# nfrasser/lasgun

Hardware: AMD Instinct MI355X
Metric: Mrays/s (primary+shadow) at 4096x4096; bit-exact RGBA8 vs CPU (higher is better)
Workload: dtype f64; 1 GPU; configs[2]: 4096x4096, Cornell shell + 1024 random plastic spheres (SplitMix64 0x1A560001), 1 spp, 1 point light; workload_key=configs2, rays_per_frame=33554429, primary=16777216

## Files before the change

bindings/rust/lasgun-hip-sys/src/lib.rs:

```rust
#![allow(non_camel_case_types)]

use std::os::raw::{c_char, c_int, c_void};

#[repr(C)]
pub struct lg_scene {
    _private: [u8; 0],
}
#[repr(C)]
pub struct lg_aggregate {
    _private: [u8; 0],
}
#[repr(C)]
pub struct lg_accel {
    _private: [u8; 0],
}
#[repr(C)]
pub struct lg_film {
    _private: [u8; 0],
}
#[repr(C)]
pub struct lg_multi {
    _private: [u8; 0],
}

// ... 250 lines not shown
    pub fn lg_scene_set_perspective_camera(a0: *mut lg_scene, fov: f64);
    pub fn lg_scene_set_orthographic_camera(a0: *mut lg_scene, scale: f64);
    pub fn lg_camera_look_at(a0: *mut lg_scene, origin: *const [f64; 3], look: *const [f64; 3], up: *const [f64; 3]);
    pub fn lg_camera_set_supersampling(a0: *mut lg_scene, base: u8);
    pub fn lg_camera_set_aperture_radius(a0: *mut lg_scene, radius: f64);
    pub fn lg_scene_set_solid_background(a0: *mut lg_scene, color: *const [f64; 3]);
    pub fn lg_scene_set_radial_background(a0: *mut lg_scene, inner: *const [f64; 3], outer: *const [f64; 3], scale: f64);
    pub fn lg_scene_set_ambient_light(a0: *mut lg_scene, color: *const [f64; 3]);
    pub fn lg_scene_set_mesh_smoothing(a0: *mut lg_scene, enabled: c_int);
    pub fn lg_scene_set_max_recursion_depth(a0: *mut lg_scene, max_depth: u32);
    pub fn lg_scene_set_threads(a0: *mut lg_scene, threads: usize);
    pub fn lg_scene_add_point_light(a0: *mut lg_scene, position: *const [f64; 3], intensity: *const [f64; 3], falloff: *const [f64; 3]);
    pub fn lg_scene_parse_obj(a0: *mut lg_scene, text: *const c_char, len: usize, out_ref: *mut u32) -> c_int;
    pub fn lg_scene_load_obj(a0: *mut lg_scene, path: *const c_char, out_ref: *mut u32) -> c_int;
    pub fn lg_scene_root(a0: *mut lg_scene) -> *mut lg_aggregate;
    pub fn lg_scene_set_root(a0: *mut lg_scene, moved: *mut lg_aggregate);
    pub fn lg_aggregate_new() -> *mut lg_aggregate;
    pub fn lg_aggregate_free(a0: *mut lg_aggregate);
    pub fn lg_aggregate_add_group(a0: *mut lg_aggregate, moved: *mut lg_aggregate);
    pub fn lg_aggregate_add_sphere(a0: *mut lg_aggregate, center: *const [f64; 3], radius: f64, a3: *const lg_material);
    pub fn lg_aggregate_add_cube(a0: *mut lg_aggregate, origin: *const [f64; 3], dim: f64, a3: *const lg_material);
    pub fn lg_aggregate_add_box(a0: *mut lg_aggregate, minbound: *const [f64; 3], maxbound: *const [f64; 3], a3: *const lg_material);
    pub fn lg_aggregate_add_obj(a0: *mut lg_aggregate, mesh: u32);
    pub fn lg_aggregate_add_obj_of(a0: *mut lg_aggregate, mesh: u32, a2: *const lg_material);
    pub fn lg_aggregate_swap_backface(a0: *mut lg_aggregate);
    pub fn lg_aggregate_translate(a0: *mut lg_aggregate, delta: *const [f64; 3]);
    pub fn lg_aggregate_scale(a0: *mut lg_aggregate, x: f64, y: f64, z: f64);
    pub fn lg_aggregate_rotate_x(a0: *mut lg_aggregate, theta_deg: f64);
    pub fn lg_aggregate_rotate_y(a0: *mut lg_aggregate, theta_deg: f64);
    pub fn lg_aggregate_rotate_z(a0: *mut lg_aggregate, theta_deg: f64);
    pub fn lg_aggregate_rotate(a0: *mut lg_aggregate, theta_deg: f64, axis: *const [f64; 3]);
    pub fn lg_film_new(width: u32, height: u32) -> *mut lg_film;
    pub fn lg_film_wrap(width: u32, height: u32, rgba: *mut u8) -> *mut lg_film;
    pub fn lg_film_pixels(a0: *mut lg_film) -> *mut u8;
    pub fn lg_film_width(a0: *mut lg_film) -> u32;
    pub fn lg_film_height(a0: *mut lg_film) -> u32;
    pub fn lg_film_free(a0: *mut lg_film);
    pub fn lg_accel_from(a0: *const lg_scene) -> *mut lg_accel;
    pub fn lg_accel_free(a0: *mut lg_accel);
    pub fn lg_capture(a0: *const lg_scene, a1: *mut lg_film) -> c_int;
    pub fn lg_capture_subset(k: usize, n: usize, a2: *const lg_accel, a3: *mut lg_film) -> c_int;
    pub fn lg_render(a0: *const lg_scene, width: u32, height: u32) -> *mut lg_film;
    pub fn lg_set_device(device: c_int) -> c_int;
    pub fn lg_device_count() -> c_int;
    pub fn lg_trim_pool(device: c_int) -> u64;
    pub fn lg_set_devices(device_ids: *const c_int, count: c_int) -> c_int;
    pub fn lg_accel_from_on(a0: *const lg_scene, device: c_int) -> *mut lg_accel;
    pub fn lg_multi_create(a0: *const lg_scene, device_ids: *const c_int, count: c_int, block_rows: u32) -> *mut lg_multi;
    pub fn lg_multi_free(a0: *mut lg_multi);
    pub fn lg_multi_capture_device(a0: *mut lg_multi, width: u32, height: u32, dev_rgba_on_root: *mut c_void) -> c_int;
    pub fn lg_multi_capture(a0: *mut lg_multi, a1: *mut lg_film) -> c_int;
    pub fn lg_multi_capture_device_all(a0: *mut lg_multi, width: u32, height: u32, dev_rgba: *mut *const c_void) -> c_int;
    pub fn lg_multi_rank_count(a0: *const lg_multi) -> c_int;
    pub fn lg_multi_accel(a0: *const lg_multi, rank: c_int) -> *mut lg_accel;
    pub fn lg_multi_uses_rccl(a0: *const lg_multi) -> c_int;
    pub fn lg_capture_rows_device(a0: *const lg_accel, width: u32, height: u32, y0: u32, y1: u32, row0: u32, dev_rgba: *mut c_void, hip_stream: *mut c_void) -> c_int;
    pub fn lg_capture_interleaved_device(a0: *const lg_accel, width: u32, height: u32, block_rows: u32, n: u32, r: u32, dev_rgba: *mut c_void, hip_stream: *mut c_void) -> c_int;
    pub fn lg_capture_subset_device(k: usize, n: usize, a2: *const lg_accel, width: u32, height: u32, dev_rgba: *mut c_void, hip_stream: *mut c_void) -> c_int;
    pub fn lg_capture_subsets(ks: *const usize, count: usize, n: usize, a3: *const lg_accel, a4: *mut lg_film) -> c_int;
    pub fn lg_capture_subsets_device(ks: *const usize, count: usize, n: usize, a3: *const lg_accel, width: u32, height: u32, dev_rgba: *mut c_void, hip_stream: *mut c_void) -> c_int;
    pub fn lg_accel_stream(a0: *const lg_accel) -> *mut c_void;
    pub fn lg_accel_synchronize(a0: *const lg_accel) -> c_int;
    pub fn lg_capture_radiance(k: usize, n: usize, a2: *const lg_accel, width: u32, height: u32, rgb: *mut f64) -> c_int;
    pub fn lg_capture_pixels(a0: *const lg_accel, width: u32, height: u32, offsets: *const u64, count: usize, rgba_out: *mut u8, rgb_out: *mut f64) -> c_int;
    pub fn lg_capture_rect(a0: *const lg_accel, width: u32, height: u32, x0: u32, y0: u32, x1: u32, y1: u32, rgba_out: *mut u8, rgb_out: *mut f64) -> c_int;
    pub fn lg_capture_stats(a0: *const lg_accel, width: u32, height: u32, y0: u32, y1: u32, out: *mut lg_stats) -> c_int;
    pub fn lg_audit_prune(a0: *const lg_accel, width: u32, height: u32, y0: u32, y1: u32, out: *mut lg_prune_audit) -> c_int;
    pub fn lg_audit_fast(a0: *const lg_accel, width: u32, height: u32, y0: u32, y1: u32, out: *mut lg_fast_audit) -> c_int;
    pub fn lg_accel_set_mode(a0: *const lg_accel, mode: c_int) -> c_int;
    pub fn lg_accel_set_prune(a0: *const lg_accel, enabled: c_int) -> c_int;
    pub fn lg_accel_set_shadow_skip(a0: *const lg_accel, enabled: c_int) -> c_int;
    pub fn lg_accel_set_level_door(a0: *const lg_accel, mask: c_int) -> c_int;
    pub fn lg_accel_set_l0_relative(a0: *const lg_accel, enabled: c_int) -> c_int;
    pub fn lg_accel_last_l0_relative(a0: *const lg_accel) -> c_int;
    pub fn lg_scene_l0_relative_origins(a0: *const lg_scene, origins: *mut f64, cap: c_int) -> c_int;
    pub fn lg_accel_set_node_pairs(a0: *const lg_accel, enabled: c_int) -> c_int;
    pub fn lg_accel_last_node_pairs(a0: *const lg_accel) -> c_int;
    pub fn lg_accel_set_packet_walk(a0: *const lg_accel, enabled: c_int) -> c_int;
    pub fn lg_accel_last_packet_walk(a0: *const lg_accel) -> c_int;
    pub fn lg_scene_packet_walk_gate(a0: *const lg_scene) -> c_int;
    pub fn lg_accel_set_fused_shade(a0: *const lg_accel, enabled: c_int) -> c_int;
    pub fn lg_accel_last_fused_shade(a0: *const lg_accel) -> c_int;
    pub fn lg_scene_fused_shade_gate(a0: *const lg_scene, camera_level0: c_int) -> c_int;
    pub fn lg_scene_lds_image(a0: *const lg_scene, pairs: c_int, words: *mut u32, cap: usize, info: *mut u32) -> i64;
    pub fn lg_accel_get_prune(a0: *const lg_accel) -> c_int;
    pub fn lg_accel_set_streaming(a0: *const lg_accel, enabled: c_int) -> c_int;
    pub fn lg_tune_export(out: *mut lg_tune_entry, capacity: usize) -> usize;
    pub fn lg_tune_import(entries: *const lg_tune_entry, count: usize) -> c_int;
    pub fn lg_tune_clear();
    pub fn lg_accel_last_organisation(a0: *const lg_accel) -> c_int;
    pub fn lg_accel_set_tile_order(a0: *const lg_accel, order: c_int) -> c_int;
    pub fn lg_accel_set_sample_order(a0: *const lg_accel, order: c_int) -> c_int;
    pub fn lg_accel_set_tile_parts(a0: *const lg_accel, parts: c_int) -> c_int;
    pub fn lg_accel_set_wf_split(a0: *const lg_accel, bands: c_int) -> c_int;
    pub fn lg_accel_set_lds_scene(a0: *const lg_accel, enabled: c_int) -> c_int;
    pub fn lg_profile_enable(a0: *const lg_accel, enabled: c_int);
    pub fn lg_profile_read(a0: *const lg_accel, total_ms: *mut f64, launches: *mut u64) -> c_int;
    pub fn lg_profile_read_kinds(a0: *const lg_accel, ms: *mut [f64; 5], launches: *mut [u64; 5]) -> c_int;
    pub fn lg_capture_stats_kind(a0: *const lg_accel, width: u32, height: u32, y0: u32, y1: u32, kind: c_int, out: *mut lg_stats) -> c_int;
    pub fn lg_accel_dump(a0: *const lg_accel, f: *mut *const f64, nf: *mut usize, i: *mut *const i64, ni: *mut usize) -> c_int;
    pub fn lg_accel_info(a0: *const lg_accel, out: *mut [u64; 8]) -> c_int;
    pub fn lg_aggregate_get_transform(a0: *mut lg_aggregate, m: *mut [f64; 16], minv: *mut [f64; 16]);
    pub fn lg_host_build_dump(a0: *const lg_scene, f: *mut *const f64, nf: *mut usize, i: *mut *const i64, ni: *mut usize, info: *mut [u64; 8]) -> c_int;
    pub fn lg_host_check_wide_records(a0: *const lg_scene, out: *mut [u64; 8]) -> c_int;
    pub fn lg_host_check_strips(a0: *const lg_scene, out: *mut [u64; 8]) -> c_int;
    pub fn lg_trace_pixel(a0: *const lg_accel, width: u32, height: u32, x: u32, y: u32, fast: c_int, out: *mut f64, out_len: usize) -> c_int;
    pub fn lg_intersect(a0: *const lg_accel, rays: *const f64, n: usize, hits: *mut lg_hit) -> c_int;
    pub fn lg_occluded(a0: *const lg_accel, rays: *const f64, n: usize, occluded: *mut u8) -> c_int;
    pub fn lg_intersect_device(a0: *const lg_accel, dev_rays: *const f64, n: usize, dev_hits: *mut lg_hit, hip_stream: *mut c_void) -> c_int;
    pub fn lg_occluded_device(a0: *const lg_accel, dev_rays: *const f64, n: usize, dev_occluded: *mut u8, hip_stream: *mut c_void) -> c_int;
    pub fn lg_visibility(a0: *const lg_accel, from: *const f64, n_from: usize, to: *const f64, n_to: usize, bits: *mut u8, row_bytes: usize, blocked: *mut u32) -> c_int;
    pub fn lg_visibility_device(a0: *const lg_accel, dev_from: *const f64, n_from: usize, dev_to: *const f64, n_to: usize, dev_bits: *mut u8, row_bytes: usize, dev_blocked: *mut u32, hip_stream: *mut c_void) -> c_int;
    pub fn lg_open_directions(a0: *const lg_accel, points: *const f64, normals: *const f64, n_points: usize, dirs: *const f64, n_dirs: usize, bits: *mut u8, row_bytes: usize, open: *mut u32, above: *mut u32) -> c_int;
    pub fn lg_open_directions_device(a0: *const lg_accel, dev_points: *const f64, dev_normals: *const f64, n_points: usize, dev_dirs: *const f64, n_dirs: usize, dev_bits: *mut u8, row_bytes: usize, dev_open: *mut u32, dev_above: *mut u32, hip_stream: *mut c_void) -> c_int;
    pub fn lg_range_scan(a0: *const lg_accel, origins: *const f64, frames: *const f64, n_poses: usize, beams: *const f64, n_beams: usize, lanes: c_int, out: *const lg_scan_out) -> c_int;
    pub fn lg_range_scan_device(a0: *const lg_accel, dev_origins: *const f64, dev_frames: *const f64, n_poses: usize, dev_beams: *const f64, n_beams: usize, lanes: c_int, dev_out: *const lg_scan_out, hip_stream: *mut c_void) -> c_int;
    pub fn lg_range_scan_lanes(n_poses: usize, n_beams: usize, lanes: c_int) -> c_int;
    pub fn lg_radiance(a0: *const lg_accel, rays: *const f64, n: usize, radiance: *mut f64) -> c_int;
    pub fn lg_radiance_device(a0: *const lg_accel, dev_rays: *const f64, n: usize, dev_radiance: *mut f64, hip_stream: *mut c_void) -> c_int;
    pub fn lg_radiance_gather(a0: *const lg_accel, origins: *const f64, frames: *const f64, n_poses: usize, dirs: *const f64, n_dirs: usize, weights: *const f64, n_weights: usize, lanes: c_int, out: *const lg_gather_out) -> c_int;
    pub fn lg_radiance_gather_device(a0: *const lg_accel, dev_origins: *const f64, dev_frames: *const f64, n_poses: usize, dev_dirs: *const f64, n_dirs: usize, dev_weights: *const f64, n_weights: usize, lanes: c_int, dev_out: *const lg_gather_out, hip_stream: *mut c_void) -> c_int;
    pub fn lg_radiance_gather_lanes(n_poses: usize, n_dirs: usize, lanes: c_int) -> c_int;
    pub fn lg_camera_rays(a0: *const lg_accel, width: u32, height: u32, x0: u32, y0: u32, x1: u32, y1: u32, rays: *mut f64) -> c_int;
    pub fn lg_camera_rays_device(a0: *const lg_accel, width: u32, height: u32, x0: u32, y0: u32, x1: u32, y1: u32, dev_rays: *mut f64, hip_stream: *mut c_void) -> c_int;
    pub fn lg_camera_samples(a0: *const lg_accel) -> u32;
    pub fn lg_capture_rays(a0: *const lg_accel, rays: *const f64, pixels: usize, samples: u32, pixel_offsets: *const u64, film: *mut lg_film, rgb: *mut f64, width: u32, height: u32) -> c_int;
    pub fn lg_capture_rays_device(a0: *const lg_accel, dev_rays: *const f64, pixels: usize, samples: u32, dev_pixel_offsets: *const u64, width: u32, height: u32, dev_rgba: *mut c_void, dev_rgb: *mut f64, hip_stream: *mut c_void) -> c_int;
    pub fn lg_capture_features(a0: *const lg_accel, width: u32, height: u32, x0: u32, y0: u32, x1: u32, y1: u32, out: *const lg_features, material_rgb: *const f64) -> c_int;
    pub fn lg_capture_features_device(a0: *const lg_accel, width: u32, height: u32, x0: u32, y0: u32, x1: u32, y1: u32, dev_out: *const lg_features, dev_material_rgb: *const f64, hip_stream: *mut c_void) -> c_int;
    pub fn lg_accel_material_count(a0: *const lg_accel) -> usize;
    pub fn lg_lens_rays(a0: *const lg_lens, width: u32, height: u32, samples_root: u32, pixel_offsets: *const u64, pixels: usize, rays: *mut f64) -> c_int;
    pub fn lg_lens_rays_device(device: c_int, a1: *const lg_lens, width: u32, height: u32, samples_root: u32, dev_pixel_offsets: *const u64, pixels: usize, dev_rays: *mut f64, hip_stream: *mut c_void) -> c_int;
    pub fn lg_view_look_at(out: *mut lg_view, perspective: c_int, param: f64, origin: *const [f64; 3], look: *const [f64; 3], up: *const [f64; 3], supersampling: u8) -> c_int;
    pub fn lg_scene_view(a0: *const lg_scene, out: *mut lg_view) -> c_int;
    pub fn lg_accel_view(a0: *const lg_accel, out: *mut lg_view) -> c_int;
    pub fn lg_view_rays(a0: *const lg_accel, a1: *const lg_view, width: u32, height: u32, x0: u32, y0: u32, x1: u32, y1: u32, rays: *mut f64) -> c_int;
    pub fn lg_view_rays_device(a0: *const lg_accel, a1: *const lg_view, width: u32, height: u32, x0: u32, y0: u32, x1: u32, y1: u32, dev_rays: *mut f64, hip_stream: *mut c_void) -> c_int;
    pub fn lg_capture_views(a0: *const lg_accel, views: *const lg_view, n_views: usize, width: u32, height: u32, rgba: *mut u8, rgb: *mut f64) -> c_int;
    pub fn lg_capture_views_device(a0: *const lg_accel, views: *const lg_view, n_views: usize, width: u32, height: u32, dev_rgba: *mut c_void, dev_rgb: *mut f64, hip_stream: *mut c_void) -> c_int;
    pub fn lg_capture_view_features(a0: *const lg_accel, views: *const lg_view, n_views: usize, width: u32, height: u32, out: *const lg_view_features, material_rgb: *const f64) -> c_int;
    pub fn lg_capture_view_features_device(a0: *const lg_accel, views: *const lg_view, n_views: usize, width: u32, height: u32, dev_out: *const lg_view_features, dev_material_rgb: *const f64, hip_stream: *mut c_void) -> c_int;
    pub fn lg_hit_layers(a0: *const lg_accel, rays: *const f64, n: usize, max_layers: u32, out: *const lg_layers_out) -> c_int;
    pub fn lg_hit_layers_device(a0: *const lg_accel, dev_rays: *const f64, n: usize, max_layers: u32, dev_out: *const lg_layers_out, hip_stream: *mut c_void) -> c_int;
    pub fn lg_trace_paths(a0: *const lg_accel, rays: *const f64, n: usize, max_bounces: u32, rules: *const lg_path_rule, n_rules: usize, normal: c_int, start_medium: *const u32, out: *const lg_paths_out) -> c_int;
    pub fn lg_trace_paths_device(a0: *const lg_accel, dev_rays: *const f64, n: usize, max_bounces: u32, rules: *const lg_path_rule, n_rules: usize, normal: c_int, dev_start_medium: *const u32, dev_out: *const lg_paths_out, hip_stream: *mut c_void) -> c_int;
    pub fn lg_radiance_groups(a0: *const lg_accel, rays: *const f64, n: usize, groups: *const lg_light_group, n_groups: usize, radiance: *mut f64) -> c_int;
    pub fn lg_radiance_groups_device(a0: *const lg_accel, dev_rays: *const f64, n: usize, groups: *const lg_light_group, n_groups: usize, dev_radiance: *mut f64, hip_stream: *mut c_void) -> c_int;
    pub fn lg_scatter(a0: *const lg_accel, rays: *const f64, n: usize, out: *const lg_scatter_out) -> c_int;
    pub fn lg_scatter_device(a0: *const lg_accel, dev_rays: *const f64, n: usize, dev_out: *const lg_scatter_out, hip_stream: *mut c_void) -> c_int;
    pub fn lg_scatter_lit(a0: *const lg_accel, rays: *const f64, n: usize, lights: *const lg_light_set, out: *const lg_lit_out) -> c_int;
    pub fn lg_scatter_lit_device(a0: *const lg_accel, dev_rays: *const f64, n: usize, lights: *const lg_light_set, dev_out: *const lg_lit_out, hip_stream: *mut c_void) -> c_int;
    pub fn lg_hit_attributes(a0: *const lg_accel, rays: *const f64, n: usize, out: *const lg_attr_out) -> c_int;
    pub fn lg_hit_attributes_device(a0: *const lg_accel, dev_rays: *const f64, n: usize, dev_out: *const lg_attr_out, hip_stream: *mut c_void) -> c_int;
    pub fn lg_hit_attributes_of(a0: *const lg_accel, rays: *const f64, hits: *const lg_hit, n: usize, out: *const lg_attr_out) -> c_int;
    pub fn lg_hit_attributes_of_device(a0: *const lg_accel, dev_rays: *const f64, dev_hits: *const lg_hit, n: usize, dev_out: *const lg_attr_out, hip_stream: *mut c_void) -> c_int;
    pub fn lg_closest_points(a0: *const lg_accel, points: *const f64, n: usize, radius: f64, out: *const lg_closest_out) -> c_int;
    pub fn lg_closest_points_device(a0: *const lg_accel, dev_points: *const f64, n: usize, radius: f64, dev_out: *const lg_closest_out, hip_stream: *mut c_void) -> c_int;
    pub fn lg_scene_closest_gate(a0: *const lg_scene, shrink: *mut f64, cap: c_int) -> c_int;
    pub fn lg_scene_closest_depth(a0: *const lg_scene) -> c_int;
    pub fn lg_accel_light_count(a0: *const lg_accel) -> c_int;
    pub fn lg_accel_set_query_order(a0: *const lg_accel, order: c_int) -> c_int;
    pub fn lg_accel_get_query_order(a0: *const lg_accel) -> c_int;
    pub fn lg_query_order(a0: *const lg_accel, rays: *const f64, n: usize, perm: *mut u32, keys: *mut u32) -> c_int;
    pub fn lg_query_order_device(a0: *const lg_accel, dev_rays: *const f64, n: usize, dev_perm: *mut u32, dev_keys: *mut u32, hip_stream: *mut c_void) -> c_int;
    pub fn lg_accel_material(a0: *const lg_accel, index: i32, out: *mut lg_material) -> c_int;
    pub fn lg_accel_instance(a0: *const lg_accel, instance: u32, parent: *mut i32, obj_ref: *mut i64) -> c_int;
// ... 6 lines not shown
```

include/lasgun_hip.h:

```cpp
#ifndef LASGUN_HIP_H
#define LASGUN_HIP_H

#include <stddef.h>
#include <stdint.h>

#ifdef __cplusplus
extern "C" {
#endif

typedef struct lg_scene lg_scene;
typedef struct lg_aggregate lg_aggregate;
typedef struct lg_accel lg_accel;
typedef struct lg_film lg_film;

typedef struct lg_material {
    int32_t kind;
    double p[10];
} lg_material;

const char *lg_last_error(void);

lg_material lg_material_default(void);
lg_material lg_material_matte(const double kd[3], double sigma);
lg_material lg_material_plastic(const double kd[3], const double ks[3], double roughness);
// ... 35 lines not shown
void lg_aggregate_rotate_y(lg_aggregate *, double theta_deg);
void lg_aggregate_rotate_z(lg_aggregate *, double theta_deg);
void lg_aggregate_rotate(lg_aggregate *, double theta_deg, const double axis[3]);

lg_film *lg_film_new(uint32_t width, uint32_t height);
lg_film *lg_film_wrap(uint32_t width, uint32_t height, uint8_t *rgba);
uint8_t *lg_film_pixels(lg_film *);
uint32_t lg_film_width(lg_film *);
uint32_t lg_film_height(lg_film *);
void lg_film_free(lg_film *);

lg_accel *lg_accel_from(const lg_scene *);
void lg_accel_free(lg_accel *);

int lg_capture(const lg_scene *, lg_film *);
int lg_capture_subset(size_t k, size_t n, const lg_accel *, lg_film *);
lg_film *lg_render(const lg_scene *, uint32_t width, uint32_t height);

typedef struct lg_stats {
    uint64_t primary_rays, shadow_rays, secondary_rays, nodes_tested, spheres_tested, cuboids_tested, triangles_tested,
        accel_entries, hits;
} lg_stats;

int lg_set_device(int device);
int lg_device_count(void);
uint64_t lg_trim_pool(int device);
int lg_set_devices(const int *device_ids, int count);

lg_accel *lg_accel_from_on(const lg_scene *, int device);

typedef struct lg_multi lg_multi;
lg_multi *lg_multi_create(const lg_scene *, const int *device_ids, int count, uint32_t block_rows);
void lg_multi_free(lg_multi *);
int lg_multi_capture_device(lg_multi *, uint32_t width, uint32_t height, void *dev_rgba_on_root);
int lg_multi_capture(lg_multi *, lg_film *);
int lg_multi_capture_device_all(lg_multi *, uint32_t width, uint32_t height, void *const *dev_rgba);
int lg_multi_rank_count(const lg_multi *);
lg_accel *lg_multi_accel(const lg_multi *, int rank);
int lg_multi_uses_rccl(const lg_multi *);

int lg_capture_rows_device(const lg_accel *, uint32_t width, uint32_t height, uint32_t y0, uint32_t y1, uint32_t row0,
                           void *dev_rgba, void *hip_stream);
int lg_capture_interleaved_device(const lg_accel *, uint32_t width, uint32_t height, uint32_t block_rows, uint32_t n,
                                  uint32_t r, void *dev_rgba, void *hip_stream);
int lg_capture_subset_device(size_t k, size_t n, const lg_accel *, uint32_t width, uint32_t height, void *dev_rgba,
                             void *hip_stream);
int lg_capture_subsets(const size_t *ks, size_t count, size_t n, const lg_accel *, lg_film *);
int lg_capture_subsets_device(const size_t *ks, size_t count, size_t n, const lg_accel *, uint32_t width, uint32_t height,
                              void *dev_rgba, void *hip_stream);
void *lg_accel_stream(const lg_accel *);
int lg_accel_synchronize(const lg_accel *);

int lg_capture_radiance(size_t k, size_t n, const lg_accel *, uint32_t width, uint32_t height, double *rgb);
int lg_capture_pixels(const lg_accel *, uint32_t width, uint32_t height, const uint64_t *offsets, size_t count,
                      uint8_t *rgba_out, double *rgb_out);
int lg_capture_rect(const lg_accel *, uint32_t width, uint32_t height, uint32_t x0, uint32_t y0, uint32_t x1, uint32_t y1,
                    uint8_t *rgba_out, double *rgb_out);
int lg_capture_stats(const lg_accel *, uint32_t width, uint32_t height, uint32_t y0, uint32_t y1, lg_stats *out);

typedef struct lg_prune_audit {
    uint64_t skipped_nodes, skipped_runs, primitives, violations;
    double min_slack_nodes, min_slack_runs;
    double max_margin_used_nodes;
} lg_prune_audit;
int lg_audit_prune(const lg_accel *, uint32_t width, uint32_t height, uint32_t y0, uint32_t y1, lg_prune_audit *out);
typedef struct lg_fast_audit { uint64_t rays, fallbacks, violations; } lg_fast_audit;
int lg_audit_fast(const lg_accel *, uint32_t width, uint32_t height, uint32_t y0, uint32_t y1, lg_fast_audit *out);

int lg_accel_set_mode(const lg_accel *, int mode);
int lg_accel_set_prune(const lg_accel *, int enabled);
int lg_accel_set_shadow_skip(const lg_accel *, int enabled);
int lg_accel_set_level_door(const lg_accel *, int mask);
int lg_accel_set_l0_relative(const lg_accel *, int enabled);
int lg_accel_last_l0_relative(const lg_accel *);
int lg_scene_l0_relative_origins(const lg_scene *, double *origins, int cap);
int lg_accel_set_node_pairs(const lg_accel *, int enabled);
int lg_accel_last_node_pairs(const lg_accel *);
int lg_accel_set_packet_walk(const lg_accel *, int enabled);
int lg_accel_last_packet_walk(const lg_accel *);
int lg_scene_packet_walk_gate(const lg_scene *);
int lg_accel_set_fused_shade(const lg_accel *, int enabled);
int lg_accel_last_fused_shade(const lg_accel *);
int lg_scene_fused_shade_gate(const lg_scene *, int camera_level0);
int64_t lg_scene_lds_image(const lg_scene *, int pairs, uint32_t *words, size_t cap, uint32_t *info);
int lg_accel_get_prune(const lg_accel *);

int lg_accel_set_streaming(const lg_accel *, int enabled);
typedef struct lg_tune_entry { uint64_t key[12]; int32_t choice; int32_t reserved; } lg_tune_entry;
size_t lg_tune_export(lg_tune_entry *out, size_t capacity);
int lg_tune_import(const lg_tune_entry *entries, size_t count);
void lg_tune_clear(void);
int lg_accel_last_organisation(const lg_accel *);
int lg_accel_set_tile_order(const lg_accel *, int order);
int lg_accel_set_sample_order(const lg_accel *, int order);
int lg_accel_set_tile_parts(const lg_accel *, int parts);


int lg_accel_set_wf_split(const lg_accel *, int bands);

int lg_accel_set_lds_scene(const lg_accel *, int enabled);


void lg_profile_enable(const lg_accel *, int enabled);
int lg_profile_read(const lg_accel *, double *total_ms, uint64_t *launches);
int lg_profile_read_kinds(const lg_accel *, double ms[5], uint64_t launches[5]);
int lg_capture_stats_kind(const lg_accel *, uint32_t width, uint32_t height, uint32_t y0, uint32_t y1, int kind, lg_stats *out);

int lg_accel_dump(const lg_accel *, const double **f, size_t *nf, const int64_t **i, size_t *ni);
int lg_accel_info(const lg_accel *, uint64_t out[8]);
void lg_aggregate_get_transform(lg_aggregate *, double m[16], double minv[16]);
int lg_host_build_dump(const lg_scene *, const double **f, size_t *nf, const int64_t **i, size_t *ni, uint64_t info[8]);
int lg_host_check_wide_records(const lg_scene *, uint64_t out[8]);
int lg_host_check_strips(const lg_scene *, uint64_t out[8]);

int lg_trace_pixel(const lg_accel *, uint32_t width, uint32_t height, uint32_t x, uint32_t y, int fast, double *out, size_t out_len);

typedef struct lg_hit {
    double t;
    double p[3];
    double ng[3];
    double ns[3];
    uint32_t kind;
    uint32_t prim;
    uint32_t instance;
    int32_t material;
} lg_hit;

int lg_intersect(const lg_accel *, const double *rays, size_t n, lg_hit *hits);
int lg_occluded(const lg_accel *, const double *rays, size_t n, uint8_t *occluded);
int lg_intersect_device(const lg_accel *, const double *dev_rays, size_t n, lg_hit *dev_hits, void *hip_stream);
int lg_occluded_device(const lg_accel *, const double *dev_rays, size_t n, uint8_t *dev_occluded, void *hip_stream);
int lg_visibility(const lg_accel *, const double *from, size_t n_from, const double *to, size_t n_to, uint8_t *bits, size_t row_bytes,
                  uint32_t *blocked);
int lg_visibility_device(const lg_accel *, const double *dev_from, size_t n_from, const double *dev_to, size_t n_to, uint8_t *dev_bits,
                         size_t row_bytes, uint32_t *dev_blocked, void *hip_stream);
int lg_open_directions(const lg_accel *, const double *points, const double *normals, size_t n_points, const double *dirs, size_t n_dirs,
                       uint8_t *bits, size_t row_bytes, uint32_t *open, uint32_t *above);
int lg_open_directions_device(const lg_accel *, const double *dev_points, const double *dev_normals, size_t n_points,
                              const double *dev_dirs, size_t n_dirs, uint8_t *dev_bits, size_t row_bytes, uint32_t *dev_open,
                              uint32_t *dev_above, void *hip_stream);
typedef struct lg_scan_out {
    float    *range;
    float    *point;
    float    *normal;
    uint32_t *id;
    uint32_t *hits;
    float    *nearest;
} lg_scan_out;
int lg_range_scan(const lg_accel *, const double *origins, const double *frames, size_t n_poses, const double *beams, size_t n_beams,
                  int lanes, const lg_scan_out *out);
int lg_range_scan_device(const lg_accel *, const double *dev_origins, const double *dev_frames, size_t n_poses, const double *dev_beams,
                         size_t n_beams, int lanes, const lg_scan_out *dev_out, void *hip_stream);
int lg_range_scan_lanes(size_t n_poses, size_t n_beams, int lanes);
int lg_radiance(const lg_accel *, const double *rays, size_t n, double *radiance);
int lg_radiance_device(const lg_accel *, const double *dev_rays, size_t n, double *dev_radiance, void *hip_stream);
typedef struct lg_gather_out {
    double *radiance;
    double *sums;
} lg_gather_out;
int lg_radiance_gather(const lg_accel *, const double *origins, const double *frames, size_t n_poses, const double *dirs, size_t n_dirs,
                       const double *weights, size_t n_weights, int lanes, const lg_gather_out *out);
int lg_radiance_gather_device(const lg_accel *, const double *dev_origins, const double *dev_frames, size_t n_poses, const double *dev_dirs,
                              size_t n_dirs, const double *dev_weights, size_t n_weights, int lanes, const lg_gather_out *dev_out,
                              void *hip_stream);
int lg_radiance_gather_lanes(size_t n_poses, size_t n_dirs, int lanes);
int lg_camera_rays(const lg_accel *, uint32_t width, uint32_t height, uint32_t x0, uint32_t y0, uint32_t x1, uint32_t y1, double *rays);
// ... 185 lines not shown
```

lasgun_amd/__init__.py:

```python
import ctypes as _C
import os as _os

import numpy as _np

from ._capi import Api, CStats, LasgunError, ObjError, QUERY_ORDER_SIGNATURES, RADIANCE_SIGNATURES, RAY_FILM_SIGNATURES, VISIBILITY_SIGNATURES, DIRECTIONS_SIGNATURES, RANGE_SCAN_SIGNATURES, HIT_LAYERS_SIGNATURES, PATHS_SIGNATURES, LIGHT_GROUPS_SIGNATURES, GATHER_SIGNATURES, FEATURES_SIGNATURES, VIEWS_SIGNATURES, VIEW_FEATURES_SIGNATURES, CView, CLens, CFeatures, CViewFeatures, CScanOut, CLayersOut, CPathRule, CPathsOut, CGatherOut, CLightGroup, GROUP_AMBIENT, MAX_LIGHT_GROUPS, SCATTER_SIGNATURES, CScatterOut, SCATTER_HIT, SCATTER_REFLECT, SCATTER_REFRACT, LIT_SIGNATURES, CLight, CLightSet, CLitOut, MAX_CALL_LIGHTS, ATTRIBUTES_SIGNATURES, CAttrOut, ATTR_HIT, ATTR_NO_HIT, ATTR_BAD_RECORD, CLOSEST_SIGNATURES, CClosestOut
from . import scenes

_HERE = _os.path.dirname(_os.path.abspath(__file__))
LIB_PATH = _os.environ.get("LASGUN_HIP_LIB") or _os.path.join(_HERE, "liblasgun_hip.so")

if not _os.path.exists(LIB_PATH):
    raise ImportError(
        "lasgun_amd: %s is missing -- build it with `python -c 'import __graft_entry__ as g; g.build()'` "
        "or `make -C lasgun_amd/csrc` (there is no CPU fallback)" % LIB_PATH)

_EXTRA = {
    "set_device": (_C.c_int, [_C.c_int]),
    "device_count": (_C.c_int, []),
    "trim_pool": (_C.c_uint64, [_C.c_int]),
    "set_devices": (_C.c_int, [_C.POINTER(_C.c_int), _C.c_int]),
    "capture_rows_device": (_C.c_int, [_C.c_void_p, _C.c_uint32, _C.c_uint32, _C.c_uint32, _C.c_uint32, _C.c_uint32,
                                       _C.c_void_p, _C.c_void_p]),
    "capture_subset_device": (_C.c_int, [_C.c_size_t, _C.c_size_t, _C.c_void_p, _C.c_uint32, _C.c_uint32, _C.c_void_p,
                                         _C.c_void_p]),
    "capture_subsets": (_C.c_int, [_C.POINTER(_C.c_size_t), _C.c_size_t, _C.c_size_t, _C.c_void_p, _C.c_void_p]),
    "capture_subsets_device": (_C.c_int, [_C.POINTER(_C.c_size_t), _C.c_size_t, _C.c_size_t, _C.c_void_p, _C.c_uint32, _C.c_uint32, _C.c_void_p,
                                          _C.c_void_p]),
    "capture_interleaved_device": (_C.c_int, [_C.c_void_p, _C.c_uint32, _C.c_uint32, _C.c_uint32, _C.c_uint32, _C.c_uint32,
                                              _C.c_void_p, _C.c_void_p]),
    "accel_stream": (_C.c_void_p, [_C.c_void_p]),
    "accel_set_mode": (_C.c_int, [_C.c_void_p, _C.c_int]),
    "accel_set_prune": (_C.c_int, [_C.c_void_p, _C.c_int]),
    "accel_set_shadow_skip": (_C.c_int, [_C.c_void_p, _C.c_int]),
    "accel_set_level_door": (_C.c_int, [_C.c_void_p, _C.c_int]),
    "accel_set_l0_relative": (_C.c_int, [_C.c_void_p, _C.c_int]),
    "accel_last_l0_relative": (_C.c_int, [_C.c_void_p]),
    "scene_l0_relative_origins": (_C.c_int, [_C.c_void_p, _C.POINTER(_C.c_double), _C.c_int]),
    "accel_set_node_pairs": (_C.c_int, [_C.c_void_p, _C.c_int]),
    "accel_last_node_pairs": (_C.c_int, [_C.c_void_p]),
    "accel_set_packet_walk": (_C.c_int, [_C.c_void_p, _C.c_int]),
    "accel_last_packet_walk": (_C.c_int, [_C.c_void_p]),
    "scene_packet_walk_gate": (_C.c_int, [_C.c_void_p]),
    "accel_set_fused_shade": (_C.c_int, [_C.c_void_p, _C.c_int]),
    "accel_last_fused_shade": (_C.c_int, [_C.c_void_p]),
    "scene_fused_shade_gate": (_C.c_int, [_C.c_void_p, _C.c_int]),
    "scene_lds_image": (_C.c_longlong, [_C.c_void_p, _C.c_int, _C.POINTER(_C.c_uint32), _C.c_size_t, _C.POINTER(_C.c_uint32)]),
    "accel_set_streaming": (_C.c_int, [_C.c_void_p, _C.c_int]),
    "accel_get_prune": (_C.c_int, [_C.c_void_p]),
    "accel_last_organisation": (_C.c_int, [_C.c_void_p]),
    "accel_set_tile_order": (_C.c_int, [_C.c_void_p, _C.c_int]),
    "accel_set_sample_order": (_C.c_int, [_C.c_void_p, _C.c_int]),
    "accel_set_tile_parts": (_C.c_int, [_C.c_void_p, _C.c_int]),
    "accel_set_lds_scene": (_C.c_int, [_C.c_void_p, _C.c_int]),
    "accel_set_wf_split": (_C.c_int, [_C.c_void_p, _C.c_int]),
    "accel_synchronize": (_C.c_int, [_C.c_void_p]),
    "capture_radiance": (_C.c_int, [_C.c_size_t, _C.c_size_t, _C.c_void_p, _C.c_uint32, _C.c_uint32, _C.c_void_p]),
    "capture_pixels": (_C.c_int, [_C.c_void_p, _C.c_uint32, _C.c_uint32, _C.c_void_p, _C.c_size_t, _C.c_void_p, _C.c_void_p]),
    "capture_rect": (_C.c_int, [_C.c_void_p, _C.c_uint32, _C.c_uint32, _C.c_uint32, _C.c_uint32, _C.c_uint32, _C.c_uint32, _C.c_void_p, _C.c_void_p]),
    "audit_prune": (_C.c_int, [_C.c_void_p, _C.c_uint32, _C.c_uint32, _C.c_uint32, _C.c_uint32, _C.c_void_p]),
    "audit_fast": (_C.c_int, [_C.c_void_p, _C.c_uint32, _C.c_uint32, _C.c_uint32, _C.c_uint32, _C.c_void_p]),
    "capture_stats": (_C.c_int, [_C.c_void_p, _C.c_uint32, _C.c_uint32, _C.c_uint32, _C.c_uint32, _C.POINTER(CStats)]),
    "profile_enable": (None, [_C.c_void_p, _C.c_int]),
    "profile_read_kinds": (_C.c_int, [_C.c_void_p, _C.c_double * 5, _C.c_uint64 * 5]),
    "capture_stats_kind": (_C.c_int, [_C.c_void_p, _C.c_uint32, _C.c_uint32, _C.c_uint32, _C.c_uint32, _C.c_int, _C.POINTER(CStats)]),
    "profile_read": (_C.c_int, [_C.c_void_p, _C.POINTER(_C.c_double), _C.POINTER(_C.c_uint64)]),
    "probe_rate": (_C.c_int, [_C.c_int, _C.POINTER(_C.c_double)]),
    "accel_from_on": (_C.c_void_p, [_C.c_void_p, _C.c_int]),
    "tune_export": (_C.c_size_t, [_C.c_void_p, _C.c_size_t]),
    "tune_import": (_C.c_int, [_C.c_void_p, _C.c_size_t]),
    "tune_clear": (None, []),
    "multi_create": (_C.c_void_p, [_C.c_void_p, _C.POINTER(_C.c_int), _C.c_int, _C.c_uint32]),
    "multi_free": (None, [_C.c_void_p]),
    "multi_capture_device": (_C.c_int, [_C.c_void_p, _C.c_uint32, _C.c_uint32, _C.c_void_p]),
    "multi_capture": (_C.c_int, [_C.c_void_p, _C.c_void_p]),
    "multi_capture_device_all": (_C.c_int, [_C.c_void_p, _C.c_uint32, _C.c_uint32, _C.POINTER(_C.c_void_p)]),
    "multi_rank_count": (_C.c_int, [_C.c_void_p]),
    "multi_accel": (_C.c_void_p, [_C.c_void_p, _C.c_int]),
    "multi_uses_rccl": (_C.c_int, [_C.c_void_p]),
    "accel_info": (_C.c_int, [_C.c_void_p, _C.c_uint64 * 8]),
    "trace_pixel": (_C.c_int, [_C.c_void_p, _C.c_uint32, _C.c_uint32, _C.c_uint32, _C.c_uint32, _C.c_int, _C.POINTER(_C.c_double), _C.c_size_t]),
    "host_build_dump": (_C.c_int, [_C.c_void_p, _C.POINTER(_C.POINTER(_C.c_double)), _C.POINTER(_C.c_size_t),
                                   _C.POINTER(_C.POINTER(_C.c_int64)), _C.POINTER(_C.c_size_t), _C.c_uint64 * 8]),
    "host_check_wide_records": (_C.c_int, [_C.c_void_p, _C.c_uint64 * 8]),
    "host_check_strips": (_C.c_int, [_C.c_void_p, _C.c_uint64 * 8]),
    "intersect": (_C.c_int, [_C.c_void_p, _C.c_void_p, _C.c_size_t, _C.c_void_p]),
    "occluded": (_C.c_int, [_C.c_void_p, _C.c_void_p, _C.c_size_t, _C.c_void_p]),
    "intersect_device": (_C.c_int, [_C.c_void_p, _C.c_void_p, _C.c_size_t, _C.c_void_p, _C.c_void_p]),
    "occluded_device": (_C.c_int, [_C.c_void_p, _C.c_void_p, _C.c_size_t, _C.c_void_p, _C.c_void_p]),
    "camera_rays": (_C.c_int, [_C.c_void_p] + [_C.c_uint32] * 6 + [_C.c_void_p]),
    "camera_rays_device": (_C.c_int, [_C.c_void_p] + [_C.c_uint32] * 6 + [_C.c_void_p, _C.c_void_p]),
    "camera_samples": (_C.c_uint32, [_C.c_void_p]),
    "accel_material": (_C.c_int, [_C.c_void_p, _C.c_int32, _C.c_void_p]),
    "accel_instance": (_C.c_int, [_C.c_void_p, _C.c_uint32, _C.POINTER(_C.c_int32), _C.POINTER(_C.c_int64)]),
    **QUERY_ORDER_SIGNATURES,
    **RADIANCE_SIGNATURES,
    **RAY_FILM_SIGNATURES,
    **VISIBILITY_SIGNATURES,
    **DIRECTIONS_SIGNATURES,
    **RANGE_SCAN_SIGNATURES,
    **HIT_LAYERS_SIGNATURES,
    **PATHS_SIGNATURES,
    **SCATTER_SIGNATURES,
    **LIT_SIGNATURES,
    **ATTRIBUTES_SIGNATURES,
    **CLOSEST_SIGNATURES,
    **LIGHT_GROUPS_SIGNATURES,
    **GATHER_SIGNATURES,
    **FEATURES_SIGNATURES,
    **VIEWS_SIGNATURES,
    **VIEW_FEATURES_SIGNATURES,
}


class Hit(_C.Structure):
    _fields_ = [("t", _C.c_double), ("p", _C.c_double * 3), ("ng", _C.c_double * 3), ("ns", _C.c_double * 3),
                ("kind", _C.c_uint32), ("prim", _C.c_uint32), ("instance", _C.c_uint32), ("material", _C.c_int32)]


HIT_DTYPE = _np.dtype(Hit)
assert _C.sizeof(Hit) == 96 and HIT_DTYPE.itemsize == 96, "lg_hit is 96 bytes"
LENS_EQUIRECTANGULAR, LENS_FISHEYE = 0, 1
assert _C.sizeof(CLens) == 112, "lg_lens is 112 bytes"
assert _C.sizeof(CFeatures) == 40, "lg_features is 40 bytes"
FEATURE_PLANES = ("depth", "normal", "albedo", "coverage", "id")
assert _C.sizeof(CScanOut) == 48, "lg_scan_out is 48 bytes"
SCAN_PLANES = ("range", "point", "normal", "id", "hits", "nearest")
_SCAN_SHAPE = {"range": ((), _np.float32, True), "point": ((3,), _np.float32, True), "normal": ((3,), _np.float32, True), "id": ((4,), _np.uint32, True),
               "hits": ((), _np.uint32, False), "nearest": ((), _np.float32, False)}
SCAN_LANES = {"auto": 0, "beam": 1, "pose": 2}
assert _C.sizeof(CLayersOut) == 40, "lg_layers_out is 40 bytes"
LAYER_PLANES = ("hits", "along", "id", "count", "inside")
_LAYER_SHAPE = {"hits": ((), HIT_DTYPE, True), "along": ((), _np.float64, True), "id": ((4,), _np.uint32, True), "count": ((), _np.uint32, False),
                "inside": ((), _np.float64, False)}
assert _C.sizeof(CPathRule) == 24 and _C.sizeof(CPathsOut) == 72, "lg_path_rule is 24 bytes, lg_paths_out 72"
PATH_PLANES = ("hits", "point", "id", "along", "count", "end", "gain", "last", "medium")
_PATH_SHAPE = {"hits": ((), HIT_DTYPE, True), "point": ((3,), _np.float64, True), "id": ((4,), _np.uint32, True), "along": ((), _np.float64, True),
               "count": ((), _np.uint32, False), "end": ((), _np.uint32, False), "gain": ((), _np.float64, False), "last": ((6,), _np.float64, False),
               "medium": ((), _np.uint32, False)}
PATH_ABSORB, PATH_REFLECT, PATH_PASS, PATH_REFRACT = 0, 1, 2, 3
PATH_END_CUT, PATH_END_ESCAPED, PATH_END_ABSORBED, PATH_END_DEGENERATE = 0, 1, 2, 3
PATH_RULE_DTYPE = _np.dtype([("action", _np.uint32), ("reserved", _np.uint32), ("ior", _np.float64), ("gain", _np.float64)])
assert PATH_RULE_DTYPE.itemsize == 24
assert _C.sizeof(CScatterOut) == 56, "lg_scatter_out is 56 bytes"
SCATTER_PLANES = ("hits", "direct", "flags", "reflect", "reflect_weight", "refract", "refract_weight")
_SCATTER_SHAPE = {"hits": ((), HIT_DTYPE), "direct": ((3,), _np.float64), "flags": ((), _np.uint32), "reflect": ((6,), _np.float64),
                  "reflect_weight": ((3,), _np.float64), "refract": ((6,), _np.float64), "refract_weight": ((5,), _np.float64)}
assert _C.sizeof(CLight) == 72 and _C.sizeof(CLightSet) == 40 and _C.sizeof(CLitOut) == 72, "lg_light is 72 bytes, lg_light_set 40, lg_lit_out 72"
LIT_PLANES = SCATTER_PLANES + ("terms", "visible")
assert _C.sizeof(CAttrOut) == 56, "lg_attr_out is 56 bytes"
ATTR_PLANES = ("hits", "flags", "bary", "uv", "local", "frame", "dp")
_ATTR_SHAPE = {"hits": ((), HIT_DTYPE), "flags": ((), _np.uint32), "bary": ((3,), _np.float64), "uv": ((2,), _np.float64), "local": ((3,), _np.float64),
               "frame": ((6,), _np.float64), "dp": ((6,), _np.float64)}
assert _C.sizeof(CClosestOut) == 24, "lg_closest_out is 24 bytes"
CLOSEST_PLANES = ("distance", "point", "id")
_CLOSEST_SHAPE = {"distance": ((), _np.float64), "point": ((3,), _np.float64), "id": ((4,), _np.uint32)}
LIGHT_DTYPE = _np.dtype([("position", _np.float64, (3,)), ("intensity", _np.float64, (3,)), ("falloff", _np.float64, (3,))])
assert LIGHT_DTYPE.itemsize == 72


def Light(position, intensity, falloff=(1.0, 0.0, 0.0)):
    return (tuple(float(x) for x in position), tuple(float(x) for x in intensity), tuple(float(x) for x in falloff))


def lights_array(lights):
    if isinstance(lights, _np.ndarray) and lights.dtype == LIGHT_DTYPE:
        return _np.ascontiguousarray(lights)
    if isinstance(lights, _np.ndarray):
        a = _np.ascontiguousarray(lights, dtype=_np.float64)
        if a.ndim < 1 or a.shape[-1] != 9:
            raise ValueError("lights: the last axis holds position, intensity and falloff, nine doubles")
        return a.view(LIGHT_DTYPE).reshape(a.shape[:-1])
    out = _np.zeros(len(lights), dtype=LIGHT_DTYPE)
    for k, (p, i, f) in enumerate(lights):
        out[k] = (p, i, f)
    return out


assert _C.sizeof(CGatherOut) == 16, "lg_gather_out is 16 bytes"
GATHER_PLANES = ("radiance", "sums")
GATHER_LANES = {"auto": 0, "direction": 1, "pose": 2}
_FEATURE_SHAPE = {"depth": ((), _np.float32), "normal": ((3,), _np.float32), "albedo": ((3,), _np.float32), "coverage": ((), _np.float32),
                  "id": ((4,), _np.uint32)}
assert _C.sizeof(CViewFeatures) == 48, "lg_view_features is 48 bytes"
VIEW_FEATURE_PLANES = FEATURE_PLANES + ("point",)
_VIEW_FEATURE_SHAPE = dict(_FEATURE_SHAPE, point=((3,), _np.float32))


def Lens(kind, origin, right, up, forward, fov_deg=180.0):
    three = lambda v: (_C.c_double * 3)(*[float(c) for c in v])
    return CLens(int(kind), 0, three(origin), three(right), three(up), three(forward), float(fov_deg))


View = CView


def _views(views):
    vs = [views] if isinstance(views, CView) else list(views)
    for v in vs:
        if not isinstance(v, CView):
            raise TypeError("views: View records (lasgun_amd.View)")
    return (CView * len(vs))(*vs)


# ... 18 lines not shown
            return _C.c_void_p(self.call("accel_stream", accel.h))
        return _C.c_void_p(int(stream))

    def set_mode(self, accel, fast):
        if self.call("accel_set_mode", accel.h, 1 if fast else 0):
            raise LasgunError(self.last_error())

    def set_prune(self, accel, enabled):
        if self.call("accel_set_prune", accel.h, -1 if enabled is None or enabled == -1 else (1 if enabled else 0)):
            raise LasgunError(self.last_error())

    def set_shadow_skip(self, accel, enabled):
        if self.call("accel_set_shadow_skip", accel.h, 1 if enabled else 0):
            raise LasgunError(self.last_error())

    def set_level_door(self, accel, mask):
        if self.call("accel_set_level_door", accel.h, int(mask)):
            raise LasgunError(self.last_error())

    def set_l0_relative(self, accel, enabled):
        if self.call("accel_set_l0_relative", accel.h, 1 if enabled else 0):
            raise LasgunError(self.last_error())

    def last_l0_relative(self, accel):
        v = self.call("accel_last_l0_relative", accel.h)
        return None if v < 0 else bool(v)

    def set_node_pairs(self, accel, enabled):
        if self.call("accel_set_node_pairs", accel.h, 1 if enabled else 0):
            raise LasgunError(self.last_error())

    def last_node_pairs(self, accel):
        v = self.call("accel_last_node_pairs", accel.h)
        return None if v < 0 else bool(v)

    def set_packet_walk(self, accel, enabled):
        if self.call("accel_set_packet_walk", accel.h, 1 if enabled else 0):
            raise LasgunError(self.last_error())

    def last_packet_walk(self, accel):
        v = self.call("accel_last_packet_walk", accel.h)
        return None if v < 0 else bool(v)

    def scene_lds_image(self, scene, pairs):
        info = (_C.c_uint32 * 8)()
        n = self.call("scene_lds_image", scene.h, 1 if pairs else 0, None, 0, info)
        if n < 0:
            raise LasgunError(self.last_error())
        if n == 0:
            return None
        words = _np.zeros(n, dtype=_np.uint32)
        self.call("scene_lds_image", scene.h, 1 if pairs else 0, words.ctypes.data_as(_C.POINTER(_C.c_uint32)), n, info)
        keys = ("units", "node_off", "prim_off", "soup_off", "accel_off", "pairs", "accels", "nodes")
        return words, {k: int(info[i]) for i, k in enumerate(keys)}

    def l0_relative_origins(self, scene):
        import numpy as np
        out = np.zeros((64, 3), dtype=np.float64)
        n = self.call("scene_l0_relative_origins", scene.h, out.ctypes.data_as(_C.POINTER(_C.c_double)), 64)
        if n < 0:
            raise LasgunError(self.last_error())
        return out[:n].copy() if n else None

    def scene_packet_walk_gate(self, scene):
        v = self.call("scene_packet_walk_gate", scene.h)
        if v < 0:
            raise LasgunError(self.last_error())
        return int(v)

    def set_fused_shade(self, accel, enabled):
        if self.call("accel_set_fused_shade", accel.h, 1 if enabled else 0):
            raise LasgunError(self.last_error())

    def last_fused_shade(self, accel):
        v = self.call("accel_last_fused_shade", accel.h)
        return None if v < 0 else bool(v)

    def scene_fused_shade_gate(self, scene, camera_level0=True):
        v = self.call("scene_fused_shade_gate", scene.h, 1 if camera_level0 else 0)
        if v < 0:
            raise LasgunError(self.last_error())
        return int(v)

    def last_organisation(self, accel):
        v = self.call("accel_last_organisation", accel.h)
        name = {0: "megakernel", 1: "wavefront", 2: "queue"}.get(v & 15) if v >= 0 else None
        if name and (v & 16):
            name += ", bottom-up"
        if name and (v & 64):
            name += ", middle-out"
        if name and (v & 32):
            name += ", samples in a row"
        if name and (v & 128):
            name += ", tiles in parts"
        return name

    def set_tile_order(self, accel, order):
        if self.call("accel_set_tile_order", accel.h, -1 if order is None else int(order)):
            raise LasgunError(self.last_error())

    def set_tile_parts(self, accel, parts):
        if self.call("accel_set_tile_parts", accel.h, -1 if parts is None else int(parts)):
            raise LasgunError(self.last_error())

    def set_sample_order(self, accel, order):
        if self.call("accel_set_sample_order", accel.h, -1 if order is None else int(order)):
            raise LasgunError(self.last_error())

    def get_prune(self, accel):
        return bool(self.call("accel_get_prune", accel.h))

    def set_streaming(self, accel, enabled):
        if self.call("accel_set_streaming", accel.h, int(enabled) if enabled in (0, 1, 2, 3) else (1 if enabled else 0)):
            raise LasgunError(self.last_error())

    def set_wf_split(self, accel, bands):
        self.call("accel_set_wf_split", accel.h, int(bands))

    def set_lds_scene(self, accel, enabled):
        return bool(self.call("accel_set_lds_scene", accel.h, 1 if enabled else 0))

    def set_device(self, device):
        if self.call("set_device", int(device)):
            raise LasgunError(self.last_error())

    def trace_pixel_log(self, accel, w, h, x, y, fast=False, nlights=1):
        need = 7 + 2 * nlights
        n = need + 1 + 4 * 4000
        out = (_C.c_double * n)()
        if self.call("trace_pixel", accel.h, int(w), int(h), int(x), int(y), 1 if fast else 0, out, n):
            raise LasgunError(self.last_error())
        cnt = int(out[need])
        return [tuple(out[need + 1 + 4 * i + k] for k in range(4)) for i in range(cnt)]

    def trace_pixel(self, accel, w, h, x, y, fast=False, max_lights=64):
        n = 7 + 2 * max_lights
        out = (_C.c_double * n)()
        if self.call("trace_pixel", accel.h, int(w), int(h), int(x), int(y), 1 if fast else 0, out, n):
            raise LasgunError(self.last_error())
        nl = int(out[3])
        return {"t": out[0], "ref": int(out[1]), "accel": int(out[2]), "shadow": [(out[4 + 2 * l], int(out[5 + 2 * l])) for l in range(nl)],
                "shadow_origin": [out[4 + 2 * nl], out[5 + 2 * nl], out[6 + 2 * nl]]}

    def set_devices(self, ids=None):
        ids = list(ids or [])
        arr = (_C.c_int * max(len(ids), 1))(*ids)
        if self.call("set_devices", arr, len(ids)):
            raise LasgunError(self.last_error())

    def trim_pool(self, device=-1):
        return int(self.call("trim_pool", int(device)))

    def device_count(self):
        return int(self.call("device_count"))

    def capture_rows_device(self, accel, width, height, y0, y1, dev_ptr, row0=None, stream=None):
        if self.call("capture_rows_device", accel.h, width, height, y0, y1, y0 if row0 is None else row0,
                     _C.c_void_p(int(dev_ptr)), self._stream(accel, stream)):
            raise LasgunError(self.last_error())

    def capture_interleaved_device(self, accel, width, height, block_rows, n, r, dev_ptr, stream=None):
        if self.call("capture_interleaved_device", accel.h, width, height, block_rows, n, r, _C.c_void_p(int(dev_ptr)),
                     self._stream(accel, stream)):
            raise LasgunError(self.last_error())

    def capture_subset_device(self, k, n, accel, width, height, dev_ptr, stream=None):
# ... 1101 lines not shown
```

lasgun_amd/csrc/accel.cpp:

```cpp
#include "internal.h"
#include "attributes_host.h"
#include "pairs_host.h"

static std::vector<uint32_t> attr_counts_of(const FlatScene &f, const Scene &scene) {
    std::vector<uint32_t> faces(f.accels.size(), 0u), tri_base(f.accels.size(), 0u), sphere_accel(f.spheres.size(), NO_HIT), cuboid_accel(f.cuboids.size(), NO_HIT);
    std::vector<uint32_t> todo;
    for (size_t id = 0; id < f.accels.size(); ++id) {
        const DAccel &A = f.accels[id];
        if (A.flags & AF_MESH) {
            const int64_t obj = id < f.accel_obj.size() ? f.accel_obj[id] : -1;
            if (obj >= 0 && (size_t)obj < scene.meshes.size() && scene.meshes[(size_t)obj]) faces[id] = (uint32_t)(scene.meshes[(size_t)obj]->tri.size() / 3);
            tri_base[id] = id < f.accel_tri_base.size() ? f.accel_tri_base[id] : 0u;
            if ((size_t)tri_base[id] + faces[id] > f.tri_v.size() / 3) faces[id] = 0u;
            continue;
        }
        if (A.node_base >= f.nodes.size()) continue;
        todo.assign(1, 0u);
        while (!todo.empty()) {
            const uint32_t nidx = todo.back();
            todo.pop_back();
            const DNode &nd = f.nodes[A.node_base + nidx];
            if (!(nd.meta & NODE_LEAF)) { todo.push_back(nidx + 1u); todo.push_back(nd.link); continue; }
            for (uint32_t k = 0; k < (nd.meta & 0xFFFFu); ++k) {
                const uint32_t ref = f.primref[(size_t)A.prim_base + nd.link + k], kind = ref >> 30, idx = ref & PRIM_INDEX_MASK;
                if (kind == PK_SPHERE && idx < sphere_accel.size()) sphere_accel[idx] = (uint32_t)id;
                else if (kind == PK_CUBOID && idx < cuboid_accel.size()) cuboid_accel[idx] = (uint32_t)id;
            }
        }
    }
    return attr_counts_build(faces, tri_base, sphere_accel, cuboid_accel);
}

static void set_lds_limits(size_t bytes, bool ldss) {
    for (auto set : {mega_set_lds_limit, wf_set_lds_limit, queue_set_lds_limit, query_set_lds_limit, rq_set_lds_limit, visibility_set_lds_limit, features_set_lds_limit,
                     open_directions_set_lds_limit, range_scan_set_lds_limit, hit_layers_set_lds_limit, trace_paths_set_lds_limit, gather_set_lds_limit, view_set_lds_limit, view_features_set_lds_limit, light_groups_set_lds_limit, scatter_set_lds_limit, lit_set_lds_limit, attributes_set_lds_limit})
        HIP_TRY(set(bytes, ldss));
}

constexpr size_t LDS_MAX = 160 * 1024;
static bool make_lds_image(lg_accel *a, size_t big_mesh_tris, std::vector<uint32_t> &img) {
    static const bool times = std::getenv("LASGUN_DEBUG_TIMES") != nullptr;
    a->lds_image_n16 = 0; a->lds_pairs = false; a->pair_refusal.clear(); a->pair_rel.clear();
    {
        {
            FlatScene &fm = a->flat;
            std::vector<uint32_t> nb, pb;
            for (const DAccel &A : fm.accels) { nb.push_back(A.node_base); nb.push_back(A.fnode_base); pb.push_back(A.prim_base); pb.push_back(A.fprim_base); }
            std::sort(nb.begin(), nb.end()); nb.erase(std::unique(nb.begin(), nb.end()), nb.end());
            std::sort(pb.begin(), pb.end()); pb.erase(std::unique(pb.begin(), pb.end()), pb.end());
            auto extent = [](const std::vector<uint32_t> &starts, uint32_t b, size_t total) {
                auto it = std::upper_bound(starts.begin(), starts.end(), b);
                return (uint32_t)((it == starts.end() ? total : (size_t)*it) - b);
            };
            std::vector<std::pair<uint32_t, uint32_t>> nruns, pruns;
            uint32_t nn = 0, np = 0;
            uint32_t np_soup = 0;
            const size_t stack_bytes = (size_t)a->stack_depth * 1024 * 4;
            const size_t accel16 = fm.accels.size() * LDS_ACCEL_UNITS;
            auto number = [&](bool own_trees) {
                nruns.clear(); pruns.clear(); nn = np = np_soup = 0;
                for (int pass = 0; pass < 2; ++pass) {
                  if (pass == 1) np_soup = np;
                  for (DAccel &A : fm.accels) {
                    if (((A.flags & AF_MESH) != 0u) != (pass == 1)) continue;
                    auto fn = own_trees ? nruns.end() : std::find_if(nruns.begin(), nruns.end(), [&](auto &r) { return r.first == A.node_base; });
                    if (fn == nruns.end()) { nruns.emplace_back(A.node_base, nn); A.lnode_base = nn; nn += extent(nb, A.node_base, fm.nodes.size()); }
                    else A.lnode_base = fn->second;
                    auto fp = std::find_if(pruns.begin(), pruns.end(), [&](auto &r) { return r.first == A.prim_base; });
                    if (fp == pruns.end()) { pruns.emplace_back(A.prim_base, np); A.lprim_base = np; np += extent(pb, A.prim_base, fm.primref.size()); }
                    else A.lprim_base = fp->second;
                  }
                }
                return (size_t)nn * LDS_NODE_STRIDE + ((size_t)np + 3) / 4 + (size_t)np_soup * 3 + accel16;
            };
            size_t n16 = number(false);
            if (fm.accels.size() <= L0_REL_MAX_ACCELS && nruns.size() < fm.accels.size()) {
                const size_t shared16 = n16, own16 = number(true);
                if (stack_bytes + own16 * 16 > LDS_MAX || (own16 - shared16) * 16 > shared16) n16 = number(false);
                else n16 = own16;
            }
            const size_t prim16 = ((size_t)np + 3) / 4;
            a->l0_rel.clear();
            if (stack_bytes + n16 * 16 <= LDS_MAX) {
                img.assign(n16 * 4, 0u);
                a->lds_node_off = 0;
                for (auto &r : nruns)
                    for (uint32_t i = 0, e = extent(nb, r.first, fm.nodes.size()); i < e; ++i) {
                        uint32_t *rec = &img[((size_t)(r.second + i) * LDS_NODE_STRIDE) * 4];
                        std::memcpy(rec, &fm.nodes[r.first + i], 56);
                    }
                a->lds_prim_off = nn * LDS_NODE_STRIDE;
                a->lds_soup_off = a->lds_prim_off + (uint32_t)prim16;
                for (auto &r : pruns)
                    for (uint32_t i = 0, e = extent(pb, r.first, fm.primref.size()); i < e; ++i) {
                        img[(size_t)a->lds_prim_off * 4 + r.second + i] = fm.primref[r.first + i];
                        if (r.second + i < np_soup)
                            std::memcpy(&img[((size_t)a->lds_soup_off + (size_t)(r.second + i) * 3) * 4], &fm.leaf_soup[r.first + i], 48);
                    }
                for (const DAccel &A : fm.accels) {
                    const uint32_t tree0 = a->lds_node_off * 16u + A.lnode_base * LDS_NODE_STRIDE * 16u;
                    for (uint32_t i = 0, e = extent(nb, A.node_base, fm.nodes.size()); i < e; ++i) {
                        uint32_t *rec = &img[((size_t)(A.lnode_base + i) * LDS_NODE_STRIDE) * 4];
                        const DNode &nd = fm.nodes[A.node_base + i];
                        if (nd.meta & NODE_LEAF) { rec[16] = A.lprim_base + nd.link; rec[17] = NODE_LEAF; rec[18] = rec[16] + (nd.meta & 0xFFFFu); rec[19] = nd.pad; }
                        else { rec[16] = tree0 + nd.link * LDS_NODE_STRIDE * 16u; rec[17] = 1u << (nd.meta & 3u); rec[18] = 0u; }
                        rec[17] |= nd.meta & NODE_NOPRUNE;
                    }
                }
                a->lds_accel_off = a->lds_soup_off + np_soup * 3u;
                for (size_t i = 0; i < fm.accels.size(); ++i) {
                    const DAccel &A = fm.accels[i];
                    uint32_t *rec = &img[((size_t)a->lds_accel_off + i * LDS_ACCEL_UNITS) * 4];
                    std::memcpy(rec, &A.minv, 96);
// ... 124 lines not shown
                    double v = (c == 3 ? A.m.c[3][r] : 0.0);
                    for (int k = 0; k < 3; ++k) v += A.m.c[k][r] * (c == 3 ? A.minv.c[3][k] : A.minv.c[c][k]);
                    const double want = (c < 3 && r == c) ? 1.0 : 0.0;
                    if (!(std::fabs(v - want) <= worst)) worst = std::fabs(v - want);
                }
            if (!(worst <= 1e-11)) {
                a->fast_available = false;
                a->fast_refusal = "fast mode unavailable: an aggregate's transform and inverse do not match (rotate() about a non-unit axis?)";
            }
        }
        for (const auto &m : a->scene->meshes) {
            if (!m || !with_fast) continue;
            double max_abs = 0.0, min_edge = INFINITY;
            for (float v : m->position) if (std::isfinite(v)) max_abs = std::fmax(max_abs, std::fabs((double)v));
            for (size_t t = 0; t + 2 < m->tri.size(); t += 3) {
                double longest = 0.0;
                for (int e = 0; e < 3; ++e) {
                    const size_t i = (size_t)m->tri[t + e].v, j = (size_t)m->tri[t + (e + 1) % 3].v;
                    double d2 = 0.0;
                    for (int c = 0; c < 3; ++c) { const double d = (double)m->position[3 * i + c] - (double)m->position[3 * j + c]; d2 += d * d; }
                    longest = std::fmax(longest, std::sqrt(d2));
                }
                if (longest > 0.0 && std::isfinite(longest)) min_edge = std::fmin(min_edge, longest);
            }
            if (std::isfinite(min_edge) && max_abs > min_edge * 0x1p20) {
                a->fast_available = false;
                a->fast_refusal = "fast mode unavailable: a mesh whose coordinates exceed 2^20 times its smallest triangle (a ray in a far triangle's plane is accepted by the reference wherever it passes)";
            }
        }
        if (!a->fast_available) a->stack_depth_fast1 = a->stack_depth;
        a->accel_image_n16 = 0;
        {
            const size_t img = f.accels.size() * LDS_ACCEL_UNITS * 16;
            if (f.accels.size() <= 64 && ((size_t)a->stack_depth * 256 * 4 + img) * 4 <= LDS_MAX) a->accel_image_n16 = (uint32_t)(f.accels.size() * LDS_ACCEL_UNITS);
        }
        const size_t extra_lds = (size_t)a->accel_image_n16 * 16;
        size_t lds = (size_t)std::max(a->stack_depth, a->stack_depth_fast1) * 256 * 4 + extra_lds;
        if (lds > 64 * 1024) set_lds_limits(lds, false);
        int per_cu = 0, cus = 0;
        HIP_TRY(trace_occupancy(a->stack_depth, false, extra_lds, &per_cu));
        int per_cu_fast = 0;
        HIP_TRY(trace_occupancy(a->stack_depth_fast1, true, 0, &per_cu_fast));
        if (per_cu_fast < 1) per_cu_fast = 1;
        a->max_blocks_fast = (uint32_t)per_cu_fast;
        HIP_TRY(hipDeviceGetAttribute(&cus, hipDeviceAttributeMultiprocessorCount, a->device));
        if (per_cu < 1) per_cu = 1;
        a->max_blocks = (uint32_t)(per_cu * cus);
        a->max_blocks_fast *= (uint32_t)cus;
        int wb = 0, wbf = 0;
        HIP_TRY(wf_trace_occupancy(a->stack_depth, false, extra_lds, &wb));
        HIP_TRY(wf_trace_occupancy(a->stack_depth_fast1, true, 0, &wbf));
        a->wf_blocks = (uint32_t)((wb < 1 ? 1 : wb) * cus);
        a->wf_blocks_fast = (uint32_t)((wbf < 1 ? 1 : wbf) * cus);
        int qb = 0;
        HIP_TRY(queue_occupancy(a->stack_depth, extra_lds, &qb));
        a->queue_blocks = (uint32_t)((qb < 1 ? 1 : qb) * cus);
        a->cus = (uint32_t)cus;
        {
            std::vector<uint32_t> img;
            if (make_lds_image(a, big_mesh_tris, img)) {
                stage.add(a->lds_image, img);
                set_lds_limits(LDS_MAX, true);
                a->ldss_blocks = (uint32_t)cus;
            }
            FlatScene &fm = a->flat;
            stage.add(a->accels, fm.accels);
            if (a->accel_image_n16) {
                std::vector<uint32_t> img((size_t)a->accel_image_n16 * 4, 0u);
                for (size_t i = 0; i < fm.accels.size(); ++i) {
                    const DAccel &A = fm.accels[i];
                    uint32_t *rec = &img[i * LDS_ACCEL_UNITS * 4];
                    std::memcpy(rec, &A.minv, 96);
                    rec[24] = A.node_base; rec[25] = A.prim_base; rec[26] = 0u; rec[27] = A.flags;
                    rec[28] = (uint32_t)A.parent; rec[29] = A.nchain; rec[30] = A.lone;
                    for (int k = 0; k < MAX_CHAIN; ++k) rec[32 + k] = A.chain[k];
                    std::memcpy(rec + 40, A.prune, sizeof A.prune);
                    std::memcpy(rec + LDS_ACCEL_DOOR * 4, A.door, sizeof A.door);
                }
                stage.add(a->accel_image, img);
            }
        }
        stage.add(a->accel_tri_base, f.accel_tri_base);
        stage.add(a->attr_counts, attr_counts_of(a->flat, *a->scene));
        stage.commit(a->arena);
        {
            size_t big_mesh = 0;
            for (const auto &m : a->scene->meshes) if (m && m->tri.size() / 3 > big_mesh) big_mesh = m->tri.size() / 3;
            a->prune_default = big_mesh >= PRUNE_MIN_TRIS;
            a->streaming_pays = f.spheres.size() + f.cuboids.size() >= 512 && !(f.has_specular && big_mesh >= 4096);
            a->mega_narrow = f.spheres.size() + f.cuboids.size() < 512;
            bool specular_mesh = false;
            for (const DAccel &A : f.accels)
                if ((A.flags & AF_MESH) && A.material >= 0) {
                    const int kind = f.materials[(size_t)A.material].kind;
                    size_t tris = 0;
                    for (const auto &m : a->scene->meshes) if (m && m->tri.size() / 3 > tris) tris = m->tri.size() / 3;
                    specular_mesh = specular_mesh || ((kind == MAT_GLASS || kind == MAT_MIRROR) && tris >= 4096);
                }
            a->queue_default = f.has_specular && big_mesh >= 4096 && specular_mesh;
            a->streaming_min_items = big_mesh >= 4096 ? (1ull << 23) : (1ull << 21);
        }
        if (times) {
            const auto t_end = std::chrono::steady_clock::now();
            auto ms = [](auto a0, auto a1) { return std::chrono::duration<double, std::milli>(a1 - a0).count(); };
            std::fprintf(stderr, "[lasgun] accel build: flatten %.3f ms, table uploads %.3f ms, streams / occupancy / LDS images %.3f ms\n", ms(t_begin, t_flat), ms(t_flat, t_up), ms(t_up, t_end));
        }
}

static void swap_tables(lg_accel &x, lg_accel &y) {
    using std::swap;
    swap(x.flat, y.flat);
    swap(x.arena, y.arena); swap(x.stats, y.stats);
    swap(x.nodes, y.nodes); swap(x.nodes4, y.nodes4); swap(x.primref, y.primref); swap(x.spheres, y.spheres); swap(x.sphere_mat, y.sphere_mat);
    swap(x.cuboids, y.cuboids); swap(x.cuboid_mat, y.cuboid_mat); swap(x.tri_v, y.tri_v); swap(x.tri_n, y.tri_n); swap(x.tri_t, y.tri_t);
    swap(x.vpos, y.vpos); swap(x.vnorm, y.vnorm); swap(x.vtex, y.vtex); swap(x.leaf_soup, y.leaf_soup); swap(x.chunks, y.chunks); swap(x.strips, y.strips);
    swap(x.sphere_ref_leaf, y.sphere_ref_leaf); swap(x.cuboid_ref_leaf, y.cuboid_ref_leaf); swap(x.tri_ref_leaf, y.tri_ref_leaf); swap(x.accel_ref_leaf, y.accel_ref_leaf);
    swap(x.accels, y.accels); swap(x.materials, y.materials); swap(x.lights, y.lights); swap(x.accel_tri_base, y.accel_tri_base); swap(x.attr_counts, y.attr_counts);
    swap(x.lds_image, y.lds_image); swap(x.accel_image, y.accel_image); swap(x.accel_image_n16, y.accel_image_n16);
    swap(x.lds_image_n16, y.lds_image_n16); swap(x.lds_node_off, y.lds_node_off); swap(x.lds_prim_off, y.lds_prim_off);
    swap(x.lds_soup_off, y.lds_soup_off); swap(x.lds_accel_off, y.lds_accel_off);
    swap(x.ldss_blocks, y.ldss_blocks); swap(x.cus, y.cus); swap(x.l0_rel, y.l0_rel);
    swap(x.lds_pairs, y.lds_pairs); swap(x.pair_refusal, y.pair_refusal); swap(x.pair_rel, y.pair_rel);
    swap(x.stack_depth, y.stack_depth); swap(x.stack_depth_fast1, y.stack_depth_fast1); swap(x.max_blocks, y.max_blocks); swap(x.max_blocks_fast, y.max_blocks_fast);
    swap(x.wf_blocks, y.wf_blocks); swap(x.wf_blocks_fast, y.wf_blocks_fast); swap(x.queue_blocks, y.queue_blocks);
    swap(x.queue_default, y.queue_default); swap(x.prune_default, y.prune_default); swap(x.queue_min_items, y.queue_min_items); swap(x.specular_small_items, y.specular_small_items);
    swap(x.device_bytes, y.device_bytes); swap(x.fast_available, y.fast_available); swap(x.fast_refusal, y.fast_refusal);
    swap(x.streaming_pays, y.streaming_pays); swap(x.streaming_min_items, y.streaming_min_items); swap(x.mega_narrow, y.mega_narrow);
    x.packet_scene = y.packet_scene = -1;
}
void rebuild_tables(const lg_accel *ca, bool fast) {
    if (fast && ca->flat.has_fast) return;
    lg_accel *a = const_cast<lg_accel *>(ca);
    use_device(a->device);
    std::unique_ptr<lg_accel> next(new lg_accel());
    next->scene = a->scene;
    next->device = a->device;
    next->prune = a->prune == 1 || a->flat.has_records ? 1 : a->prune;
    next->node_pairs = a->node_pairs;
    next->image_prune = a->prune;
    build_and_upload(next.get(), fast || a->flat.has_fast);
    next->prune = a->prune;
    if (next->flat.dump_f.size() != a->flat.dump_f.size() ||
        (!a->flat.dump_f.empty() && std::memcmp(next->flat.dump_f.data(), a->flat.dump_f.data(), a->flat.dump_f.size() * sizeof(a->flat.dump_f[0])) != 0) ||
        next->flat.dump_i != a->flat.dump_i)
        throw Error("the scene was modified after lg_accel_from: the accel's reference trees no longer match it (build a new accel)");
    HIP_TRY(hipDeviceSynchronize());
    swap_tables(*a, *next);
    std::swap(a->flat.dump_f, next->flat.dump_f);
    std::swap(a->flat.dump_i, next->flat.dump_i);
}

lg_accel *accel_from_on(const lg_scene *s, int device) {
    lg_accel *a = nullptr;
    int rc = guarded([&] {
        a = new lg_accel();
        a->scene = &s->s;
        a->device = device;
        build_and_upload(a, false);
    });
    if (rc) { delete a; return nullptr; }
    return a;
}
```

lasgun_amd/csrc/capi.cpp:

```cpp
#include "internal.h"
#include "choice.h"
#include "packet_host.h"
#include "fused_host.h"
#include "closest_host.h"

extern "C" {

const char *lg_last_error(void) { return tl_error.c_str(); }

size_t lg_tune_export(lg_tune_entry *out, size_t capacity) {
    const size_t n = lg::tune::snapshot(nullptr, nullptr, 0);
    if (!out || capacity == 0) return n;
    std::vector<lg::tune::Key> keys(capacity);
    std::vector<int> choices(capacity);
    const size_t m = lg::tune::snapshot(keys.data(), choices.data(), capacity);
    for (size_t i = 0; i < std::min(m, capacity); ++i) {
        std::memcpy(out[i].key, keys[i].v, sizeof out[i].key);
        out[i].choice = choices[i];
        out[i].reserved = 0;
    }
    return m;
}
int lg_tune_import(const lg_tune_entry *entries, size_t count) {
    if (count != 0 && !entries) return fail("lg_tune_import: entries is NULL");
// ... 689 lines not shown
int lg_accel_set_packet_walk(const lg_accel *a, int enabled) {
    if (enabled != 0 && enabled != 1) return fail("packet walk must be 0 or 1");
    std::lock_guard<std::mutex> g(a->mtx);
    a->packet_walk = enabled == 1;
    return 0;
}
int lg_accel_last_packet_walk(const lg_accel *a) {
    std::lock_guard<std::mutex> g(a->mtx);
    return a->last_packet_walk;
}
int lg_scene_l0_relative_origins(const lg_scene *s, double *origins, int cap) {
    int n = 0;
    int rc = guarded([&] {
        FlatScene f;
        flatten_scene(s->s, f, false, false);
        const Camera &c = s->s.camera;
        std::vector<V3> local;
        if (!l0_relative_camera(c.origin, c.up, c.aux, c.pixel_separation) || !l0_relative_origins(f, c.origin, local)) return;
        n = (int)local.size();
        for (int i = 0; i < n && i < cap && origins; ++i) { origins[3 * i] = local[(size_t)i].x; origins[3 * i + 1] = local[(size_t)i].y; origins[3 * i + 2] = local[(size_t)i].z; }
    });
    return rc ? -1 : n;
}
int lg_scene_packet_walk_gate(const lg_scene *s) {
    int v = 0;
    int rc = guarded([&] {
        FlatScene f;
        flatten_scene(s->s, f, false, false);
        v = (int)packet_scene_gate(f.accels.data(), f.accels.size(), f.nodes.data(), f.nodes.size(), f.primref.data(), f.primref.size(), f.max_stack + 2u);
    });
    return rc ? -1 : v;
}
int lg_scene_closest_gate(const lg_scene *s, double *shrink, int cap) {
    int v = -1;
    int rc = guarded([&] {
        if (!s) throw Error("scene is NULL");
        FlatScene f;
        flatten_scene(s->s, f, false, false);
        v = closest_gate(ClosestScene{f.accels.data(), f.accels.size(), f.nodes.data(), f.nodes.size(), f.primref.data(), f.primref.size(), f.leaf_soup.data(),
                                      f.leaf_soup.size()}, shrink, cap);
    });
    return rc ? -2 : v;
}
int lg_scene_closest_depth(const lg_scene *s) {
    int v = 0;
    int rc = guarded([&] {
        if (!s) throw Error("scene is NULL");
        FlatScene f;
        flatten_scene(s->s, f, false, false);
        v = (int)closest_tables(ClosestScene{f.accels.data(), f.accels.size(), f.nodes.data(), f.nodes.size(), f.primref.data(), f.primref.size(), f.leaf_soup.data(),
                                             f.leaf_soup.size()}).depth;
    });
    return rc ? -1 : v;
}
int lg_accel_set_fused_shade(const lg_accel *a, int enabled) {
    if (enabled != 0 && enabled != 1) return fail("fused shade must be 0 or 1");
    std::lock_guard<std::mutex> g(a->mtx);
    a->fused_shade = enabled == 1;
    return 0;
}
int lg_accel_last_fused_shade(const lg_accel *a) {
    std::lock_guard<std::mutex> g(a->mtx);
    return a->last_fused_shade;
}
int lg_scene_fused_shade_gate(const lg_scene *s, int camera_level0) {
    int v = 0;
    int rc = guarded([&] {
        FlatScene f;
        flatten_scene(s->s, f, false, false);
        std::vector<uint32_t> img;
        uint32_t inf[8] = {0, 0, 0, 0, 0, 0, 0, 0};
        const bool pairs = scene_lds_image(s->s, true, img, inf) && inf[5] == 1u;
        FusedAsk q;
        q.switched_on = true;
        q.camera_level0 = camera_level0 != 0;
        q.levels = (f.has_specular && s->s.recursion > 0) ? (unsigned)s->s.recursion + 1u : 1u;
        q.nlights = (unsigned long)f.lights.size();
        q.packet_closest = pairs && packet_scene_gate(f.accels.data(), f.accels.size(), f.nodes.data(), f.nodes.size(), f.primref.data(), f.primref.size(), f.max_stack + 2u) == PACKET_OK;
        q.pair_shadow = pairs;
        v = (int)fused_shade_gate(q);
    });
    return rc ? -1 : v;
}
int lg_accel_set_mode(const lg_accel *a, int mode) {
    if (mode != 0 && mode != 1) return fail("mode must be 0 (reference traversal) or 1 (fast)");
    std::lock_guard<std::mutex> g(a->mtx);
    if (mode == 1) {
        int rc = guarded([&] { rebuild_tables(a, true); });
        if (rc) return rc;
    }
    if (mode == 1 && !a->fast_available) return fail(a->fast_refusal);
    a->fast = mode == 1;
    return 0;
}
void lg_profile_enable(const lg_accel *a, int enabled) {
    std::lock_guard<std::mutex> g(a->mtx);
    a->profiling = enabled != 0;
}
int lg_profile_read(const lg_accel *a, double *total_ms, uint64_t *launches) {
    return guarded([&] {
        std::lock_guard<std::mutex> g(a->mtx);
        double total = 0.0;
        for (auto &e : a->events) {
            HIP_TRY(hipEventSynchronize(e.second));
            float ms = 0.f;
            HIP_TRY(hipEventElapsedTime(&ms, e.first, e.second));
            total += ms;
            (void)hipEventDestroy(e.first); (void)hipEventDestroy(e.second);
        }
        *total_ms = total;
        *launches = a->events.size();
        a->events.clear();
    });
}

int lg_profile_read_kinds(const lg_accel *a, double ms[5], uint64_t launches[5]) {
    return guarded([&] {
        std::lock_guard<std::mutex> g(a->mtx);
        for (int k = 0; k < 5; ++k) {
            double total = 0.0;
            for (auto &e : a->kind_events[k]) {
                HIP_TRY(hipEventSynchronize(e.second));
                float t = 0.f;
                HIP_TRY(hipEventElapsedTime(&t, e.first, e.second));
                if (std::getenv("LASGUN_DEBUG")) std::fprintf(stderr, "[lasgun] kind %d launch: %.3f ms\n", k, t);
                total += t;
                (void)hipEventDestroy(e.first); (void)hipEventDestroy(e.second);
            }
            ms[k] = total; launches[k] = a->kind_events[k].size();
            a->kind_events[k].clear();
        }
    });
}
int lg_accel_dump(const lg_accel *a, const double **f, size_t *nf, const int64_t **i, size_t *ni) {
    *f = a->flat.dump_f.data(); *nf = a->flat.dump_f.size();
    *i = a->flat.dump_i.data(); *ni = a->flat.dump_i.size();
    return 0;
}
int lg_host_build_dump(const lg_scene *s, const double **f, size_t *nf, const int64_t **i, size_t *ni, uint64_t info[8]) {
    static thread_local FlatScene flat;
    return guarded([&] {
        flatten_scene(s->s, flat);
        *f = flat.dump_f.data(); *nf = flat.dump_f.size();
        *i = flat.dump_i.data(); *ni = flat.dump_i.size();
        info[0] = flat.nodes.size(); info[1] = flat.primref.size(); info[2] = flat.spheres.size(); info[3] = flat.cuboids.size();
        info[4] = flat.tri_v.size() / 3; info[5] = flat.accels.size(); info[6] = flat.max_stack; info[7] = flat.has_specular ? 1 : 0;
    });
}
int lg_host_check_strips(const lg_scene *s, uint64_t out[8]) {
    return guarded([&] {
        FlatScene flat;
        flatten_scene(s->s, flat, false);
        for (int k = 0; k < 8; ++k) out[k] = 0;
        std::vector<char> seen_node(flat.nodes.size(), 0);
        for (const DAccel &A : flat.accels) {
            if (!(A.flags & AF_MESH)) continue;
            std::vector<uint32_t> todo{0};
            while (!todo.empty()) {
                const uint32_t nidx = todo.back(); todo.pop_back();
                if (seen_node[A.node_base + nidx]) continue;
                seen_node[A.node_base + nidx] = 1;
                const DNode &nd = flat.nodes[A.node_base + nidx];
                if (!(nd.meta & NODE_LEAF)) { todo.push_back(nidx + 1); todo.push_back(nd.link); continue; }
                const uint32_t nrec = nd.pad >> 24, rec0 = nd.pad & 0x00FFFFFFu;
                if (nrec == 0) continue;
                out[0]++;
// ... 244 lines not shown
```

lasgun_amd/csrc/dscene.h:

```cpp
#pragma once
#include "vecmath.h"

namespace lg {

enum PrimKind : uint32_t { PK_SPHERE = 0, PK_CUBOID = 1, PK_TRIANGLE = 2, PK_ACCEL = 3 };
constexpr uint32_t PRIM_INDEX_MASK = 0x3FFFFFFFu;
constexpr uint32_t NO_HIT = 0xFFFFFFFFu;
constexpr uint32_t WF_NONE = 0xFFFFFFFFu, WF_MISS = 0xFFFFFFFEu;
constexpr uint32_t WF_SKIP = 0x80000000u;
constexpr int MAX_CHAIN = 8;
constexpr uint32_t TILE_HEADS = 8u, TILE_HEAD_STRIDE = 32u;
constexpr uint32_t TILE_HEAD0 = 32u, TILE_GONE = 16u;
constexpr uint32_t TILE_COUNTER_WORDS = TILE_HEAD0 + TILE_HEADS * TILE_HEAD_STRIDE;
constexpr uint32_t NO_TILE = 0xFFFFFFFFu;
constexpr uint32_t NODE_LEAF = 0x80000000u;
constexpr uint32_t NODE_NOPRUNE = 0x40000000u;
constexpr double PRUNE_E1 = 0x1p-46;
constexpr double PRUNE_E0_PER_COORD = 0x1p-46;
constexpr double PRUNE_E2_TIMES_RMIN = 0x1p-42;
constexpr double PRUNE_LIMIT_REL = 0x1p-40;
constexpr double PRUNE_RANGE = 0x1p100;
constexpr uint32_t LDS_NODE_STRIDE = 5u;
constexpr uint32_t LDS_ACCEL_UNITS = 16u;
constexpr uint32_t PAIR_REC_BYTES = 112u, PAIR_ROOT_BYTES = 64u, PAIR_WORDS_OFF = 96u, PAIR_ROOT_WORD_OFF = 48u;
// ... 33 lines not shown
struct alignas(64) DChunk {
    float bmin[3], bmax[3];
    float axis[3];
    float cos_t;
    float g2;
    float hmin;
    uint32_t start, count;
    float sin_t;
    uint32_t pad;
};
static_assert(sizeof(DChunk) == 64, "DChunk is one 64-byte line");
struct alignas(16) DStrip {
    float x, y, z;
    uint32_t code;
};
constexpr uint32_t STRIP_TRI = 0x80000000u, STRIP_SLOT_MASK = 0x0FFFFFFFu;
constexpr uint32_t CHUNK_SHIFT = 5u;
constexpr uint32_t CHUNK_GROUP = 2u;
constexpr uint32_t CHUNK_IS_GROUP = 0xFFFFFFFFu;
constexpr float CHUNK_K0 = 0x1p-38f;
constexpr float CHUNK_SIGMA_MIN = 1e-3f;
constexpr float CHUNK_HGATE = 0x1p-40f;

struct DMaterial {
    int32_t kind;
    int32_t pad;
    double p[10];
};
enum MatKind : int32_t { MAT_MATTE = 0, MAT_PLASTIC = 1, MAT_METAL = 2, MAT_GLASS = 3, MAT_MIRROR = 4 };

struct DLight {
    double pos[3], intensity[3], falloff[3];
};

enum AccelFlags : uint32_t { AF_SWAP_BACKFACE = 1, AF_MESH = 2, AF_HAS_N = 4, AF_HAS_UV = 8, AF_IDENTITY = 16  };

struct alignas(16) DAccel {
    Affine m;
    Affine minv;
    uint32_t node_base;
    uint32_t prim_base;
    int32_t parent;
    int32_t material;
    uint32_t flags;
    uint32_t nchain;
    uint32_t chain[MAX_CHAIN];
    uint32_t fnode_base;
    uint32_t fprim_base;
    uint32_t lnode_base;
    uint32_t lprim_base;
    uint32_t lone;
    uint32_t pad;
    double prune[6];
    double door[6];
};

constexpr uint32_t QC_FINISHED = 0u, QC_ERROR = 32u, QC_HEADS = 64u , QC_LEVEL0 = 384u,
                   QC_LEVEL_WORDS = 128u, QC_COUNT = 0u, QC_CLAIMED = 32u, QC_STATE = 64u;
constexpr uint32_t QC_MAX_LEVELS = 8u;
constexpr uint32_t QC_WORDS = QC_LEVEL0 + QC_LEVEL_WORDS * QC_MAX_LEVELS;
constexpr uint32_t QR_LAST = 0x80000000u;
constexpr uint32_t QR_SLACK = 16u;

struct DStats {
    unsigned long long primary_rays, shadow_rays, secondary_rays, nodes_tested, spheres_tested, cuboids_tested,
        triangles_tested, accel_entries, hits;
    unsigned long long audit_nodes, audit_runs, audit_prims, audit_violations, audit_slack_nodes, audit_slack_runs;
    unsigned long long audit_used_nodes;
};

constexpr int FRAME_DOUBLES = 18;
constexpr int STASH_DOUBLES = 13;

struct DRowTab { uint32_t base, rem; };

constexpr uint32_t L0_REL_MAX_ACCELS = 16u;
struct DRelAccel {
    double o[3];
    uint32_t node_off;
    uint32_t node_n;
    uint32_t slot0;
    uint32_t slot_n;
};

struct DParams {
    const DNode *nodes;
    const DNode4 *nodes4;
    const uint32_t *primref;
    const DSphere *spheres;
    const int32_t *sphere_mat;
    const DCuboid *cuboids;
    const int32_t *cuboid_mat;
    const uint32_t *tri_v;
    const uint32_t *tri_n;
    const uint32_t *tri_t;
    const float *vpos;
    const float *vnorm;
    const float *vtex;
    const DLeafRec *leaf_soup;
    const DChunk *chunks;
    const DStrip *strips;
    const uint32_t *sphere_ref_leaf, *cuboid_ref_leaf, *tri_ref_leaf, *accel_ref_leaf;
    const DAccel *accels;
    const DMaterial *materials;
    const DLight *lights;
    uint32_t nlights;
    uint32_t recursion;
    int32_t default_material;
    uint32_t stack_depth;
    V3 cam_origin, cam_view, cam_up, cam_aux;
    double image_plane_height, pixel_separation, ss_distance;
    uint32_t ss_root;
    uint32_t boxes_finite;
    double ah_omax, ah_dmin, ah_dmax;
    V3 bg_inner, bg_outer;
    double bg_scale;
    V3 ambient;
    uint32_t w, h;
    double winv, hinv, aspect;
    uint32_t mode;
    uint32_t x0, y0, x1, y1;
    uint32_t tiles_x;
    uint32_t ilv_n, ilv_r, ilv_b;
    unsigned long long sub_k, sub_n, sub_count;
    uint32_t sub_m;
    uint32_t sub_cols;
    uint32_t sub_rows;
    uint32_t sub_kk, sub_kdiv;
    const DRowTab *sub_rowtab;
    uint32_t ntiles;
    uint32_t tile_rev;
    uint32_t out_row0;
    uint32_t out_x0;
    uint32_t out_pitch;
    uint32_t out_compact;
    const unsigned long long *pixel_list;
    uint8_t *out_rgba;
    double *out_radiance;
    uint32_t *tile_counter;
    double *frames;
    unsigned long long frame_threads;
    double *stash;
    DStats *stats;
    double *dbg_log;
    unsigned long long n_items;
    double *frame;
    uint32_t *vis;
    double *accum;
    uint32_t sample_index;
    uint32_t ss_par;
    uint32_t split_shift;
    uint32_t wf_level;
    uint32_t wf_levels;
    uint32_t tile0;
    uint32_t prune;
    uint32_t *wf_counts;
    unsigned long long wf_cap;
    unsigned long long wf_cap_next;
    unsigned long long wf_hit_cap;
    unsigned long long wf_hit_stride;
    double *wf_q;
    double *wf_out;
    double *wf_spec;
    uint32_t *wf_child;
    double *wf_q_next;
    double *wf_out_next;
    uint32_t *wf_hq;
    uint32_t *q_ctl;
    uint32_t *q_ready;
    uint32_t *q_err;
    uint32_t q_units, q_unit_tiles;
    uint32_t q_order, q_blocks_x, q_tiles_y, q_seq_len;
    double *q_rays[8];
    double *q_out[8];
    double *q_spec[8];
    uint32_t *q_child[8];
    const void *lds_image;
    uint32_t lds_image_n16;
    uint32_t mega_lanes;
    uint32_t lds_node_off;
    uint32_t lds_prim_off;
    uint32_t lds_soup_off;
    uint32_t lds_accel_off;
    const void *accel_image;
    uint32_t accel_image_n16;
    unsigned long long *stamp_counts;
    uint32_t stats_filter;
    uint32_t audit;
    uint32_t shadow_skip;
    uint32_t level_door;
    uint32_t l0_rel_n;
    DRelAccel l0_rel[L0_REL_MAX_ACCELS];
    uint32_t lds_pairs;
    struct { uint32_t root_off, pair_off, pair_n, pad; } pair_rel[L0_REL_MAX_ACCELS];
    uint32_t packet;
    uint32_t fused;
};
static_assert(sizeof(DParams) <= 4096, "DParams is passed by value: a kernel's arguments are at most 4 KB");
inline bool wf_takes_pairs(const DParams &P, bool fast) { return P.lds_image && P.lds_pairs && !fast && !P.prune; }

struct RadianceArgs {
    const double *rays;
    double *radiance;
    const uint32_t *perm;
    unsigned long long n;
    unsigned long long base;
};
struct FilmArgs : RadianceArgs {
    const unsigned long long *offsets;
    unsigned long long npix;
    uint32_t *rgba;
    double *rgb;
};

constexpr uint32_t MAX_LIGHT_GROUPS = 64u;
constexpr uint32_t GROUP_AMBIENT = 1u;
struct DLightGroup { uint32_t lights, flags; };
struct GroupArgs : RadianceArgs {
    double *xout, *xout_next;
    uint32_t n_groups, pad;
    DLightGroup groups[MAX_LIGHT_GROUPS];
};

struct ScatterArgs : RadianceArgs {
    void *hits;
    double *direct;
    uint32_t *flags;
    double *reflect;
    double *reflect_weight;
    double *refract;
    double *refract_weight;
    const uint32_t *tri_base;
};
constexpr uint32_t SCATTER_HIT = 1u, SCATTER_REFLECT = 2u, SCATTER_REFRACT = 4u;

constexpr uint32_t MAX_CALL_LIGHTS = 1024u;
struct LitArgs : ScatterArgs {
    const DLight *lights;
    double *terms;
    uint32_t *visible;
    uint32_t n_lights, per_ray, vis_words, skip;
    double ambient[3];
};

struct GatherArgs {
    const double *origins;
    const double *frames;
    const double *dirs;
    double *li;
    unsigned long long n_poses, n_dirs;
    unsigned long long base_tile;
    uint32_t tiles_per;
    uint32_t pose_lanes;
};

struct DView {
    V3 origin, view, up, aux;
    double image_plane_height, pixel_separation, ss_distance;
    uint32_t ss_root, pad;
};
struct ViewArgs {
    const DView *views;
    unsigned long long n_views;
    uint32_t w, h;
    uint32_t tiles_x;
    uint32_t tiles_per_view;
    unsigned long long base_tile;
    uint32_t *rgba;
    double *rgb;
};

struct DLens {
    int32_t kind, reserved;
    V3 origin, right, up, forward;
    double fov_deg;
};

}
```

lasgun_amd/csrc/internal.h:

```cpp
#pragma once
#include <hip/hip_runtime_api.h>

#include <algorithm>
#include <array>
#include <atomic>
#include <chrono>
#include <cstdio>
#include <cstdlib>
#include <cmath>
#include <cstring>
#include <functional>
#include <map>
#include <memory>
#include <mutex>
#include <set>
#include <string>
#include <thread>
#include <vector>

#include "../../include/lasgun_hip.h"
#include "host.h"
#include "raykey.h"
#include "tune.h"

namespace lg {
hipError_t launch_trace(const DParams &P, bool stats, bool fast, uint32_t blocks, uint32_t stack_depth, hipStream_t stream);
hipError_t trace_occupancy(uint32_t stack_depth, bool fast, size_t extra_lds, int *blocks_per_cu);
hipError_t launch_wf_trace(const DParams &P, bool fast, bool shadow, uint32_t blocks, uint32_t stack_depth, hipStream_t stream);
hipError_t launch_wf_shade(const DParams &P, uint32_t blocks, hipStream_t stream);
hipError_t launch_wf_combine(const DParams &P, uint32_t blocks, hipStream_t stream);
hipError_t launch_query(const DParams &P, const double *rays, unsigned long long n, void *hits, uint8_t *occluded, const uint32_t *tri_base,
                        const uint32_t *perm, bool fast, uint32_t blocks, uint32_t stack_depth, hipStream_t stream);
size_t sort_scratch_bytes(unsigned long long n);
hipError_t launch_query_order(const double *rays, unsigned long long n, const KeyBounds &B, void *scratch, uint32_t *keys_out, uint32_t *perm_out,
                              const uint32_t **perm, uint32_t grid_cap, hipStream_t stream);
hipError_t launch_camera_rays(const DParams &P, double *rays, unsigned long long n, uint32_t blocks, hipStream_t stream);
hipError_t query_occupancy(const DParams &P, bool fast, uint32_t stack_depth, int *blocks_per_cu);
hipError_t query_set_lds_limit(size_t bytes, bool ldss);
hipError_t launch_wf_resolve(const DParams &P, uint32_t blocks, hipStream_t stream);
hipError_t launch_rq_closest(const DParams &P, const RadianceArgs &Q, bool fast, uint32_t blocks, uint32_t stack_depth, hipStream_t stream);
hipError_t launch_rq_shade(const DParams &P, const RadianceArgs &Q, uint32_t blocks, hipStream_t stream);
hipError_t launch_rq_combine(const DParams &P, const RadianceArgs &Q, uint32_t blocks, hipStream_t stream);
hipError_t launch_rf_closest(const DParams &P, const FilmArgs &Q, bool fast, uint32_t blocks, uint32_t stack_depth, hipStream_t stream);
hipError_t launch_rf_shade(const DParams &P, const FilmArgs &Q, uint32_t blocks, hipStream_t stream);
hipError_t launch_rf_combine(const DParams &P, const FilmArgs &Q, uint32_t blocks, hipStream_t stream);
hipError_t launch_rf_resolve(const FilmArgs &Q, const double *li, unsigned long long slots, uint32_t samples, uint32_t blocks, hipStream_t stream);
hipError_t rq_set_lds_limit(size_t bytes, bool ldss);
hipError_t launch_scatter_closest(const DParams &P, const ScatterArgs &Q, bool fast, uint32_t blocks, uint32_t stack_depth, hipStream_t stream);
hipError_t launch_scatter_emit(const DParams &P, const ScatterArgs &Q, uint32_t blocks, hipStream_t stream);
hipError_t scatter_set_lds_limit(size_t bytes, bool ldss);
hipError_t launch_lit_closest(const DParams &P, const LitArgs &Q, bool fast, uint32_t blocks, uint32_t stack_depth, hipStream_t stream);
hipError_t launch_lit_shadow(const DParams &P, const LitArgs &Q, bool fast, uint32_t blocks, uint32_t stack_depth, hipStream_t stream);
hipError_t launch_lit_emit(const DParams &P, const LitArgs &Q, uint32_t blocks, hipStream_t stream);
hipError_t lit_set_lds_limit(size_t bytes, bool ldss);
hipError_t launch_lg_closest(const DParams &P, const GroupArgs &Q, bool fast, uint32_t blocks, uint32_t stack_depth, hipStream_t stream);
hipError_t launch_lg_shade(const DParams &P, const GroupArgs &Q, uint32_t blocks, hipStream_t stream);
hipError_t launch_lg_combine(const DParams &P, const GroupArgs &Q, uint32_t blocks, hipStream_t stream);
hipError_t launch_lg_spread(const DParams &P, const GroupArgs &Q, uint32_t blocks, hipStream_t stream);
hipError_t light_groups_set_lds_limit(size_t bytes, bool ldss);
hipError_t launch_gather_closest(const DParams &P, const GatherArgs &Q, bool fast, uint32_t blocks, uint32_t stack_depth, hipStream_t stream);
hipError_t launch_gather_shade(const DParams &P, const GatherArgs &Q, uint32_t blocks, hipStream_t stream);
hipError_t launch_gather_combine(const DParams &P, const GatherArgs &Q, uint32_t blocks, hipStream_t stream);
hipError_t launch_gather_resolve(const double *li, const double *weights, double *sums, unsigned long long n_poses, unsigned long long n_dirs, unsigned long long n_weights,
                                 uint32_t blocks, hipStream_t stream);
hipError_t gather_set_lds_limit(size_t bytes, bool ldss);
hipError_t launch_view_closest(const DParams &P, const ViewArgs &Q, bool fast, uint32_t blocks, uint32_t stack_depth, hipStream_t stream);
hipError_t launch_view_shade(const DParams &P, const ViewArgs &Q, uint32_t blocks, hipStream_t stream);
hipError_t launch_view_combine(const DParams &P, const ViewArgs &Q, uint32_t blocks, hipStream_t stream);
hipError_t launch_view_resolve(const DParams &P, const ViewArgs &Q, uint32_t blocks, hipStream_t stream);
hipError_t view_set_lds_limit(size_t bytes, bool ldss);
hipError_t launch_lens_rays(const DLens &L, uint32_t w, uint32_t h, uint32_t root, const unsigned long long *offsets, unsigned long long n, double *rays,
                            uint32_t blocks, hipStream_t stream);
hipError_t launch_visibility(const DParams &P, const double *from, unsigned long long n_from, const double *to, unsigned long long n_to, uint8_t *bits,
                             unsigned long long row_bytes, uint32_t *blocked, bool fast, uint32_t blocks, uint32_t stack_depth, hipStream_t stream);
hipError_t visibility_occupancy(const DParams &P, bool fast, uint32_t stack_depth, int *blocks_per_cu);
hipError_t visibility_set_lds_limit(size_t bytes, bool ldss);
hipError_t launch_open_directions(const DParams &P, const double *points, const double *normals, unsigned long long n_points, const double *dirs,
                                  unsigned long long n_dirs, uint8_t *bits, unsigned long long row_bytes, uint32_t *open, uint32_t *above, bool fast,
                                  uint32_t blocks, uint32_t stack_depth, hipStream_t stream);
hipError_t open_directions_occupancy(const DParams &P, bool fast, uint32_t stack_depth, int *blocks_per_cu);
hipError_t open_directions_set_lds_limit(size_t bytes, bool ldss);
hipError_t launch_range_scan(const DParams &P, const double *origins, const double *frames, unsigned long long n_poses, const double *beams,
                             unsigned long long n_beams, bool pose_lanes, float *range, float *point, float *normal, void *id, uint32_t *hits, uint32_t *nearest,
                             const uint32_t *tri_base, bool fast, uint32_t blocks, uint32_t stack_depth, hipStream_t stream);
hipError_t range_scan_occupancy(const DParams &P, bool fast, uint32_t stack_depth, int *blocks_per_cu);
hipError_t range_scan_set_lds_limit(size_t bytes, bool ldss);
hipError_t launch_hit_layers(const DParams &P, const double *rays, unsigned long long n, uint32_t max_layers, void *hits, double *along, void *id, uint32_t *count,
                             double *inside, const uint32_t *tri_base, const uint32_t *perm, bool fast, uint32_t blocks, uint32_t stack_depth, hipStream_t stream);
hipError_t hit_layers_occupancy(const DParams &P, bool fast, uint32_t stack_depth, int *blocks_per_cu);
hipError_t hit_layers_set_lds_limit(size_t bytes, bool ldss);
hipError_t launch_attributes(const DParams &P, const double *rays, unsigned long long n, void *hits, uint32_t *flags, double *bary, double *uv, double *local,
                             double *frame, double *dp, const uint32_t *tri_base, const uint32_t *perm, bool fast, uint32_t blocks, uint32_t stack_depth,
                             hipStream_t stream);
hipError_t launch_attr_of(const DParams &P, const double *rays, const void *records, unsigned long long n, const uint32_t *counts, uint32_t *flags, double *bary,
                          double *uv, double *local, double *frame, double *dp, uint32_t blocks, hipStream_t stream);
hipError_t attributes_occupancy(const DParams &P, bool fast, uint32_t stack_depth, int *blocks_per_cu);
hipError_t attributes_set_lds_limit(size_t bytes, bool ldss);
hipError_t launch_closest(const DParams &P, const double *points, unsigned long long n, double r2, double qmax, double *distance, double *point, void *id,
                          const uint32_t *tri_base, const void *cl, uint32_t *tile_counter, uint32_t blocks, uint32_t stack_depth, hipStream_t stream);
hipError_t closest_occupancy(uint32_t stack_depth, int *blocks_per_cu);
hipError_t closest_set_lds_limit(size_t bytes);
size_t closest_stack_bytes(uint32_t stack_depth);
struct ClosestTables;
hipError_t launch_trace_paths(const DParams &P, const double *rays, unsigned long long n, uint32_t max_bounces, const void *rules, uint32_t n_rules, bool use_ns,
                              const uint32_t *start_medium, void *hits, double *point, void *id, double *along, uint32_t *count, uint32_t *end, double *gain, double *last,
                              uint32_t *medium, const uint32_t *tri_base, const uint32_t *perm, bool fast, uint32_t blocks, uint32_t stack_depth, hipStream_t stream);
hipError_t trace_paths_occupancy(const DParams &P, bool fast, uint32_t stack_depth, int *blocks_per_cu);
hipError_t trace_paths_set_lds_limit(size_t bytes, bool ldss);
hipError_t launch_features(const DParams &P, float *depth, float *normal, float *albedo, float *coverage, void *id, const double *material_rgb, uint32_t nmat,
                           const uint32_t *tri_base, bool fast, uint32_t blocks, uint32_t stack_depth, hipStream_t stream);
hipError_t features_occupancy(const DParams &P, bool fast, uint32_t stack_depth, int *blocks_per_cu);
hipError_t features_set_lds_limit(size_t bytes, bool ldss);
hipError_t launch_view_features(const DParams &P, const ViewArgs &V, float *depth, float *normal, float *albedo, float *coverage, void *id, float *point,
// ... 200 lines not shown
    void give(size_t cap, void *q) {
        if (!q) return;
        {
            std::lock_guard<std::mutex> g(mtx);
            if (spare.size() < 64) { spare.emplace_back(cap, q); return; }
        }
        (void)hipHostFree(q);
    }
};
extern PinnedPool &g_pinned;
struct PinnedBuf {
    void *p = nullptr;
    size_t cap = 0;
    PinnedBuf() = default;
    PinnedBuf(const PinnedBuf &) = delete;
    PinnedBuf &operator=(const PinnedBuf &) = delete;
    void need(size_t bytes) { if (cap < bytes) { g_pinned.give(cap, p); p = nullptr; cap = 0; p = g_pinned.take(bytes, &cap); } }
    ~PinnedBuf() { g_pinned.give(cap, p); }
};


struct ErrWords {
    std::mutex mtx;
    std::vector<uint32_t *> pages;
    std::vector<uint32_t *> spare;
    uint32_t *take() {
        std::lock_guard<std::mutex> g(mtx);
        if (spare.empty()) {
            void *q = nullptr;
            hipError_t e = hipHostMalloc(&q, 4096, hipHostMallocPortable | hipHostMallocMapped);
            if (e != hipSuccess) throw Error(std::string("hipHostMalloc(error words): ") + hipGetErrorString(e));
            std::memset(q, 0, 4096);
            pages.push_back((uint32_t *)q);
            for (int i = 1023; i >= 0; --i) spare.push_back((uint32_t *)q + i);
        }
        uint32_t *w = spare.back();
        spare.pop_back();
        *(volatile uint32_t *)w = 0u;
        return w;
    }
    void give(uint32_t *w) {
        if (!w) return;
        std::lock_guard<std::mutex> g(mtx);
        spare.push_back(w);
    }
};
extern ErrWords &g_err_words;

struct lg_scene {
    Scene s;
};
struct lg_aggregate {
    Aggregate a;
};
struct lg_film {
    uint32_t w = 0, h = 0;
    std::vector<uint8_t> owned;
    uint8_t *px = nullptr;
};

struct lg_accel {
    const Scene *scene = nullptr;
    int device = 0;
    FlatScene flat;
    DevBuf<uint8_t> arena;
    DevBuf<DNode> nodes;
    DevBuf<DNode4> nodes4;
    DevBuf<uint32_t> primref;
    DevBuf<DSphere> spheres;
    DevBuf<int32_t> sphere_mat;
    DevBuf<DCuboid> cuboids;
    DevBuf<int32_t> cuboid_mat;
    DevBuf<uint32_t> tri_v, tri_n, tri_t;
    DevBuf<float> vpos, vnorm, vtex;
    DevBuf<DLeafRec> leaf_soup;
    DevBuf<DChunk> chunks;
    DevBuf<DStrip> strips;
    DevBuf<uint32_t> sphere_ref_leaf, cuboid_ref_leaf, tri_ref_leaf, accel_ref_leaf;
    DevBuf<DAccel> accels;
    DevBuf<DMaterial> materials;
    DevBuf<DLight> lights;
    DevBuf<uint32_t> accel_tri_base;
    DevBuf<uint32_t> attr_counts;
    mutable std::shared_ptr<ClosestTables> closest;
    mutable DevBuf<uint8_t> closest_cl;
    struct LaunchCtx {
        hipStream_t key = nullptr;
        unsigned long long last_use = 0;
        DevBuf<uint32_t> tile_counter;
        DevBuf<double> frames, stash;
        DevBuf<uint8_t> wf_mem;
        DevBuf<uint32_t> wf_counters;
        DevBuf<double> film_li;
        DevBuf<double> gather_li;
        DevBuf<uint8_t> sort_mem;
        struct RowTable { uint32_t w = 0, h = 0; unsigned long long n = 0, last_use = 0; DevBuf<DRowTab> buf; PinnedBuf stage; hipEvent_t up = nullptr; };
        std::vector<std::unique_ptr<RowTable>> rowtabs;
        unsigned long long rowtab_clock = 0;
        struct KsTable { DevBuf<unsigned long long> buf; PinnedBuf stage; hipEvent_t done = nullptr; };
        std::vector<std::unique_ptr<KsTable>> ks_live;
        ~LaunchCtx() {
            for (auto &k : ks_live) if (k->done) (void)hipEventDestroy(k->done);
            for (auto &r : rowtabs) if (r->up) (void)hipEventDestroy(r->up);
        }
    };
    mutable std::vector<std::unique_ptr<LaunchCtx>> ctxs;
    mutable std::vector<hipStream_t> aux_streams;
    mutable std::vector<hipEvent_t> aux_done;
    mutable hipEvent_t aux_fork = nullptr;
    mutable unsigned wf_split = 0;
    mutable unsigned long long ctx_clock = 0;
    mutable bool streaming = true;
    mutable bool streaming_forced = false;
    bool streaming_pays = false;
    unsigned long long streaming_min_items = 1ull << 20;
    unsigned long long specular_small_items = 1ull << 20;
    bool mega_narrow = false;
    uint32_t wf_blocks = 1, wf_blocks_fast = 1;
    uint32_t queue_blocks = 1;
    mutable uint32_t *q_err = nullptr;
    mutable int queue = -1;
    mutable int last_org = -1;
    mutable int tile_parts = -1;
    mutable int sample_order = -1;
    mutable int query_order = 0;
    mutable int tile_order = -1;
    bool queue_default = false;
    mutable size_t queue_budget = 0;
    unsigned long long queue_min_items = 1ull << 16;
    mutable size_t wf_budget = 0;
    DevBuf<uint32_t> lds_image;
    DevBuf<uint32_t> accel_image;
    uint32_t accel_image_n16 = 0;
    uint32_t lds_image_n16 = 0, lds_node_off = 0, lds_prim_off = 0, lds_soup_off = 0, lds_accel_off = 0;
    std::vector<DRelAccel> l0_rel;
    mutable bool l0_relative = true;
    mutable int last_l0_relative = -1;
    bool lds_pairs = false;
    int image_prune = -2;
    std::string pair_refusal;
    std::vector<std::array<uint32_t, 3>> pair_rel;
    mutable bool node_pairs = true;
    mutable int last_node_pairs = -1;
    mutable bool packet_walk = true;
    mutable int last_packet_walk = -1;
    mutable bool fused_shade = true;
    mutable int last_fused_shade = -1;
    mutable int packet_scene = -1;
    uint32_t ldss_blocks = 0;
    uint32_t cus = 1;
    mutable bool lds_scene = true;
    mutable DevBuf<DStats> stats;
    mutable DevBuf<uint8_t> staging;
    mutable DevBuf<double> staging_rad;
    mutable std::mutex mtx;
    hipStream_t stream = nullptr;
    uint32_t stack_depth = 1;
    uint32_t stack_depth_fast1 = 1;
    uint32_t max_blocks = 1;
    uint32_t max_blocks_fast = 1;
    uint64_t device_bytes = 0;
    mutable bool profiling = false;
    mutable bool fast = false;
    mutable int prune = -1;
    bool prune_default = false;
    mutable bool shadow_skip = true;
    mutable uint32_t level_door = 3u;
    bool fast_available = true;
    std::string fast_refusal = "fast mode unavailable: its tree is too deep for the LDS stack";
    mutable std::vector<std::pair<hipEvent_t, hipEvent_t>> events;
    mutable std::vector<std::pair<hipEvent_t, hipEvent_t>> kind_events[5];
    ~lg_accel() {
        for (auto &e : events) { (void)hipEventDestroy(e.first); (void)hipEventDestroy(e.second); }
        for (auto &v : kind_events) for (auto &e : v) { (void)hipEventDestroy(e.first); (void)hipEventDestroy(e.second); }
        for (auto e : aux_done) (void)hipEventDestroy(e);
        if (aux_fork) (void)hipEventDestroy(aux_fork);
        for (auto st : aux_streams) g_streams.give(device, st);
        g_streams.give(device, stream);
        g_err_words.give(q_err);
    }
};

inline bool prune_effective(const lg_accel &a) {
    const bool dflt = prune_env() < 0 ? a.prune_default : prune_env() != 0;
    return !a.fast && (a.prune < 0 ? dflt : a.prune != 0);
}
inline bool lds_resident(const lg_accel &a) { return !a.fast && a.lds_scene && a.ldss_blocks && !(a.lds_pairs && prune_effective(a)); }

constexpr size_t MAX_LAUNCH_CTXS = 8;
constexpr unsigned MAX_WF_BANDS = 4;
constexpr size_t PRUNE_MIN_TRIS = 4096;

lg_accel::LaunchCtx &ctx_for(const lg_accel &a, hipStream_t stream);
void check_queue_error(const lg_accel &a);
void sync_checked(const lg_accel &a);
DParams base_params(const lg_accel &a, uint32_t w, uint32_t h);
void set_lds_scene(const lg_accel &a, DParams &P);
bool scene_lds_image(const Scene &scene, bool pairs, std::vector<uint32_t> &img, uint32_t info[8]);
void ensure_aux_streams(const lg_accel &a, unsigned n);
void enqueue(const lg_accel &a, DParams &P, bool stats, hipStream_t stream);
void enqueue_radiance(const lg_accel &a, const double *rays, size_t n, double *radiance, const uint32_t *perm, lg_accel::LaunchCtx &c, hipStream_t stream);
void enqueue_radiance_groups(const lg_accel &a, const double *rays, size_t n, const DLightGroup *groups, uint32_t n_groups, double *radiance, const uint32_t *perm,
                             lg_accel::LaunchCtx &c, hipStream_t stream);
void enqueue_scatter(const lg_accel &a, const double *rays, size_t n, ScatterArgs Q, const uint32_t *perm, lg_accel::LaunchCtx &c, hipStream_t stream);
void enqueue_scatter_lit(const lg_accel &a, const double *rays, size_t n, LitArgs Q, const DLight *shared, const uint32_t *perm, lg_accel::LaunchCtx &c, hipStream_t stream);
void enqueue_ray_film(const lg_accel &a, const double *rays, size_t slots, uint32_t samples, const FilmArgs &film, const uint32_t *perm, lg_accel::LaunchCtx &c,
                      hipStream_t stream);
struct GatherCall {
    const double *origins, *frames, *dirs, *weights;
    size_t n_poses, n_dirs, n_weights;
    bool pose_lanes;
    double *radiance, *sums;
    size_t batch_poses;
};
void enqueue_radiance_gather(const lg_accel &a, const GatherCall &g, lg_accel::LaunchCtx &c, hipStream_t stream);
void enqueue_view_batch(const lg_accel &a, const DView *views, ViewArgs V, uint32_t samples_root, lg_accel::LaunchCtx &c, hipStream_t stream);
const DView *stage_view_table(const DView *views, size_t n_views, lg_accel::LaunchCtx &c, hipStream_t stream);
const void *stage_rule_table(const void *rules, size_t bytes, lg_accel::LaunchCtx &c, hipStream_t stream);
void set_rect(DParams &P, uint32_t x0, uint32_t y0, uint32_t x1, uint32_t y1);
unsigned long long subset_count(unsigned long long area, unsigned long long k, unsigned long long n);
void set_subset(const lg_accel &a, hipStream_t stream, DParams &P, size_t k, size_t n, uint32_t w, uint32_t h);
struct SubsetBatch {
    std::vector<unsigned long long> ks;
    unsigned long long n = 1, periods = 0, items = 0;
    bool whole = false;
};
SubsetBatch make_batch(const size_t *ks, size_t count, size_t n, uint32_t w, uint32_t h);
void set_subsets(const lg_accel &a, DParams &P, const SubsetBatch &b, hipStream_t stream);
void subsets_enqueued(const lg_accel &a, hipStream_t stream);
void subsets_abandoned(const lg_accel &a, hipStream_t stream);
struct CallScope {
    CallScope();
    ~CallScope();
};
template <class F> int guarded(F f) {
    try {
        CallScope call;
        f();
        return 0;
    } catch (const std::exception &e) {
        return fail(e.what());
    }
}

void rebuild_tables(const lg_accel *ca, bool fast);
lg_accel *accel_from_on(const lg_scene *s, int device);
```

lasgun_amd/csrc/k_wavefront.hip:

```cpp
#include <cstdlib>

#include "wflevel.h"
#include "packet.h"

namespace lg {


#ifndef LG_REFILL_MIN
#define LG_REFILL_MIN 16
#endif
struct ShadowRefill {
    static constexpr bool enabled = true;
    static constexpr unsigned long long NONE = ~0ull;
    const DParams &P;
    const HitSlots &hs;
    uint32_t band, left;
    uint32_t tile = NO_TILE, slot = 64u;
    bool exhausted = false;
    unsigned long long h = NONE;
    uint32_t light = 0u, vis = 0u;
    V3 hit_p{0.0, 0.0, 0.0};
    __device__ __forceinline__ ShadowRefill(const DParams &p, const HitSlots &s, uint32_t b) : P(p), hs(s), band(b), left(TILE_HEADS) {}
    __device__ __forceinline__ uint32_t threshold() const { return exhausted ? (P.nlights > 1u ? 1u : 65u) : (uint32_t)LG_REFILL_MIN; }
    __device__ __forceinline__ Ray shadow_ray() const {
// ... 135 lines not shown
    const uint32_t level = L0 ? 0u : P.wf_level;
    unsigned long long n_work = 0;
    HitSlots hs;
    uint32_t ntiles;
    const uint32_t lpt = L0 ? 64u : wf_lanes_per_tile(wf_level_rays(P, level));
    if (SHADOW) { hs = hit_slots(P, level, lpt); ntiles = hs.tiles; }
    else {
        n_work = L0 ? (unsigned long long)P.ntiles * 64ull : P.wf_counts[level];
        ntiles = L0 ? P.ntiles : (uint32_t)((n_work + lpt - 1u) / lpt);
    }
    if (ntiles == 0u) return;
    uint32_t *stack = lds_stack + (PACKET ? tid & ~63u : tid);
    constexpr uint32_t stride = LDSS ? LG_LDSS_BLOCK : LG_BLOCK;
    const uint4 *scn = nullptr;
    if (LDSS) {
        uint4 *dst = reinterpret_cast<uint4 *>(lds_stack + P.stack_depth * stride);
        const uint4 *src = reinterpret_cast<const uint4 *>(P.lds_image);
        copy_to_lds(dst, src, P.lds_image_n16, tid, stride);
        __syncthreads();
        if (REL) {
            l0_rewrite<PAIR>(P, dst, tid);
            __syncthreads();
        }
        scn = dst;
    }
    const uint4 *const arec = (LDSS || FAST) ? nullptr : load_accel_image(P, P.stack_depth * LG_BLOCK);
    Counters cnt = {0, 0, 0, 0, 0, 0, 0, 0, 0}; (void)cnt;
    if (!wave_has_work(ntiles)) return;
    if (REFILL) {
        ShadowRefill rf(P, hs, xcc_id());
        Best b;
        b.ref = NO_HIT; b.t = INFINITY; b.accel = 0u;
        Ray first = ray_new(V3{0.0, 0.0, 0.0}, V3{0.0, 0.0, 1.0});
        const bool live = rf.next(true, b, first);
        bool tie = false;
        traverse_ref<LDSS, false, PRUNE, false, ShadowRefill>(P, first, true, stack, stride, b, scn, tie, cnt, arec, &rf, live);
        rf.finish(b);
        return;
    }
    uint32_t band = LDSS ? xcc_id() : 0u, bands_left = TILE_HEADS;
    for (bool final = false; !final;) {
        uint32_t tile;
        if (LDSS) tile = claim_tile(P.tile_counter, ntiles, band, bands_left, final);
        else tile = claim_tile_single(P.tile_counter, ntiles, final);
        if (tile == NO_TILE) break;
        if (!SHADOW) {
            const unsigned long long i = (unsigned long long)tile * lpt + lane;
            Pixel px;
            px.active = false;
            Ray ray = ray_new(V3{0.0, 0.0, 0.0}, V3{0.0, 0.0, 1.0});
            if (L0) {
                uint32_t sample;
                const uint32_t ptile = l0_tile(P, tile, sample);
                px = pixel_of(P, P.tile0 + ptile, lane);
                if (px.active) ray = camera_ray(P, px.x, px.y, sample);
            } else if (lane < lpt && i < n_work) {
                px.active = true;
                ray = wf_load_ray(P, i);
            }
            const bool active = px.active;
            Best b;
            b.ref = NO_HIT; b.t = INFINITY; b.accel = 0u;
            if constexpr (PACKET) packet_walk<REL>(P, ray, active, stack, stride, b, scn);
            else if (active) {
                bool tie = false;
                walk<LDSS, FAST, PRUNE, false, REL, PAIR ? 1 : 0>(P, ray, false, stack, stride, b, scn, cnt, arec);
                (void)tie;
            }
            const bool hit = active && b.ref != NO_HIT;
            const unsigned long long mask = __builtin_amdgcn_ballot_w64(hit);
            const uint32_t nhit = (uint32_t)__builtin_popcountll(mask);
            unsigned long long h = i;
            const bool mine = L0 || lane < lpt;
            if (nhit * 64u < WF_FULL_MIN * lpt) {
                if (mine) P.wf_hq[i] = WF_NONE;
                if (nhit != 0u) {
                    uint32_t base_v = 0u;
                    if (lane == 0u) base_v = atomicAdd(P.wf_counts + P.wf_levels + level, nhit);
                    h = P.wf_hit_cap + (uint32_t)__builtin_amdgcn_readfirstlane((int)base_v) + lanes_below(mask);
                }
            } else if (!hit && mine) P.wf_hq[i] = WF_NONE;
            if (hit) {
                Shade sh;
                shade_frame(P, ray, b, sh);
                if constexpr (FUSED) fused_closest_hit(P, px, i, h, sh);
                else {
                    const bool skip = P.shadow_skip && shadow_skippable(P, sh);
                    P.wf_hq[h] = skip ? (uint32_t)i | WF_SKIP : (uint32_t)i;
                    if (skip) P.vis[h] = 0u;
                    const unsigned long long n = P.wf_hit_stride;
                    double *f = P.frame + h;
                    f[0 * n] = sh.praw.x; f[1 * n] = sh.praw.y; f[2 * n] = sh.praw.z;
                    f[3 * n] = sh.ng.x; f[4 * n] = sh.ng.y; f[5 * n] = sh.ng.z;
                    f[6 * n] = sh.ns.x; f[7 * n] = sh.ns.y; f[8 * n] = sh.ns.z;
                    f[9 * n] = sh.ss.x; f[10 * n] = sh.ss.y; f[11 * n] = sh.ss.z;
                    f[12 * n] = (double)sh.mat;
                }
            } else if (active) {
                const V3 value = background(P, normalize(ray.d));
                if (P.wf_levels == 1u) finish_pixel(P, px, i, value);
                else {
                    const unsigned long long n = P.wf_cap;
                    P.wf_out[i] = value.x; P.wf_out[n + i] = value.y; P.wf_out[2 * n + i] = value.z;
                    if (level + 1u < P.wf_levels) P.wf_child[i] = WF_MISS;
                }
            }
        } else {
            unsigned long long h;
            bool skip;
            if (!hit_of(P, hs, tile, lane, h, skip) || skip) continue;
            const unsigned long long n = P.wf_hit_stride;
            if constexpr (FUSED) {
                const V3 hit_p{P.frame[0 * n + h], P.frame[1 * n + h], P.frame[2 * n + h]};
                const DLight L = P.lights[0];
                Ray sray = ray_new(hit_p, V3{L.pos[0], L.pos[1], L.pos[2]} - hit_p);
                Best b;
                walk<LDSS, FAST, PRUNE, false, false, PAIR ? 1 : 0>(P, sray, true, stack, stride, b, scn, cnt, arec);
                fused_shadow_tail(P, h, !(b.t < 1.0));
            } else {
                V3 praw{P.frame[0 * n + h], P.frame[1 * n + h], P.frame[2 * n + h]};
                V3 ng{P.frame[3 * n + h], P.frame[4 * n + h], P.frame[5 * n + h]};
                const double err = 2.220446049250313e-16 * 65536.0;
                V3 hit_p = praw + ng * err;
                uint32_t vis = 0u;
                for (uint32_t l = 0; l < P.nlights; ++l) {
                    const DLight L = P.lights[l];
                    Ray sray = ray_new(hit_p, V3{L.pos[0], L.pos[1], L.pos[2]} - hit_p);
                    Best b;
                    bool tie = false;
                    walk<LDSS, FAST, PRUNE, false, false, PAIR ? 1 : 0>(P, sray, true, stack, stride, b, scn, cnt, arec);
                    (void)tie;
                    if (!(b.t < 1.0)) vis |= 1u << l;
                }
                P.vis[h] = vis;
            }
        }
    }
}

template <int KIND, bool L0>
__global__ void __launch_bounds__(LG_BLOCK, 3) wf_shade_kernel(const DParams P) {
    const uint32_t level = L0 ? 0u : P.wf_level;
    const HitSlots hs = hit_slots(P, level, 64u);
    const uint32_t wave = threadIdx.x >> 6, lane = threadIdx.x & 63u;
    const unsigned long long t_step = L0 ? ~0ull >> 1 : (unsigned long long)gridDim.x * (LG_BLOCK / 64u);
    for (unsigned long long t = (unsigned long long)blockIdx.x * (LG_BLOCK / 64u) + wave; t < hs.tiles; t += t_step) {
        unsigned long long h = 0;
        const bool valid = hit_of(P, hs, (uint32_t)t, lane, h);
        unsigned long long j = 0;
        Pixel px;
        px.active = false;
        bool has_r = false, has_t = false;
        Sample sr, st;
        Shade sh;
        V3 output = vzero();
        if (valid) {
            j = hq_ray(P.wf_hq[h]);
            Ray ray;
            if (L0) {
                uint32_t sample;
                const uint32_t ptile = l0_tile(P, (uint32_t)(j >> 6), sample);
                px = pixel_of(P, P.tile0 + ptile, (uint32_t)(j & 63u));
                ray = camera_ray(P, px.x, px.y, sample);
            } else ray = wf_load_ray(P, j);
            const unsigned long long n = P.wf_hit_stride;
            const double *f = P.frame + h;
            V3 p{f[0 * n], f[1 * n], f[2 * n]};
            sh.ng = V3{f[3 * n], f[4 * n], f[5 * n]};
            sh.ns = V3{f[6 * n], f[7 * n], f[8 * n]};
// ... 217 lines not shown
```

lasgun_amd/csrc/launch.cpp:

```cpp
#include "internal.h"
#include "choice.h"
#include "packet_host.h"
#include "fused_host.h"

lg_accel::LaunchCtx &ctx_for(const lg_accel &a, hipStream_t stream) {
    for (auto &c : a.ctxs)
        if (c->key == stream) { c->last_use = ++a.ctx_clock; return *c; }
    lg_accel::LaunchCtx *c = nullptr;
    if (a.ctxs.size() < MAX_LAUNCH_CTXS) {
        a.ctxs.emplace_back(new lg_accel::LaunchCtx());
        c = a.ctxs.back().get();
        c->tile_counter.alloc(TILE_COUNTER_WORDS);
        HIP_TRY(hipMemset(c->tile_counter.p, 0, TILE_COUNTER_WORDS * sizeof(uint32_t)));
    } else {
        c = a.ctxs[0].get();
        for (auto &x : a.ctxs) if (x->last_use < c->last_use) c = x.get();
        HIP_TRY(hipDeviceSynchronize());
    }
    c->key = stream;
    c->last_use = ++a.ctx_clock;
    return *c;
}

void check_queue_error(const lg_accel &a) {
    if (!a.q_err) return;
    volatile uint32_t *w = a.q_err;
    if (*w == 0u) return;
    *w = 0u;
    throw Error("queue organisation: a wave gave up waiting for work (scheduler stalled); the film is incomplete");
}
void sync_checked(const lg_accel &a) {
    HIP_TRY(hipStreamSynchronize(a.stream));
    check_queue_error(a);
}

DParams base_params(const lg_accel &a, uint32_t w, uint32_t h) {
    const Scene &s = *a.scene;
    DParams P{};
    P.nodes = a.nodes.p; P.nodes4 = a.nodes4.p; P.primref = a.primref.p; P.spheres = a.spheres.p; P.sphere_mat = a.sphere_mat.p;
    P.cuboids = a.cuboids.p; P.cuboid_mat = a.cuboid_mat.p; P.tri_v = a.tri_v.p; P.tri_n = a.tri_n.p; P.tri_t = a.tri_t.p;
    P.vpos = a.vpos.p; P.vnorm = a.vnorm.p; P.vtex = a.vtex.p; P.leaf_soup = a.leaf_soup.p; P.chunks = a.chunks.p; P.strips = a.strips.p; P.sphere_ref_leaf = a.sphere_ref_leaf.p; P.cuboid_ref_leaf = a.cuboid_ref_leaf.p;
    P.tri_ref_leaf = a.tri_ref_leaf.p; P.accel_ref_leaf = a.accel_ref_leaf.p; P.accels = a.accels.p; P.materials = a.materials.p;
    P.lights = a.lights.p;
    P.nlights = (uint32_t)a.flat.lights.size();
    P.recursion = s.recursion;
    P.default_material = a.flat.default_material;
    P.stack_depth = a.stack_depth;
    {
        static const bool accel_lds = env_on("LASGUN_ACCEL_LDS");
        P.accel_image = a.accel_image_n16 && accel_lds ? a.accel_image.p : nullptr; P.accel_image_n16 = a.accel_image_n16;
    }
    {
        P.prune = prune_effective(a) ? 1u : 0u;
    }
    {
        static const bool skip_env = env_on("LASGUN_SHADOW_SKIP");
        bool ok = skip_env && a.shadow_skip && !a.flat.lights.empty() && a.flat.lights.size() <= 32;
        for (const DLight &L : a.flat.lights)
            for (int k = 0; k < 3; ++k) ok = ok && std::isfinite(PI * L.intensity[k]);
        P.shadow_skip = ok ? 1u : 0u;
    }
    {
        static const uint32_t door_env = [] { const char *e = std::getenv("LASGUN_LEVEL_DOOR"); return e && e[0] >= '0' && e[0] <= '3' && !e[1] ? (uint32_t)(e[0] - '0') : 3u; }();
        P.level_door = door_env & a.level_door;
    }
    P.cam_origin = s.camera.origin; P.cam_view = s.camera.view; P.cam_up = s.camera.up; P.cam_aux = s.camera.aux;
    P.image_plane_height = s.camera.image_plane_height;
    P.pixel_separation = s.camera.pixel_separation;
    P.ss_distance = s.camera.ss_distance;
    P.ss_root = s.camera.ss_root;
    {
        static const bool signs = env_on("LASGUN_SLAB_SIGNS");
        P.boxes_finite = a.flat.boxes_finite && signs ? 1u : 0u;
    }
    P.ah_omax = a.flat.ah_omax; P.ah_dmin = a.flat.ah_dmin; P.ah_dmax = a.flat.ah_dmax;
    P.bg_inner = s.bg_inner; P.bg_outer = s.bg_outer; P.bg_scale = s.bg_scale;
    P.ambient = s.ambient;
    P.w = w; P.h = h;
    P.winv = 1. / (double)w; P.hinv = 1. / (double)h; P.aspect = (double)w / (double)h;
    return P;
}

void ensure_aux_streams(const lg_accel &a, unsigned n) {
    while (a.aux_streams.size() < n) {
        hipStream_t st = g_streams.take(a.device); hipEvent_t ev = nullptr;
        HIP_TRY(hipEventCreateWithFlags(&ev, hipEventDisableTiming));
// ... 122 lines not shown
    GroupArgs *lg = nullptr;
    const std::vector<double *> *xout = nullptr;
    bool own() const { return q != nullptr; }
    bool every_level() const { return lg != nullptr; }
    void level(uint32_t d) const {
        if (!lg) return;
        lg->xout = (*xout)[d];
        lg->xout_next = d + 1 < xout->size() ? (*xout)[d + 1] : nullptr;
    }
    hipError_t spread(const DParams &P, uint32_t blocks, hipStream_t s) const { return launch_lg_spread(P, *lg, blocks, s); }
    hipError_t closest(const DParams &P, bool fast, uint32_t blocks, uint32_t depth, hipStream_t s) const { return closest_(P, q, fast, blocks, depth, s); }
    hipError_t shadow(const DParams &P, bool fast, uint32_t blocks, uint32_t depth, hipStream_t s) const { return shadow_(P, q, fast, blocks, depth, s); }
    hipError_t shade(const DParams &P, uint32_t blocks, hipStream_t s) const { return shade_(P, q, blocks, s); }
    hipError_t combine(const DParams &P, uint32_t blocks, hipStream_t s) const { return combine_(P, q, blocks, s); }
    hipError_t resolve(const DParams &P, uint32_t blocks, hipStream_t s) const { return resolve_(P, q, blocks, s); }
};
template <class ARGS> using L0Closest = hipError_t (*)(const DParams &, const ARGS &, bool, uint32_t, uint32_t, hipStream_t);
template <class ARGS> using L0Flat = hipError_t (*)(const DParams &, const ARGS &, uint32_t, hipStream_t);
template <class ARGS, L0Closest<ARGS> F> static hipError_t l0_closest(const DParams &P, const void *q, bool fast, uint32_t blocks, uint32_t depth, hipStream_t s) {
    return F(P, *static_cast<const ARGS *>(q), fast, blocks, depth, s);
}
template <class ARGS, L0Flat<ARGS> F> static hipError_t l0_flat(const DParams &P, const void *q, uint32_t blocks, hipStream_t s) { return F(P, *static_cast<const ARGS *>(q), blocks, s); }
template <class ARGS, L0Closest<ARGS> CLOSEST, L0Flat<ARGS> SHADE, L0Flat<ARGS> COMBINE> static Level0 bind_level0(const ARGS &Q) {
    Level0 l0;
    l0.q = &Q;
    l0.closest_ = l0_closest<ARGS, CLOSEST>;
    l0.shade_ = l0_flat<ARGS, SHADE>;
    l0.combine_ = l0_flat<ARGS, COMBINE>;
    return l0;
}
static void combine_levels(const lg_accel &a, DParams &P, const LevelArrays &K, const ChunkPlan &plan, hipStream_t s, const Level0 &l0 = Level0()) {
    const unsigned long long n0 = plan.n0();
    const uint32_t flat_blocks0 = (uint32_t)(((unsigned long long)P.ntiles * 64ull + 255ull) / 256ull), flat_cap = a.cus * 16u;
    for (uint32_t d = plan.levels - 1; d-- > 0;) {
        P.wf_level = d;
        P.wf_cap = n0 << d; P.wf_cap_next = n0 << (d + 1);
        P.wf_out = K.out[d]; P.wf_spec = K.spec[d]; P.wf_child = K.child[d]; P.wf_out_next = K.out[d + 1];
        l0.level(d);
        if (l0.own() && (d == 0 || l0.every_level())) timed(a, 1, s, [&] { return l0.combine(P, d == 0 ? flat_blocks0 : flat_cap, s); });
        else timed(a, 1, s, [&] { return launch_wf_combine(P, d == 0 ? flat_blocks0 : flat_cap, s); });
    }
}
static void resolve_samples(const lg_accel &a, const DParams &P, uint32_t pixel_tiles, hipStream_t s) {
    DParams R = P;
    R.ntiles = pixel_tiles;
    timed(a, 1, s, [&] { return launch_wf_resolve(R, (uint32_t)(((unsigned long long)pixel_tiles * 64ull + 255ull) / 256ull), s); });
}

static bool l0_relative(const lg_accel &a, DParams &P) {
    static const bool env = env_on("LASGUN_L0_RELATIVE");
    P.l0_rel_n = 0u;
    if (!env || !a.l0_relative || a.fast || P.prune || !P.lds_image || !P.boxes_finite || P.wf_level != 0u) return false;
    if (a.l0_rel.empty() || a.l0_rel.size() != a.flat.accels.size() || a.l0_rel.size() > L0_REL_MAX_ACCELS) return false;
    if (!l0_relative_camera(P.cam_origin, P.cam_up, P.cam_aux, P.pixel_separation)) return false;
    std::vector<V3> local;
    if (!l0_relative_origins(a.flat, P.cam_origin, local)) return false;
    for (size_t i = 0; i < a.l0_rel.size(); ++i) {
        P.l0_rel[i] = a.l0_rel[i];
        P.l0_rel[i].o[0] = local[i].x; P.l0_rel[i].o[1] = local[i].y; P.l0_rel[i].o[2] = local[i].z;
    }
    P.l0_rel_n = (uint32_t)a.l0_rel.size();
    return true;
}

static uint32_t packet_walk(const lg_accel &a, const DParams &P, bool camera_level0) {
    static const bool env = env_on("LASGUN_PACKET_WALK");
    if (packet_launch_gate(wf_takes_pairs(P, a.fast), camera_level0, a.packet_walk && env) != PACKET_OK) return 0u;
    if (a.packet_scene < 0)
        a.packet_scene = (int)packet_scene_gate(a.flat.accels.data(), a.flat.accels.size(), a.flat.nodes.data(), a.flat.nodes.size(), a.flat.primref.data(),
                                                a.flat.primref.size(), a.stack_depth);
    return a.packet_scene == (int)PACKET_OK ? 1u : 0u;
}

static uint32_t fused_shade(const lg_accel &a, const DParams &P, bool camera_level0, uint32_t levels) {
    static const bool env = env_on("LASGUN_FUSED_SHADE");
    FusedAsk q;
    q.switched_on = a.fused_shade && env;
    q.camera_level0 = camera_level0;
    q.levels = levels;
    q.nlights = (unsigned long)P.nlights;
    q.packet_closest = P.packet != 0u;
    q.pair_shadow = wf_takes_pairs(P, a.fast);
    return fused_shade_gate(q) == FUSED_OK ? 1u : 0u;
}

struct WfChunk {
    const ChunkPlan &plan;
    uint32_t levels, nlaunch;
    static constexpr uint32_t CL = TILE_COUNTER_WORDS;
    LevelArrays L;
    uint32_t *hq = nullptr, *vis = nullptr, *counters = nullptr;
    double *frame = nullptr;
    uint32_t groups;
    std::vector<double *> xout;
    uint32_t vis_words;
    WfChunk(const ChunkPlan &p, uint32_t groups_ = 1, uint32_t vis_words_ = 1) : plan(p), levels(p.levels), nlaunch(4 * p.levels), groups(groups_), vis_words(vis_words_) {}
    static size_t extra_per_item(uint32_t levels, uint32_t groups = 1, uint32_t vis_words = 1) {
        return ((size_t)(4 + STASH_DOUBLES * 8 + 4 * (size_t)vis_words) << (levels - 1)) * 7 / 4 + (levels > 1 ? (size_t)3 * 8 * (groups - 1) * (((size_t)1 << levels) - 1) : 0);
    }
    size_t hit_cap() const { return (size_t)plan.n0() << (levels - 1); }
    size_t hit_len() const { return hit_cap() + hit_cap() / 64 * (WF_FULL_MIN_HOST - 1); }
    void carve(lg_accel::LaunchCtx &cx) {
        grow(cx.wf_mem, plan.need());
        grow(cx.wf_counters, CL * (1 + nlaunch));
        L = plan.carve(cx.wf_mem.p, [&](auto &take) {
            hq = (uint32_t *)take(hit_len() * 4);
            frame = (double *)take(hit_len() * STASH_DOUBLES * 8);
            vis = (uint32_t *)take(hit_len() * 4 * vis_words);
            xout.assign(levels, nullptr);
            for (uint32_t d = 0; levels > 1 && groups > 1 && d < levels; ++d) xout[d] = (double *)take(((size_t)plan.n0() << d) * 3 * 8 * (groups - 1));
        });
        counters = cx.wf_counters.p;
    }
    void params(const lg_accel &a, DParams &P) const {
        P.n_items = plan.n0();
        P.accum = L.accum;
        P.wf_levels = levels;
        P.wf_counts = counters;
        P.wf_hit_cap = hit_cap(); P.wf_hit_stride = hit_len(); P.wf_hq = hq; P.frame = frame; P.vis = vis;
        if (lds_resident(a)) set_lds_scene(a, P);
    }
    void run(const lg_accel &a, DParams &P, hipStream_t ls, const Level0 &l0 = Level0()) const {
        const bool ldss = P.lds_image != nullptr;
        const uint32_t depth = a.fast ? a.stack_depth_fast1 : a.stack_depth;
        const uint32_t trace_cap = ldss ? a.ldss_blocks : (a.fast ? a.wf_blocks_fast : a.wf_blocks), flat_cap = a.cus * 16u;
        const uint32_t trace_blocks0 = ldss ? trace_cap : std::min(trace_cap, (P.ntiles + 3u) / 4u);
        const uint32_t shade_blocks0 = (uint32_t)(((unsigned long long)P.ntiles + ((unsigned long long)P.ntiles * (WF_FULL_MIN_HOST - 1) + 63ull) / 64ull + 3ull) / 4ull);
        const unsigned long long n0 = plan.n0();
        HIP_TRY(hipMemsetAsync(counters, 0, CL * (1 + nlaunch) * sizeof(uint32_t), ls));
        uint32_t launch_no = 0;
        auto level_params = [&](uint32_t d) {
            P.wf_level = d;
            P.wf_cap = n0 << d; P.wf_cap_next = n0 << (d + 1);
            P.wf_q = L.q[d]; P.wf_out = L.out[d]; P.wf_spec = L.spec[d]; P.wf_child = L.child[d];
            P.wf_q_next = d + 1 < levels ? L.q[d + 1] : nullptr;
            P.wf_out_next = d + 1 < levels ? L.out[d + 1] : nullptr;
            P.tile_counter = counters + CL * (1 + launch_no++);
            l0.level(d);
        };
        for (uint32_t d = 0; d < levels; ++d) {
            const uint32_t tb = d == 0 ? trace_blocks0 : trace_cap, fb = d == 0 ? shade_blocks0 : flat_cap;
            const bool own0 = d == 0 && l0.own();
            level_params(d);
            P.packet = packet_walk(a, P, d == 0 && !own0);
            if (d == 0) a.last_packet_walk = (int)P.packet;
            P.fused = d == 0 ? fused_shade(a, P, !own0 && !l0.every_level(), levels) : 0u;
            if (d == 0) a.last_fused_shade = (int)P.fused;
            if (own0) timed(a, 0, ls, [&] { return l0.closest(P, a.fast, tb, depth, ls); });
            else {
                if (d == 0) a.last_l0_relative = l0_relative(a, P) ? 1 : 0;
                timed(a, 0, ls, [&] { return launch_wf_trace(P, a.fast, false, tb, depth, ls); });
                P.l0_rel_n = 0u;
            }
            if (own0 && l0.own_shadow) {
                if (l0.shadow_) {
                    if (((unsigned long long)P.ntiles * 7ull / 4ull + 1ull) * l0.vis_words > 0xFFFFFFFFull) throw Error("level 0's shadow pass: hit tiles x visibility words do not fit 32 bits");
                    const uint32_t sb = ldss ? trace_cap : (uint32_t)std::min<unsigned long long>(trace_cap, ((unsigned long long)P.ntiles * l0.vis_words + 3ull) / 4ull);
                    level_params(d);
                    timed(a, 2, ls, [&] { return l0.shadow(P, a.fast, sb, depth, ls); });
                }
            } else
            if (P.nlights > 0) {
                level_params(d);
                timed(a, 2, ls, [&] { return launch_wf_trace(P, a.fast, true, tb, depth, ls); });
            }
            level_params(d);
            if (l0.every_level() && d >= 1 && d + 1 == levels) timed(a, 1, ls, [&] { return l0.spread(P, flat_cap, ls); });
            if (own0 || l0.every_level()) timed(a, 3, ls, [&] { return l0.shade(P, fb, ls); });
            else if (!P.fused) timed(a, 3, ls, [&] { return launch_wf_shade(P, fb, ls); });
        }
        P.packet = 0u; P.fused = 0u;
        combine_levels(a, P, L, plan, ls, l0);
    }
};

static void enqueue_wavefront(const lg_accel &a, DParams &P0, lg_accel::LaunchCtx &c, hipStream_t stream) {
    const uint32_t levels = levels_of(a, P0);
    const uint32_t nsamples = P0.ss_root * P0.ss_root;
    const uint32_t S = nsamples > 1 && a.sample_order != 1 ? nsamples : 1u;
    ChunkPlan plan(a, P0, false, S, WfChunk::extra_per_item(levels));
    static const unsigned split_env = [] { const char *e = std::getenv("LASGUN_WF_SPLIT"); return e && std::atoi(e) > 0 ? (unsigned)std::atoi(e) : 1u; }();
    const unsigned want = a.wf_split ? a.wf_split : split_env;
    const unsigned split = (unsigned long long)P0.ntiles * 64ull >= (1ull << 21) ? std::min(want, MAX_WF_BANDS) : 1u;
    if (split > 1) plan.chunk_tiles = std::min<unsigned long long>(plan.chunk_tiles, (P0.ntiles + split - 1) / split);
    const unsigned long long nchunks = (P0.ntiles + plan.chunk_tiles - 1) / plan.chunk_tiles;
    const unsigned nstreams = split > 1 && nchunks > 1 ? (unsigned)std::min<unsigned long long>(split, nchunks) : 0u;
    if (nstreams) ensure_aux_streams(a, nstreams);
    std::vector<WfChunk> carved;
    std::vector<hipStream_t> lanes;
    plan.fit([&] {
        carved.clear(); lanes.clear();
        if (nstreams) for (unsigned j = 0; j < nstreams; ++j) { lanes.push_back(a.aux_streams[j]); carved.emplace_back(plan); carved.back().carve(ctx_for(a, a.aux_streams[j])); }
        else { lanes.push_back(stream); carved.emplace_back(plan); carved.back().carve(c); }
    });
    const unsigned long long chunk_tiles = plan.chunk_tiles;
    if (nstreams) {
        HIP_TRY(hipEventRecord(a.aux_fork, stream));
        for (unsigned j = 0; j < nstreams; ++j) HIP_TRY(hipStreamWaitEvent(a.aux_streams[j], a.aux_fork, 0));
    }

    const bool ldss = lds_resident(a);
    Span span(a, stream);
    if (std::getenv("LASGUN_DEBUG"))
        std::fprintf(stderr, "[lasgun] wavefront: levels %u, %llu tiles in chunks of %llu on %u stream(s) (%.1f MiB per context), trace grid %u x %u, stack %u, max_blocks %u\n", levels,
                     (unsigned long long)P0.ntiles, chunk_tiles, nstreams ? nstreams : 1u, plan.need() / 1048576.0, ldss ? a.ldss_blocks : (a.fast ? a.wf_blocks_fast : a.wf_blocks),
                     ldss ? 1024u : 256u, a.fast ? a.stack_depth_fast1 : a.stack_depth, a.max_blocks);
    unsigned long long chunk_no = 0;
    for (unsigned long long t0 = 0; t0 < P0.ntiles; t0 += chunk_tiles, ++chunk_no) {
        const WfChunk &K = carved[chunk_no % carved.size()];
        const hipStream_t ls = lanes[chunk_no % lanes.size()];
        DParams P = P0;
        P.tile0 = (uint32_t)t0;
        const uint32_t pixel_tiles = (uint32_t)std::min<unsigned long long>(chunk_tiles, P0.ntiles - t0);
        P.ntiles = pixel_tiles * S;
        P.ss_par = S;
        K.params(a, P);
#ifdef LG_STAMPS
        P.stats = a.stats.p;
        P.stamp_counts = reinterpret_cast<unsigned long long *>(a.stats.p + 1);
#endif
        for (uint32_t sidx = 0; sidx < nsamples / S; ++sidx) {
            P.sample_index = sidx;
            K.run(a, P, ls);
        }
        if (S > 1) resolve_samples(a, P, pixel_tiles, ls);
    }
    for (unsigned j = 0; j < nstreams; ++j) {
        HIP_TRY(hipEventRecord(a.aux_done[j], a.aux_streams[j]));
        HIP_TRY(hipStreamWaitEvent(stream, a.aux_done[j], 0));
    }
    span.end(a.events);
}

struct Level0Call {
    uint32_t tiles = 0;
// ... 570 lines not shown
```

lasgun_amd/csrc/shade.h:

```cpp
#pragma once
#include "walk.h"

namespace lg {
__device__ __forceinline__ double cos2_theta(V3 w) { return w.z * w.z; }
__device__ __forceinline__ double abs_cos_theta(V3 w) { return fabs(w.z); }
__device__ __forceinline__ double sin2_theta(V3 w) { return fmax_(1.0 - cos2_theta(w), 0.0); }
__device__ __forceinline__ double sin_theta(V3 w) { return sqrt(sin2_theta(w)); }
__device__ __forceinline__ double tan_theta(V3 w) { return sin_theta(w) / w.z; }
__device__ __forceinline__ double tan2_theta(V3 w) { return sin2_theta(w) / cos2_theta(w); }
__device__ __forceinline__ double cos_phi(V3 w) { double s = sin_theta(w); return s == 0.0 ? 1.0 : fmin_(fmax_(w.x / s, -1.0), 1.0); }
__device__ __forceinline__ double sin_phi(V3 w) { double s = sin_theta(w); return s == 0.0 ? 0.0 : fmin_(fmax_(w.y / s, -1.0), 1.0); }

__device__ __forceinline__ double fr_dielectric(double cos_i, double eta_i, double eta_t) {
    cos_i = fmin_(fmax_(cos_i, -1.0), 1.0);
    bool entering = cos_i > 0.0;
    if (!entering) { double tmp = eta_i; eta_i = eta_t; eta_t = tmp; cos_i = fabs(cos_i); }
    double sin_i = sqrt(fmax_(1.0 - cos_i * cos_i, 0.0));
    double sin_t = eta_i / eta_t * sin_i;
    if (sin_t >= 1.0) return 1.0;
    double cos_t = sqrt(fmax_(1.0 - sin_t * sin_t, 0.0));
    double r_parl = ((eta_t * cos_i) - (eta_i * cos_t)) / ((eta_t * cos_i) + (eta_i * cos_t));
    double r_perp = ((eta_i * cos_i) - (eta_t * cos_t)) / ((eta_i * cos_i) + (eta_t * cos_t));
    return (r_parl * r_parl + r_perp * r_perp) * 0.5;
}
// ... 181 lines not shown
    return (uint32_t)as_u8(round(fmin_(fmax_(c, 0.0), 1.0) * 255.0));
}
__device__ __forceinline__ V3 background(const DParams &P, V3 d) {
    double a = fabs(dot(V3{0.0, 0.0, 1.0}, d));
    double t = fmin_(sqrt(1.0 - a * a) / P.bg_scale, 1.0);
    return V3{lerp(t, P.bg_inner.x, P.bg_outer.x), lerp(t, P.bg_inner.y, P.bg_outer.y), lerp(t, P.bg_inner.z, P.bg_outer.z)};
}

enum { FR_ACC = 0, FR_SPEC_R = 3, FR_STATE = 6, FR_TO = 7, FR_TD = 10, FR_SPEC_T = 13, FR_A = 16, FR_PDF = 17 };
__device__ __forceinline__ double &frame_at(const DParams &P, uint32_t depth, int field, unsigned long long gtid) {
    return P.frames[((unsigned long long)depth * FRAME_DOUBLES + field) * P.frame_threads + gtid];
}
__device__ __forceinline__ void frame_put3(const DParams &P, uint32_t depth, int field, unsigned long long g, V3 v) {
    frame_at(P, depth, field, g) = v.x; frame_at(P, depth, field + 1, g) = v.y; frame_at(P, depth, field + 2, g) = v.z;
}
__device__ __forceinline__ V3 frame_get3(const DParams &P, uint32_t depth, int field, unsigned long long g) {
    return V3{frame_at(P, depth, field, g), frame_at(P, depth, field + 1, g), frame_at(P, depth, field + 2, g)};
}

struct Pixel {
    uint32_t x, y;
    unsigned long long pix;
    bool active;
};
__device__ __forceinline__ Pixel pixel_of(const DParams &P, uint32_t tile, uint32_t lane) {
    Pixel px;
    if (P.mode == 0) {
        uint32_t tx = tile % P.tiles_x, ty = tile / P.tiles_x;
        px.x = P.x0 + tx * 8u + (lane & 7u);
        const uint32_t vy = P.y0 + ty * 8u + (lane >> 3);
        px.active = px.x < P.x1 && vy < P.y1;
        px.y = P.ilv_n > 1u ? ((vy / P.ilv_b) * P.ilv_n + P.ilv_r) * P.ilv_b + vy % P.ilv_b : vy;
        px.pix = (unsigned long long)(vy - P.out_row0) * P.out_pitch + (px.x - P.out_x0);
    } else if (P.mode == 4 || P.mode == 5) {
        const uint32_t ty = tile / P.sub_cols, c = tile - ty * P.sub_cols;
        uint32_t r = lane, j = 0u, kk = P.sub_kk, kdiv = P.sub_kdiv;
        if (P.mode == 5) {
            r = lane / P.sub_m; j = lane - r * P.sub_m;
            const unsigned long long kd = P.pixel_list[P.sub_m + j];
            kk = (uint32_t)kd; kdiv = (uint32_t)(kd >> 32);
        }
        const uint32_t y = ty * P.sub_rows + r;
        const bool in = r < P.sub_rows && y < P.h;
        const DRowTab rt = P.sub_rowtab[in ? y : 0u];
        int32_t ph = (int32_t)kk - (int32_t)rt.rem;
        const uint32_t wrapped = ph < 0 ? 1u : 0u;
        if (wrapped) ph += (int32_t)P.sub_n;
        const uint32_t x = (uint32_t)ph + (uint32_t)P.sub_n * c;
        const long long q = (long long)rt.base + (long long)c + (long long)wrapped - (long long)kdiv;
        px.active = in && x < P.w && q >= 0;
        px.x = px.active ? x : 0u;
        px.y = px.active ? y : 0u;
        const unsigned long long place = P.mode == 5 ? (unsigned long long)q * P.sub_m + j : (unsigned long long)q;
        px.pix = px.active ? (P.out_compact ? place : (unsigned long long)y * P.w + x) : 0ull;
    } else {
        unsigned long long i = (unsigned long long)tile * 64ull + lane;
        px.active = i < P.sub_count;
        unsigned long long off;
        if (P.mode == 1) off = P.sub_k + i * P.sub_n;
        else if (P.mode == 3) {
            const uint32_t q = (uint32_t)i / P.sub_m, j = (uint32_t)i - q * P.sub_m;
            off = P.pixel_list[j] + (unsigned long long)q * P.sub_n;
            px.active = px.active && off < (unsigned long long)P.w * P.h;
            if (!px.active) off = 0ull;
        } else off = px.active ? P.pixel_list[i] : 0ull;
        px.x = (uint32_t)(off % P.w);
        px.y = (uint32_t)(off / P.w);
        px.pix = P.out_compact ? i : off;
    }
    return px;
}

extern __shared__ __attribute__((aligned(16))) uint32_t lds_stack[];

__device__ __forceinline__ const uint4 *load_accel_image(const DParams &P, uint32_t stack_words) {
    if (!P.accel_image) return nullptr;
    uint4 *dst = reinterpret_cast<uint4 *>(lds_stack + stack_words);
    const uint4 *src = reinterpret_cast<const uint4 *>(P.accel_image);
    copy_to_lds(dst, src, P.accel_image_n16, threadIdx.x, blockDim.x);
    __syncthreads();
    return dst;
}

__device__ __forceinline__ void shade_frame(const DParams &P, const Ray &ray, const Best &best, Shade &sh) {
    Isect is;
    sh.mat = resolve_hit(P, ray, best, is);
    sh.wo = -normalize(ray.d);
    sh.ng = face_forward(normalize(cross(is.gu, is.gv)), sh.wo);
    sh.ns = is.has_n ? normalize(is.n) : normalize(cross(is.su, is.sv));
    const double err = 2.220446049250313e-16 * 65536.0;
    V3 p = ray.o + ray.d * is.t;
    V3 p_err = sh.ng * err;
    sh.praw = p;
    sh.p = p + p_err;
    sh.pm = p - p_err;
    sh.ss = normalize(is.su);
    sh.ts = cross(sh.ns, sh.ss);
}

__device__ __forceinline__ void stash_put(const DParams &P, unsigned long long g, const Shade &sh) {
    const unsigned long long n = P.frame_threads;
    V3 p = sh.praw;
    double *s = P.stash + g;
    s[0 * n] = p.x; s[1 * n] = p.y; s[2 * n] = p.z;
    s[3 * n] = sh.ng.x; s[4 * n] = sh.ng.y; s[5 * n] = sh.ng.z;
    s[6 * n] = sh.ns.x; s[7 * n] = sh.ns.y; s[8 * n] = sh.ns.z;
    s[9 * n] = sh.ss.x; s[10 * n] = sh.ss.y; s[11 * n] = sh.ss.z;
    s[12 * n] = (double)sh.mat;
}
__device__ __forceinline__ void stash_get(const DParams &P, unsigned long long g, Shade &sh, const Ray &ray) {
    const unsigned long long n = P.frame_threads;
    const double *s = P.stash + g;
    V3 p{s[0 * n], s[1 * n], s[2 * n]};
    sh.ng = V3{s[3 * n], s[4 * n], s[5 * n]};
    sh.ns = V3{s[6 * n], s[7 * n], s[8 * n]};
    sh.ss = V3{s[9 * n], s[10 * n], s[11 * n]};
    sh.mat = (int32_t)s[12 * n];
    sh.wo = -normalize(ray.d);
    const double err = 2.220446049250313e-16 * 65536.0;
    V3 p_err = sh.ng * err;
    sh.praw = p;
    sh.p = p + p_err;
    sh.pm = p - p_err;
    sh.ts = cross(sh.ns, sh.ss);
}

__device__ __forceinline__ uint32_t tile_in_order(const DParams &P, uint32_t s) {
    if (P.tile_rev == 0u) return s;
    if (P.tile_rev == 1u) return P.ntiles - 1u - s;
    const uint32_t mid = P.ntiles >> 1;
    return (s & 1u) ? mid - 1u - (s >> 1) : mid + (s >> 1);
}
__device__ __forceinline__ uint32_t l0_tile(const DParams &P, uint32_t vt, uint32_t &sample) {
    if (P.ss_par <= 1u) { sample = P.sample_index; return vt; }
    const uint32_t t = vt / P.ss_par;
    sample = vt - t * P.ss_par;
    return t;
}
__device__ __forceinline__ void write_pixel(const DParams &P, const Pixel &px, V3 color) {
    const unsigned long long pix = px.pix;
    if (P.out_rgba) {
        uint32_t rgba = to_byte(color.x) | (to_byte(color.y) << 8) | (to_byte(color.z) << 16) | (255u << 24);
        reinterpret_cast<uint32_t *>(P.out_rgba)[pix] = rgba;
    }
    if (P.out_radiance) {
        P.out_radiance[3 * pix] = color.x; P.out_radiance[3 * pix + 1] = color.y; P.out_radiance[3 * pix + 2] = color.z;
    }
}
__device__ __forceinline__ void finish_pixel(const DParams &P, const Pixel &px, unsigned long long widx, V3 value) {
    const uint32_t nsamples = P.ss_root * P.ss_root;
    if (P.ss_par > 1u) {
        P.accum[widx] = value.x; P.accum[P.n_items + widx] = value.y; P.accum[2 * P.n_items + widx] = value.z;
        return;
    }
    V3 color = vzero();
    if (P.sample_index > 0) color = V3{P.accum[widx], P.accum[P.n_items + widx], P.accum[2 * P.n_items + widx]};
    color = color + value;
    if (P.sample_index + 1 < nsamples) {
        P.accum[widx] = color.x; P.accum[P.n_items + widx] = color.y; P.accum[2 * P.n_items + widx] = color.z;
        return;
    }
    const double weight = 1. / (double)nsamples;
    color = color * weight;
    write_pixel(P, px, color);
}
struct LightTerm {
    V3 wi;
    double f_att, wi_dot_n;
    bool reflect;
};
__device__ __forceinline__ LightTerm light_term(const DLight &L, const Shade &sh) {
    LightTerm t;
    V3 wi = V3{L.pos[0], L.pos[1], L.pos[2]} - sh.p;
    double d = magnitude(wi);
    t.f_att = L.falloff[0] + L.falloff[1] * d + L.falloff[2] * d * d;
    t.wi = normalize(wi);
    t.wi_dot_n = dot(t.wi, sh.ns);
    t.reflect = bsdf_reflect(sh, sh.wo, t.wi);
    return t;
}
// ... 50 lines not shown
```

lasgun_amd/csrc/walk.h:

```cpp
#pragma once
#include "kcommon.h"

namespace lg {

__device__ __forceinline__ bool slab_intersects(const double bmin[3], const double bmax[3], const Ray &r) {
    double t1 = (bmin[0] - r.o.x) * r.dinv.x, t2 = (bmax[0] - r.o.x) * r.dinv.x;
    double tnear = fmax_(-INFINITY, fmin_(t1, t2));
    double tfar = fmin_(INFINITY, fmax_(t1, t2));
    t1 = (bmin[1] - r.o.y) * r.dinv.y; t2 = (bmax[1] - r.o.y) * r.dinv.y;
    tnear = fmax_(tnear, fmin_(t1, t2));
    tfar = fmin_(tfar, fmax_(t1, t2));
    t1 = (bmin[2] - r.o.z) * r.dinv.z; t2 = (bmax[2] - r.o.z) * r.dinv.z;
    tnear = fmax_(tnear, fmin_(t1, t2));
    tfar = fmin_(tfar, fmax_(t1, t2));
    return tnear <= tfar && tfar > 0.0;
}

__device__ __forceinline__ bool slab_intersects_nc(const double bmin[3], const double bmax[3], const Ray &r) {
    double t1 = (bmin[0] - r.o.x) * r.dinv.x, t2 = (bmax[0] - r.o.x) * r.dinv.x;
    double tnear = fmin_(t1, t2), tfar = fmax_(t1, t2);
    t1 = (bmin[1] - r.o.y) * r.dinv.y; t2 = (bmax[1] - r.o.y) * r.dinv.y;
    tnear = fmax_(tnear, fmin_(t1, t2));
    tfar = fmin_(tfar, fmax_(t1, t2));
    t1 = (bmin[2] - r.o.z) * r.dinv.z; t2 = (bmax[2] - r.o.z) * r.dinv.z;
// ... 159 lines not shown
    h.b0 = e0 * invdet; h.b1 = e1 * invdet; h.b2 = e2 * invdet;
    h.t = tscaled * invdet;
    return true;
}

struct TriSetup {
    int kz;
    double sx, sy, sz;
};
__device__ __forceinline__ TriSetup tri_setup(const Ray &ray) {
    TriSetup s;
    s.kz = max_dimension(vabs(ray.d));
    int kx = s.kz + 1; if (kx == 3) kx = 0;
    int ky = kx + 1; if (ky == 3) ky = 0;
    double dx = comp(ray.d, kx), dy = comp(ray.d, ky), dz = comp(ray.d, s.kz);
    s.sx = -dx / dz; s.sy = -dy / dz;
    s.sz = comp(ray.dinv, s.kz);
    return s;
}
template <int KZ> __device__ __forceinline__ V3 permute_kz(V3 v) {
    if (KZ == 0) return V3{v.y, v.z, v.x};
    if (KZ == 1) return V3{v.z, v.x, v.y};
    return v;
}
template <int KZ>
__device__ __forceinline__ bool triangle_t_pre(V3 p0, V3 p1, V3 p2, V3 o, double sx, double sy, double sz, TriHit &h) {
    V3 p0t = permute_kz<KZ>(p0 - o), p1t = permute_kz<KZ>(p1 - o), p2t = permute_kz<KZ>(p2 - o);
    p0t.x += sx * p0t.z; p0t.y += sy * p0t.z;
    p1t.x += sx * p1t.z; p1t.y += sy * p1t.z;
    p2t.x += sx * p2t.z; p2t.y += sy * p2t.z;
    double e0 = p1t.x * p2t.y - p1t.y * p2t.x;
    double e1 = p2t.x * p0t.y - p2t.y * p0t.x;
    double e2 = p0t.x * p1t.y - p0t.y * p1t.x;
    if ((e0 < 0.0 || e1 < 0.0 || e2 < 0.0) && (e0 > 0.0 || e1 > 0.0 || e2 > 0.0)) return false;
    double det = e0 + e1 + e2;
    if (det == 0.0) return false;
    p0t.z *= sz; p1t.z *= sz; p2t.z *= sz;
    double tscaled = e0 * p0t.z + e1 * p1t.z + e2 * p2t.z;
    if ((det < 0.0 && tscaled >= 0.0) || (det > 0.0 && tscaled <= 0.0)) return false;
    double invdet = 1.0 / det;
    h.b0 = e0 * invdet; h.b1 = e1 * invdet; h.b2 = e2 * invdet;
    h.t = tscaled * invdet;
    return true;
}

__device__ __forceinline__ V3 load_f3(const float *base, uint32_t idx) {
    const float *p = base + 3ull * idx;
    return V3{(double)p[0], (double)p[1], (double)p[2]};
}

struct Isect {
    double t;
    V3 gu, gv;
    V3 su, sv;
    V3 n;
    bool has_n;
};
__device__ __forceinline__ void isect_set(Isect &i, double t, V3 dpdu, V3 dpdv) {
    i.t = t; i.gu = dpdu; i.gv = dpdv; i.su = dpdu; i.sv = dpdv; i.has_n = false; i.n = vzero();
}

__device__ __forceinline__ void sphere_full(const DSphere &s, const Ray &ray, double t, bool inside, Isect &is) {
    V3 cen{s.cx, s.cy, s.cz};
    V3 p = ray.o + ray.d * t - cen;
    if (p.x == 0.0 && p.y == 0.0) p.x = 1e-5 * s.r;
    double phi = p_atan2(p.y, p.x);
    if (phi < 0.0) phi += 2.0 * PI;
    double theta = p_acos(fmin_(fmax_(p.z / s.r, -1.0), 1.0));
    V3 dpdu{-2.0 * PI * p.y, 2.0 * PI * p.x, 0.0};
    double sin_phi, cos_phi;
    double sin_theta = 0.0;
    sin_phi = 0.0; cos_phi = 0.0;
#pragma clang loop unroll(disable)
    for (int i = 0; i < 2; ++i) {
        double sn, cs;
        p_sincos(i == 0 ? phi : theta, sn, cs);
        if (i == 0) { sin_phi = sn; cos_phi = cs; } else sin_theta = sn;
    }
    V3 dpdv = PI * V3{p.z * cos_phi, p.z * sin_phi, -s.r * sin_theta};
    if (inside) isect_set(is, t, dpdu, dpdv);
    else isect_set(is, t, dpdv, dpdu);
}

__device__ __forceinline__ void triangle_full(const DParams &P, uint32_t tri, uint32_t aflags, const Ray &ray, Isect &is) {
    const uint32_t *vi = P.tri_v + 3ull * tri;
    V3 p0 = load_f3(P.vpos, vi[0]), p1 = load_f3(P.vpos, vi[1]), p2 = load_f3(P.vpos, vi[2]);
    TriHit h;
    triangle_t(p0, p1, p2, ray, h);
    double uv[3][2];
    if (aflags & AF_HAS_UV) {
        const uint32_t *ti = P.tri_t + 3ull * tri;
#pragma unroll
        for (int k = 0; k < 3; ++k) { uv[k][0] = (double)P.vtex[2ull * ti[k]]; uv[k][1] = (double)P.vtex[2ull * ti[k] + 1]; }
    } else {
        uv[0][0] = 0.0; uv[0][1] = 0.0; uv[1][0] = 1.0; uv[1][1] = 0.0; uv[2][0] = 1.0; uv[2][1] = 1.0;
    }
    double duv02x = uv[0][0] - uv[2][0], duv02y = uv[0][1] - uv[2][1];
    double duv12x = uv[1][0] - uv[2][0], duv12y = uv[1][1] - uv[2][1];
    V3 dp02 = p0 - p2, dp12 = p1 - p2;
    double determinant = (duv02x * duv12y) - (duv02y * duv12x);
    V3 dpdu, dpdv;
    if (determinant == 0.0) {
        coordinate_system(cross(p2 - p1, p1 - p0), dpdu, dpdv);
    } else {
        double inv = 1.0 / determinant;
        dpdu = (duv12y * dp02 - duv02y * dp12) * inv;
        dpdv = (-duv12x * dp02 - duv02x * dp12) * inv;
    }
    isect_set(is, h.t, dpdu, dpdv);
    if (aflags & AF_HAS_N) {
        const uint32_t *ni = P.tri_n + 3ull * tri;
        V3 n0 = load_f3(P.vnorm, ni[0]), n1 = load_f3(P.vnorm, ni[1]), n2 = load_f3(P.vnorm, ni[2]);
        V3 ns = h.b0 * n0 + h.b1 * n1 + h.b2 * n2;
        V3 ss = is.gu;
        V3 ts = cross(ns, ss);
        if (magnitude2(ts) > 0.0) ss = cross(ts, ns);
        else coordinate_system(ns, ss, ts);
        is.has_n = true; is.n = ns;
        is.su = ss; is.sv = ts;
    } else {
        is.has_n = true;
        is.n = face_forward(cross(dp02, dp12), -ray.d);
    }
}

__device__ __forceinline__ void dbg_event(const DParams &P, double code, double a, double b, double c) {
    if (!P.dbg_log) return;
    const uint32_t n = (uint32_t)P.dbg_log[0];
    if (n >= 4000u) return;
    double *e = P.dbg_log + 1 + 4 * (size_t)n;
    e[0] = code; e[1] = a; e[2] = b; e[3] = c;
    P.dbg_log[0] = (double)(n + 1u);
}
struct Counters {
    uint32_t primary, shadow, secondary, nodes, spheres, cuboids, triangles, entries, hits;
    uint32_t a_nodes = 0u, a_runs = 0u, a_prims = 0u, a_viol = 0u;
    double a_slack_n = INFINITY, a_slack_r = INFINITY;
    double a_used_n = 0.0;
};

__device__ __forceinline__ Affine load_affine(const Affine *p) { return *p; }

__device__ __forceinline__ Ray local_ray(const DParams &P, const Ray &wray, uint32_t accel) {
    const DAccel *a = P.accels + accel;
    uint32_t n = a->nchain;
    Ray r = wray;
    for (uint32_t i = 0; i < n; ++i) r = ray_to_local(P.accels[a->chain[i]].minv, r);
    return r;
}

typedef uint32_t lg_u32x4 __attribute__((ext_vector_type(4)));
typedef const __attribute__((address_space(4))) lg_u32x4 *lg_const_u4;
__device__ __forceinline__ uint4 load_const_u4(lg_const_u4 q, int i) {
    const lg_u32x4 v = q[i];
    return uint4{v.x, v.y, v.z, v.w};
}
typedef const __attribute__((address_space(3))) lg_u32x4 *lg_lds_u4;
typedef double lg_f64x2 __attribute__((ext_vector_type(2)));
typedef const __attribute__((address_space(3))) lg_f64x2 *lg_lds_d2;
typedef const __attribute__((address_space(3))) uint32_t *lg_lds_u32;
__device__ __forceinline__ uint4 lds_u4(const uint4 *p) {
    const lg_u32x4 v = *(lg_lds_u4)p;
    return uint4{v.x, v.y, v.z, v.w};
}
__device__ __forceinline__ double2 lds_d2(const void *p) {
    const lg_f64x2 v = *(lg_lds_d2)p;
    return double2{v.x, v.y};
}
struct NodeRec {
    double bmin[3], bmax[3];
    uint32_t link, meta, parent, pad;
};
__device__ __forceinline__ double u2d(uint32_t lo, uint32_t hi) { return __hiloint2double((int)hi, (int)lo); }
template <bool LDSS>
__device__ __forceinline__ NodeRec load_node(const DParams &P, const uint4 *scn, uint32_t idx) {
    NodeRec n;
    if (LDSS) {
        static_assert(LDS_NODE_STRIDE == 5u, "idx * 5 below is written as a shift and an add");
        const uint4 *q4 = scn + (P.lds_node_off + ((idx << 2) + idx));
        const double2 *q = reinterpret_cast<const double2 *>(q4);
        const double2 a = q[0], b = q[1], c = q[2];
        const uint2 d = *reinterpret_cast<const uint2 *>(q4 + 3);
        n.bmin[0] = a.x; n.bmin[1] = a.y; n.bmin[2] = b.x;
        n.bmax[0] = b.y; n.bmax[1] = c.x; n.bmax[2] = c.y;
        n.link = d.x; n.meta = d.y; n.parent = 0u; n.pad = 0u;
    } else {
        const DNode *nd = P.nodes + idx;
        n.bmin[0] = nd->bmin[0]; n.bmin[1] = nd->bmin[1]; n.bmin[2] = nd->bmin[2];
        n.bmax[0] = nd->bmax[0]; n.bmax[1] = nd->bmax[1]; n.bmax[2] = nd->bmax[2];
        n.link = nd->link; n.meta = nd->meta; n.parent = nd->parent; n.pad = nd->pad;
    }
    return n;
}
__device__ __forceinline__ NodeRec load_node_uniform(const DParams &P, uint32_t idx) {
    lg_const_u4 q = (lg_const_u4)(uintptr_t)(P.nodes + idx);
    const uint4 a = load_const_u4(q, 0), b = load_const_u4(q, 1), c = load_const_u4(q, 2), d = load_const_u4(q, 3);
    NodeRec n;
    n.bmin[0] = u2d(a.x, a.y); n.bmin[1] = u2d(a.z, a.w); n.bmin[2] = u2d(b.x, b.y);
    n.bmax[0] = u2d(b.z, b.w); n.bmax[1] = u2d(c.x, c.y); n.bmax[2] = u2d(c.z, c.w);
    n.link = d.x; n.meta = d.y; n.parent = d.z; n.pad = d.w;
    return n;
}
template <bool LDSS>
__device__ __forceinline__ uint32_t load_primref(const DParams &P, const uint4 *scn, uint32_t i) {
    if (LDSS) return reinterpret_cast<const uint32_t *>(scn + P.lds_prim_off)[i];
// ... 1101 lines not shown
            }
            if (FAST && (L.flags & AF_MESH)) tri = tri_setup(ray);
            fast_level_root<COUNT>(P, L, ray, limit, state, cur, li, le, cnt);
        }
        while (state == ST_LEVEL_DONE) {
            if (L.accel == 0u) state = ST_DONE;
            else {
                const uint32_t w2 = stk[(sp - 1u) * stride];
                le = stk[(sp - 2u) * stride]; li = stk[(sp - 3u) * stride];
                sp -= 3u; base = w2 & ~FRAME_SAME_RAY;
                if (COUNT) dbg_event(P, 5.0, (double)L.accel, (double)li, (double)le);
                uint32_t parent, nchain;
                const uint32_t *chain;
                if (LDSS) {
                    const uint4 *rec = scn + (P.lds_accel_off + L.accel * LDS_ACCEL_UNITS);
                    parent = rec[7].x;
                    const uint4 *prec = scn + (P.lds_accel_off + parent * LDS_ACCEL_UNITS);
                    nchain = prec[7].y; chain = reinterpret_cast<const uint32_t *>(prec + 8);
                } else {
                    parent = (uint32_t)P.accels[L.accel].parent;
                    nchain = P.accels[parent].nchain; chain = P.accels[parent].chain;
                }
                lvl_set<LDSS, FAST>(P, scn, L, parent);
                if (!(w2 & FRAME_SAME_RAY)) {
                    ray = root;
                    for (uint32_t i = 1; i < nchain; ++i) {
                        const uint32_t c = chain[i];
                        const uint32_t cflags = LDSS ? scn[P.lds_accel_off + c * LDS_ACCEL_UNITS + 6u].w : P.accels[c].flags;
                        if (!((cflags & AF_IDENTITY) && ray_plain(ray))) ray = accel_local_ray<LDSS>(P, scn, c, ray);
                    }
                    dd = dot(ray.d, ray.d);
                    four_a = 4.0 * dd;
                    negmask = neg_mask(ray);
                }
                if (li < le) state = ST_LEAF;
                else if (sp != base) { --sp; take(stk[sp * stride]); }
                else state = ST_LEVEL_DONE;
            }
        }
        if (!wave_any(state != ST_DONE)) break;
    }
}


template <bool LDSS, bool FAST, bool PRUNE = false, bool COUNT = false, bool REL = false, int PAIRSEL = 2>
__device__ __forceinline__ void walk(const DParams &P, const Ray &ray, const bool anyhit, uint32_t *stack, const uint32_t stride, Best &best,
                                     const uint4 *scn, Counters &cnt, const uint4 *arec = nullptr) {
    bool tie = false;
    if (FAST && !anyhit_exit_ok(P, ray)) {
        traverse_ref<false, false, false, COUNT>(P, ray, anyhit, stack, stride, best, nullptr, tie, cnt, arec);
        return;
    }
    if (FAST) traverse_fast<COUNT>(P, ray, anyhit, stack, stride, best, scn, tie, cnt);
    else
    if (LDSS && !FAST && !PRUNE && !COUNT && PAIRSEL != 0) {
        constexpr bool CAN = LDSS && !FAST && !PRUNE && !COUNT;
        if (PAIRSEL == 1 || P.lds_pairs != 0u) traverse_ref<LDSS, FAST, PRUNE, COUNT, NoRefill, REL, CAN>(P, ray, anyhit, stack, stride, best, scn, tie, cnt, arec);
        else traverse_ref<LDSS, FAST, PRUNE, COUNT, NoRefill, REL>(P, ray, anyhit, stack, stride, best, scn, tie, cnt, arec);
    } else
    traverse_ref<LDSS, FAST, PRUNE, COUNT, NoRefill, REL>(P, ray, anyhit, stack, stride, best, scn, tie, cnt, arec);
    if (!FAST) return;
    if (COUNT) dbg_event(P, 9.0, tie ? 1.0 : 0.0, best.t, (double)best.ref);
    bool redo;
    if (anyhit && !(best.t < 1.0)) redo = tie;
    else {
        redo = anyhit ? false : tie;
        if (!redo && best.ref != NO_HIT) redo = !ref_candidate(P, ray, best);
    }
    if (COUNT && redo) cnt.a_runs++;
    if (redo) traverse_ref<false, false, false, COUNT>(P, ray, anyhit, stack, stride, best, nullptr, tie, cnt, arec);
}
__device__ __forceinline__ void audit_fast_ray(const DParams &P, const Ray &ray, const bool anyhit, uint32_t *stack, const uint32_t stride, const Best &got,
                                               Counters &cnt, const uint4 *arec) {
    Best want;
    bool tie = false;
    Counters unused = {0, 0, 0, 0, 0, 0, 0, 0, 0};
    traverse_ref<false, false, false, false>(P, ray, anyhit, stack, stride, want, nullptr, tie, unused, arec);
    cnt.a_prims++;
    const bool same = anyhit ? ((got.t < 1.0) == (want.t < 1.0))
                             : (got.ref == want.ref && (got.ref == NO_HIT || (got.accel == want.accel && __double_as_longlong(got.t) == __double_as_longlong(want.t))));
    if (!same) cnt.a_viol++;
}

__device__ __forceinline__ int32_t resolve_hit(const DParams &P, const Ray &wray, const Best &best, Isect &is) {
    Ray lr = local_ray(P, wray, best.accel);
    uint32_t kind = best.ref >> 30, idx = best.ref & PRIM_INDEX_MASK;
    int32_t prim_mat = -1;
    if (kind == PK_SPHERE) {
        DSphere s = P.spheres[idx];
        bool inside;
        double t = sphere_t(lr, V3{s.cx, s.cy, s.cz}, s.r, inside);
        sphere_full(s, lr, t, inside, is);
        prim_mat = P.sphere_mat[idx];
    } else if (kind == PK_CUBOID) {
        DCuboid c = P.cuboids[idx];
        double t; V3 d0, d1;
        cuboid_hit<true>(c.mn, c.mx, lr, t, d0, d1);
        isect_set(is, t, d0, d1);
        is.has_n = true;
        is.n = face_forward(cross(d0, d1), -lr.d);
        prim_mat = P.cuboid_mat[idx];
    } else {
        triangle_full(P, idx, P.accels[best.accel].flags, lr, is);
    }
    int32_t isect_mat = P.default_material;
    int32_t a = (int32_t)best.accel;
    while (a >= 0) {
        const DAccel *A = P.accels + a;
        V3 gu = xf_vector(A->m, is.gu), gv = xf_vector(A->m, is.gv);
        if (vne(is.gu, is.su) || vne(is.gv, is.sv)) {
            is.su = xf_vector(A->m, is.su); is.sv = xf_vector(A->m, is.sv);
        } else {
            is.su = gu; is.sv = gv;
        }
        is.gu = gu; is.gv = gv;
        if (is.has_n) is.n = xf_normal(A->minv, is.n);
        if (A->material >= 0) isect_mat = A->material;
        if (A->flags & AF_SWAP_BACKFACE) {
            V3 tmp = is.gu; is.gu = is.gv; is.gv = tmp;
            tmp = is.su; is.su = is.sv; is.sv = tmp;
            if (is.has_n) is.n = -is.n;
        }
        a = A->parent;
    }
    return prim_mat >= 0 ? prim_mat : isect_mat;
}


}
```

Before: 6012 Mrays/s.

## Precompute per-triangle shading frames for small meshes and use them in fused shading

At build time a new kernel precomputes a record for each triangle of small meshes without vertex normals, capped per instance and in total. The record holds the face normal, both flip variants of the shading axes, and the resolved material. In the fused closest-hit path, when a ballot shows every lane in the wavefront hit such a triangle, shading reads the record instead of recomputing the UV partials and walking the transform chain. This trades recomputation for an extra 176-byte table read per hit. It also adds a new public API, a host-side planner, and an env/flag gate that decides whether the path runs.

```diff
diff --git a/bindings/rust/lasgun-hip-sys/src/lib.rs b/bindings/rust/lasgun-hip-sys/src/lib.rs
--- a/bindings/rust/lasgun-hip-sys/src/lib.rs
+++ b/bindings/rust/lasgun-hip-sys/src/lib.rs
@@ -356,6 +356,10 @@
     pub fn lg_accel_set_fused_shade(a0: *const lg_accel, enabled: c_int) -> c_int;
     pub fn lg_accel_last_fused_shade(a0: *const lg_accel) -> c_int;
     pub fn lg_scene_fused_shade_gate(a0: *const lg_scene, camera_level0: c_int) -> c_int;
+    pub fn lg_accel_set_tri_frames(a0: *const lg_accel, enabled: c_int) -> c_int;
+    pub fn lg_accel_last_tri_frames(a0: *const lg_accel) -> c_int;
+    pub fn lg_scene_tri_frames_gate(a0: *const lg_scene, base: *mut u32, cap: c_int) -> c_int;
+    pub fn lg_accel_read_tri_frames(a0: *const lg_accel, records: *mut c_void, cap: c_int) -> c_int;
     pub fn lg_scene_lds_image(a0: *const lg_scene, pairs: c_int, words: *mut u32, cap: usize, info: *mut u32) -> i64;
     pub fn lg_accel_get_prune(a0: *const lg_accel) -> c_int;
     pub fn lg_accel_set_streaming(a0: *const lg_accel, enabled: c_int) -> c_int;
diff --git a/include/lasgun_hip.h b/include/lasgun_hip.h
--- a/include/lasgun_hip.h
+++ b/include/lasgun_hip.h
@@ -141,6 +141,10 @@
 int lg_accel_set_fused_shade(const lg_accel *, int enabled);
 int lg_accel_last_fused_shade(const lg_accel *);
 int lg_scene_fused_shade_gate(const lg_scene *, int camera_level0);
+int lg_accel_set_tri_frames(const lg_accel *, int enabled);
+int lg_accel_last_tri_frames(const lg_accel *);
+int lg_scene_tri_frames_gate(const lg_scene *, uint32_t *base, int cap);
+int lg_accel_read_tri_frames(const lg_accel *, void *records, int cap);
 int64_t lg_scene_lds_image(const lg_scene *, int pairs, uint32_t *words, size_t cap, uint32_t *info);
 int lg_accel_get_prune(const lg_accel *);
 
diff --git a/lasgun_amd/__init__.py b/lasgun_amd/__init__.py
--- a/lasgun_amd/__init__.py
+++ b/lasgun_amd/__init__.py
@@ -44,6 +44,10 @@
     "accel_set_fused_shade": (_C.c_int, [_C.c_void_p, _C.c_int]),
     "accel_last_fused_shade": (_C.c_int, [_C.c_void_p]),
     "scene_fused_shade_gate": (_C.c_int, [_C.c_void_p, _C.c_int]),
+    "accel_set_tri_frames": (_C.c_int, [_C.c_void_p, _C.c_int]),
+    "accel_last_tri_frames": (_C.c_int, [_C.c_void_p]),
+    "scene_tri_frames_gate": (_C.c_int, [_C.c_void_p, _C.POINTER(_C.c_uint32), _C.c_int]),
+    "accel_read_tri_frames": (_C.c_int, [_C.c_void_p, _C.c_void_p, _C.c_int]),
     "scene_lds_image": (_C.c_longlong, [_C.c_void_p, _C.c_int, _C.POINTER(_C.c_uint32), _C.c_size_t, _C.POINTER(_C.c_uint32)]),
     "accel_set_streaming": (_C.c_int, [_C.c_void_p, _C.c_int]),
     "accel_get_prune": (_C.c_int, [_C.c_void_p]),
@@ -119,6 +123,8 @@
 
 HIT_DTYPE = _np.dtype(Hit)
 assert _C.sizeof(Hit) == 96 and HIT_DTYPE.itemsize == 96, "lg_hit is 96 bytes"
+TRI_FRAME_DTYPE = _np.dtype([("c", "<f8", (3,)), ("ng0", "<f8", (3,)), ("ss", "<f8", (3,)), ("ns", "<f8", (2, 3)), ("ts", "<f8", (2, 3)), ("mat", "<i4"), ("pad", "<u4")])
+assert TRI_FRAME_DTYPE.itemsize == 176, "a frame record is 176 bytes"
 LENS_EQUIRECTANGULAR, LENS_FISHEYE = 0, 1
 assert _C.sizeof(CLens) == 112, "lg_lens is 112 bytes"
 assert _C.sizeof(CFeatures) == 40, "lg_features is 40 bytes"
@@ -303,6 +309,30 @@
             raise LasgunError(self.last_error())
         return int(v)
 
+    def set_tri_frames(self, accel, enabled):
+        if self.call("accel_set_tri_frames", accel.h, 1 if enabled else 0):
+            raise LasgunError(self.last_error())
+
+    def last_tri_frames(self, accel):
+        v = self.call("accel_last_tri_frames", accel.h)
+        return None if v < 0 else bool(v)
+
+    def read_tri_frames(self, accel):
+        n = self.call("accel_read_tri_frames", accel.h, None, 0)
+        if n < 0:
+            raise LasgunError(self.last_error())
+        rows = _np.zeros(n, dtype=TRI_FRAME_DTYPE)
+        if n and self.call("accel_read_tri_frames", accel.h, rows.ctypes.data, n) != n:
+            raise LasgunError(self.last_error())
+        return rows
+
+    def scene_tri_frames_gate(self, scene, cap=4096):
+        base = (_C.c_uint32 * cap)(*([0xFFFFFFFE] * cap))
+        v = self.call("scene_tri_frames_gate", scene.h, base, cap)
+        if v < 0:
+            raise LasgunError(self.last_error())
+        return int(v), [None if b == 0xFFFFFFFF else int(b) for b in base if b != 0xFFFFFFFE]
+
     def last_organisation(self, accel):
         v = self.call("accel_last_organisation", accel.h)
         name = {0: "megakernel", 1: "wavefront", 2: "queue"}.get(v & 15) if v >= 0 else None
diff --git a/lasgun_amd/csrc/accel.cpp b/lasgun_amd/csrc/accel.cpp
--- a/lasgun_amd/csrc/accel.cpp
+++ b/lasgun_amd/csrc/accel.cpp
@@ -1,6 +1,7 @@
 #include "internal.h"
 #include "attributes_host.h"
 #include "pairs_host.h"
+#include "tri_frames_host.h"
 
 static std::vector<uint32_t> attr_counts_of(const FlatScene &f, const Scene &scene) {
     std::vector<uint32_t> faces(f.accels.size(), 0u), tri_base(f.accels.size(), 0u), sphere_accel(f.spheres.size(), NO_HIT), cuboid_accel(f.cuboids.size(), NO_HIT);
@@ -29,6 +30,22 @@
         }
     }
     return attr_counts_build(faces, tri_base, sphere_accel, cuboid_accel);
+}
+
+static std::vector<TriFramesAccel> tri_frames_accels(const FlatScene &f, const Scene &scene) {
+    std::vector<TriFramesAccel> t(f.accels.size());
+    for (size_t id = 0; id < f.accels.size(); ++id) {
+        t[id] = TriFramesAccel{f.accels[id].flags, id < f.accel_tri_base.size() ? f.accel_tri_base[id] : 0u, 0u};
+        const int64_t obj = id < f.accel_obj.size() ? f.accel_obj[id] : -1;
+        if ((f.accels[id].flags & AF_MESH) && obj >= 0 && (size_t)obj < scene.meshes.size() && scene.meshes[(size_t)obj])
+            t[id].faces = (uint32_t)std::min<size_t>(scene.meshes[(size_t)obj]->tri.size() / 3, 0xFFFFFFFFu);
+    }
+    return t;
+}
+uint32_t scene_tri_frames(const FlatScene &f, const Scene &scene, std::vector<uint32_t> &base) {
+    const std::vector<TriFramesAccel> t = tri_frames_accels(f, scene);
+    base.assign(t.size(), NO_HIT);
+    return tri_frames_plan(t.data(), t.size(), f.tri_v.size() / 3, base.data());
 }
 
 static void set_lds_limits(size_t bytes, bool ldss) {
@@ -319,7 +336,24 @@
         }
         stage.add(a->accel_tri_base, f.accel_tri_base);
         stage.add(a->attr_counts, attr_counts_of(a->flat, *a->scene));
+        std::vector<uint32_t> tf_base;
+        a->tri_frame_records = scene_tri_frames(a->flat, *a->scene, tf_base);
+        {
+            std::vector<DTriFrameJob> jobs(a->tri_frame_records);
+            const std::vector<TriFramesAccel> ta = tri_frames_accels(a->flat, *a->scene);
+            if (a->tri_frame_records && !tri_frames_jobs(ta.data(), ta.size(), a->flat.tri_v.size() / 3, tf_base.data(), a->tri_frame_records, jobs.data()))
+                throw Error("frame table: the plan does not add up");
+            stage.add(a->tri_frame_base, tf_base); stage.add(a->tri_frame_jobs, jobs);
+            stage.add(a->tri_frames, std::vector<DTriFrame>(a->tri_frame_records));
+        }
         stage.commit(a->arena);
+        if (a->tri_frame_records) {
+            DParams T{};
+            T.accels = a->accels.p; T.tri_v = a->tri_v.p; T.tri_t = a->tri_t.p; T.vpos = a->vpos.p; T.vtex = a->vtex.p;
+            T.default_material = a->flat.default_material;
+            HIP_TRY(launch_tri_frames(T, a->tri_frame_jobs.p, a->tri_frame_records, a->tri_frames.p, a->stream));
+            HIP_TRY(hipStreamSynchronize(a->stream));
+        }
         {
             size_t big_mesh = 0;
             for (const auto &m : a->scene->meshes) if (m && m->tri.size() / 3 > big_mesh) big_mesh = m->tri.size() / 3;
@@ -353,6 +387,7 @@
     swap(x.vpos, y.vpos); swap(x.vnorm, y.vnorm); swap(x.vtex, y.vtex); swap(x.leaf_soup, y.leaf_soup); swap(x.chunks, y.chunks); swap(x.strips, y.strips);
     swap(x.sphere_ref_leaf, y.sphere_ref_leaf); swap(x.cuboid_ref_leaf, y.cuboid_ref_leaf); swap(x.tri_ref_leaf, y.tri_ref_leaf); swap(x.accel_ref_leaf, y.accel_ref_leaf);
     swap(x.accels, y.accels); swap(x.materials, y.materials); swap(x.lights, y.lights); swap(x.accel_tri_base, y.accel_tri_base); swap(x.attr_counts, y.attr_counts);
+    swap(x.tri_frames, y.tri_frames); swap(x.tri_frame_jobs, y.tri_frame_jobs); swap(x.tri_frame_base, y.tri_frame_base); swap(x.tri_frame_records, y.tri_frame_records);
     swap(x.lds_image, y.lds_image); swap(x.accel_image, y.accel_image); swap(x.accel_image_n16, y.accel_image_n16);
     swap(x.lds_image_n16, y.lds_image_n16); swap(x.lds_node_off, y.lds_node_off); swap(x.lds_prim_off, y.lds_prim_off);
     swap(x.lds_soup_off, y.lds_soup_off); swap(x.lds_accel_off, y.lds_accel_off);
diff --git a/lasgun_amd/csrc/capi.cpp b/lasgun_amd/csrc/capi.cpp
--- a/lasgun_amd/csrc/capi.cpp
+++ b/lasgun_amd/csrc/capi.cpp
@@ -795,6 +795,42 @@
     });
     return rc ? -1 : v;
 }
+int lg_accel_set_tri_frames(const lg_accel *a, int enabled) {
+    if (enabled != 0 && enabled != 1) return fail("tri frames must be 0 or 1");
+    std::lock_guard<std::mutex> g(a->mtx);
+    a->tri_frames_on = enabled == 1;
+    return 0;
+}
+int lg_accel_last_tri_frames(const lg_accel *a) {
+    std::lock_guard<std::mutex> g(a->mtx);
+    return a->last_tri_frames;
+}
+int lg_accel_read_tri_frames(const lg_accel *a, void *records, int cap) {
+    int v = 0;
+    int rc = guarded([&] {
+        if (!a) throw Error("accel is NULL");
+        std::lock_guard<std::mutex> g(a->mtx);
+        v = (int)a->tri_frame_records;
+        const size_t n = std::min<size_t>(a->tri_frame_records, cap > 0 ? (size_t)cap : 0u);
+        if (records && n) {
+            use_device(a->device);
+            HIP_TRY(hipMemcpy(records, a->tri_frames.p, n * sizeof(DTriFrame), hipMemcpyDeviceToHost));
+        }
+    });
+    return rc ? -1 : v;
+}
+int lg_scene_tri_frames_gate(const lg_scene *s, uint32_t *base, int cap) {
+    int v = 0;
+    int rc = guarded([&] {
+        if (!s) throw Error("scene is NULL");
+        FlatScene f;
+        flatten_scene(s->s, f, false, false);
+        std::vector<uint32_t> b;
+        v = (int)scene_tri_frames(f, s->s, b);
+        for (int i = 0; base && i < cap && (size_t)i < b.size(); ++i) base[i] = b[(size_t)i];
+    });
+    return rc ? -1 : v;
+}
 int lg_accel_set_mode(const lg_accel *a, int mode) {
     if (mode != 0 && mode != 1) return fail("mode must be 0 (reference traversal) or 1 (fast)");
     std::lock_guard<std::mutex> g(a->mtx);
diff --git a/lasgun_amd/csrc/dscene.h b/lasgun_amd/csrc/dscene.h
--- a/lasgun_amd/csrc/dscene.h
+++ b/lasgun_amd/csrc/dscene.h
@@ -139,6 +139,15 @@
     uint32_t slot0;
     uint32_t slot_n;
 };
+
+struct DTriFrame {
+    double c[3], ng0[3], ss[3];
+    double ns[2][3], ts[2][3];
+    int32_t mat;
+    uint32_t pad;
+};
+static_assert(sizeof(DTriFrame) == 176, "DTriFrame is 21 doubles and a word (tri_frames_host.h, TRI_FRAME_BYTES)");
+struct DTriFrameJob { uint32_t accel, tri; };
 
 struct DParams {
     const DNode *nodes;
@@ -252,6 +261,9 @@
     struct { uint32_t root_off, pair_off, pair_n, pad; } pair_rel[L0_REL_MAX_ACCELS];
     uint32_t packet;
     uint32_t fused;
+    const DTriFrame *tri_frames;
+    const uint32_t *tri_frame_base;
+    const uint32_t *tri_base;
 };
 static_assert(sizeof(DParams) <= 4096, "DParams is passed by value: a kernel's arguments are at most 4 KB");
 inline bool wf_takes_pairs(const DParams &P, bool fast) { return P.lds_image && P.lds_pairs && !fast && !P.prune; }
diff --git a/lasgun_amd/csrc/internal.h b/lasgun_amd/csrc/internal.h
--- a/lasgun_amd/csrc/internal.h
+++ b/lasgun_amd/csrc/internal.h
@@ -29,6 +29,7 @@
 hipError_t launch_wf_trace(const DParams &P, bool fast, bool shadow, uint32_t blocks, uint32_t stack_depth, hipStream_t stream);
 hipError_t launch_wf_shade(const DParams &P, uint32_t blocks, hipStream_t stream);
 hipError_t launch_wf_combine(const DParams &P, uint32_t blocks, hipStream_t stream);
+hipError_t launch_tri_frames(const DParams &P, const DTriFrameJob *jobs, uint32_t n, DTriFrame *out, hipStream_t stream);
 hipError_t launch_query(const DParams &P, const double *rays, unsigned long long n, void *hits, uint8_t *occluded, const uint32_t *tri_base,
                         const uint32_t *perm, bool fast, uint32_t blocks, uint32_t stack_depth, hipStream_t stream);
 size_t sort_scratch_bytes(unsigned long long n);
@@ -395,6 +396,10 @@
     DevBuf<DLight> lights;
     DevBuf<uint32_t> accel_tri_base;
     DevBuf<uint32_t> attr_counts;
+    DevBuf<DTriFrame> tri_frames;
+    DevBuf<DTriFrameJob> tri_frame_jobs;
+    DevBuf<uint32_t> tri_frame_base;
+    uint32_t tri_frame_records = 0;
     mutable std::shared_ptr<ClosestTables> closest;
     mutable DevBuf<uint8_t> closest_cl;
     struct LaunchCtx {
@@ -459,6 +464,8 @@
     mutable int last_packet_walk = -1;
     mutable bool fused_shade = true;
     mutable int last_fused_shade = -1;
+    mutable bool tri_frames_on = true;
+    mutable int last_tri_frames = -1;
     mutable int packet_scene = -1;
     uint32_t ldss_blocks = 0;
     uint32_t cus = 1;
@@ -510,6 +517,7 @@
 DParams base_params(const lg_accel &a, uint32_t w, uint32_t h);
 void set_lds_scene(const lg_accel &a, DParams &P);
 bool scene_lds_image(const Scene &scene, bool pairs, std::vector<uint32_t> &img, uint32_t info[8]);
+uint32_t scene_tri_frames(const FlatScene &f, const Scene &scene, std::vector<uint32_t> &base);
 void ensure_aux_streams(const lg_accel &a, unsigned n);
 void enqueue(const lg_accel &a, DParams &P, bool stats, hipStream_t stream);
 void enqueue_radiance(const lg_accel &a, const double *rays, size_t n, double *radiance, const uint32_t *perm, lg_accel::LaunchCtx &c, hipStream_t stream);
diff --git a/lasgun_amd/csrc/k_tri_frames.hip b/lasgun_amd/csrc/k_tri_frames.hip
--- /dev/null
+++ b/lasgun_amd/csrc/k_tri_frames.hip
@@ -0,0 +1,42 @@
+#include "shade.h"
+
+namespace lg {
+
+__global__ void __launch_bounds__(64) tri_frames_kernel(const DParams P, const DTriFrameJob *jobs, const uint32_t n, DTriFrame *out) {
+    const uint32_t r = blockIdx.x * 64u + threadIdx.x;
+    if (r >= n) return;
+    const uint32_t accel = jobs[r].accel, tri = jobs[r].tri;
+    const uint32_t *vi = P.tri_v + 3ull * tri;
+    const V3 p0 = load_f3(P.vpos, vi[0]), p1 = load_f3(P.vpos, vi[1]), p2 = load_f3(P.vpos, vi[2]);
+    V3 dpdu, dpdv;
+    triangle_partials(P, tri, P.accels[accel].flags, p0, p1, p2, dpdu, dpdv);
+    const V3 c = triangle_c(p0, p1, p2);
+    DTriFrame f;
+    f.c[0] = c.x; f.c[1] = c.y; f.c[2] = c.z;
+    f.pad = 0u;
+#pragma unroll
+    for (int v = 0; v < 2; ++v) {
+        Isect is;
+        isect_set(is, 0.0, dpdu, dpdv);
+        is.has_n = true;
+        is.n = v ? -c : c;
+        const int32_t mat = chain_up(P, accel, is);
+        const FrameAxes ax = frame_axes(is);
+        if (v == 0) {
+            f.ng0[0] = ax.ng0.x; f.ng0[1] = ax.ng0.y; f.ng0[2] = ax.ng0.z;
+            f.ss[0] = ax.ss.x; f.ss[1] = ax.ss.y; f.ss[2] = ax.ss.z;
+            f.mat = mat;
+        }
+        f.ns[v][0] = ax.ns.x; f.ns[v][1] = ax.ns.y; f.ns[v][2] = ax.ns.z;
+        f.ts[v][0] = ax.ts.x; f.ts[v][1] = ax.ts.y; f.ts[v][2] = ax.ts.z;
+    }
+    out[r] = f;
+}
+
+hipError_t launch_tri_frames(const DParams &P, const DTriFrameJob *jobs, uint32_t n, DTriFrame *out, hipStream_t stream) {
+    if (n == 0u) return hipSuccess;
+    hipLaunchKernelGGL(tri_frames_kernel, dim3((n + 63u) / 64u), dim3(64), 0, stream, P, jobs, n, out);
+    return hipGetLastError();
+}
+
+}
diff --git a/lasgun_amd/csrc/k_wavefront.hip b/lasgun_amd/csrc/k_wavefront.hip
--- a/lasgun_amd/csrc/k_wavefront.hip
+++ b/lasgun_amd/csrc/k_wavefront.hip
@@ -241,9 +241,12 @@
             } else if (!hit && mine) P.wf_hq[i] = WF_NONE;
             if (hit) {
                 Shade sh;
-                shade_frame(P, ray, b, sh);
-                if constexpr (FUSED) fused_closest_hit(P, px, i, h, sh);
-                else {
+                if constexpr (FUSED) {
+                    if (__builtin_amdgcn_ballot_w64(!tri_frame_hit(P, b)) == 0ull) shade_frame_tri(P, ray, b, sh);
+                    else shade_frame(P, ray, b, sh);
+                    fused_closest_hit(P, px, i, h, sh);
+                } else {
+                    shade_frame(P, ray, b, sh);
                     const bool skip = P.shadow_skip && shadow_skippable(P, sh);
                     P.wf_hq[h] = skip ? (uint32_t)i | WF_SKIP : (uint32_t)i;
                     if (skip) P.vis[h] = 0u;
diff --git a/lasgun_amd/csrc/launch.cpp b/lasgun_amd/csrc/launch.cpp
--- a/lasgun_amd/csrc/launch.cpp
+++ b/lasgun_amd/csrc/launch.cpp
@@ -2,6 +2,7 @@
 #include "choice.h"
 #include "packet_host.h"
 #include "fused_host.h"
+#include "tri_frames_host.h"
 
 lg_accel::LaunchCtx &ctx_for(const lg_accel &a, hipStream_t stream) {
     for (auto &c : a.ctxs)
@@ -290,6 +291,15 @@
     q.packet_closest = P.packet != 0u;
     q.pair_shadow = wf_takes_pairs(P, a.fast);
     return fused_shade_gate(q) == FUSED_OK ? 1u : 0u;
+}
+
+static bool tri_frames(const lg_accel &a, DParams &P) {
+    static const bool env = env_on("LASGUN_TRI_FRAMES");
+    P.tri_frames = nullptr; P.tri_frame_base = nullptr; P.tri_base = nullptr;
+    if (!tri_frames_launch_gate(a.tri_frames_on && env, P.fused != 0u && P.packet != 0u && P.wf_level == 0u, a.tri_frame_records)) return false;
+    if (!a.tri_frames.p || !a.tri_frame_base.p || !a.accel_tri_base.p || a.tri_frames.n != a.tri_frame_records) return false;
+    P.tri_frames = a.tri_frames.p; P.tri_frame_base = a.tri_frame_base.p; P.tri_base = a.accel_tri_base.p;
+    return true;
 }
 
 struct WfChunk {
@@ -353,12 +363,14 @@
             P.packet = packet_walk(a, P, d == 0 && !own0);
             if (d == 0) a.last_packet_walk = (int)P.packet;
             P.fused = d == 0 ? fused_shade(a, P, !own0 && !l0.every_level(), levels) : 0u;
-            if (d == 0) a.last_fused_shade = (int)P.fused;
+            if (d == 0) { a.last_fused_shade = (int)P.fused; a.last_tri_frames = 0; }
             if (own0) timed(a, 0, ls, [&] { return l0.closest(P, a.fast, tb, depth, ls); });
             else {
                 if (d == 0) a.last_l0_relative = l0_relative(a, P) ? 1 : 0;
+                if (d == 0) a.last_tri_frames = tri_frames(a, P) ? 1 : 0;
                 timed(a, 0, ls, [&] { return launch_wf_trace(P, a.fast, false, tb, depth, ls); });
                 P.l0_rel_n = 0u;
+                P.tri_frames = nullptr; P.tri_frame_base = nullptr; P.tri_base = nullptr;
             }
             if (own0 && l0.own_shadow) {
                 if (l0.shadow_) {
diff --git a/lasgun_amd/csrc/shade.h b/lasgun_amd/csrc/shade.h
--- a/lasgun_amd/csrc/shade.h
+++ b/lasgun_amd/csrc/shade.h
@@ -287,20 +287,65 @@
     return dst;
 }
 
+__device__ __forceinline__ V3 frame_ng0(const Isect &is) { return normalize(cross(is.gu, is.gv)); }
+__device__ __forceinline__ V3 frame_ns(const Isect &is) { return is.has_n ? normalize(is.n) : normalize(cross(is.su, is.sv)); }
+__device__ __forceinline__ V3 frame_ss(const Isect &is) { return normalize(is.su); }
+struct FrameAxes {
+    V3 ng0, ns, ss, ts;
+};
+__device__ __forceinline__ FrameAxes frame_axes(const Isect &is) {
+    FrameAxes ax;
+    ax.ng0 = frame_ng0(is);
+    ax.ns = frame_ns(is);
+    ax.ss = frame_ss(is);
+    ax.ts = cross(ax.ns, ax.ss);
+    return ax;
+}
 __device__ __forceinline__ void shade_frame(const DParams &P, const Ray &ray, const Best &best, Shade &sh) {
     Isect is;
     sh.mat = resolve_hit(P, ray, best, is);
     sh.wo = -normalize(ray.d);
-    sh.ng = face_forward(normalize(cross(is.gu, is.gv)), sh.wo);
-    sh.ns = is.has_n ? normalize(is.n) : normalize(cross(is.su, is.sv));
+    sh.ng = face_forward(frame_ng0(is), sh.wo);
+    sh.ns = frame_ns(is);
     const double err = 2.220446049250313e-16 * 65536.0;
     V3 p = ray.o + ray.d * is.t;
     V3 p_err = sh.ng * err;
     sh.praw = p;
     sh.p = p + p_err;
     sh.pm = p - p_err;
-    sh.ss = normalize(is.su);
+    sh.ss = frame_ss(is);
     sh.ts = cross(sh.ns, sh.ss);
+}
+__device__ __forceinline__ void shade_frame_finish(const Ray &ray, const double t, const V3 ng0, Shade &sh) {
+    sh.wo = -normalize(ray.d);
+    sh.ng = face_forward(ng0, sh.wo);
+    const double err = 2.220446049250313e-16 * 65536.0;
+    V3 p = ray.o + ray.d * t;
+    V3 p_err = sh.ng * err;
+    sh.praw = p;
+    sh.p = p + p_err;
+    sh.pm = p - p_err;
+}
+
+__device__ __forceinline__ bool tri_frame_hit(const DParams &P, const Best &best) {
+    return P.tri_frames && (best.ref >> 30) == PK_TRIANGLE && P.tri_frame_base[best.accel] != NO_HIT;
+}
+__device__ __forceinline__ void shade_frame_tri(const DParams &P, const Ray &ray, const Best &best, Shade &sh) {
+    const Ray lr = local_ray(P, ray, best.accel);
+    const uint32_t idx = best.ref & PRIM_INDEX_MASK;
+    const uint32_t *vi = P.tri_v + 3ull * idx;
+    TriHit h;
+    triangle_t(load_f3(P.vpos, vi[0]), load_f3(P.vpos, vi[1]), load_f3(P.vpos, vi[2]), lr, h);
+    const DTriFrame *f = P.tri_frames + (P.tri_frame_base[best.accel] + (idx - P.tri_base[best.accel]));
+    const V3 c{f->c[0], f->c[1], f->c[2]};
+    const bool flip = dot(c, -lr.d) < 0.0;
+    const V3 ns0{f->ns[0][0], f->ns[0][1], f->ns[0][2]}, ns1{f->ns[1][0], f->ns[1][1], f->ns[1][2]};
+    const V3 ts0{f->ts[0][0], f->ts[0][1], f->ts[0][2]}, ts1{f->ts[1][0], f->ts[1][1], f->ts[1][2]};
+    sh.mat = f->mat;
+    sh.ns = flip ? ns1 : ns0;
+    sh.ts = flip ? ts1 : ts0;
+    sh.ss = V3{f->ss[0], f->ss[1], f->ss[2]};
+    shade_frame_finish(ray, h.t, V3{f->ng0[0], f->ng0[1], f->ng0[2]}, sh);
 }
 
 __device__ __forceinline__ void stash_put(const DParams &P, unsigned long long g, const Shade &sh) {
diff --git a/lasgun_amd/csrc/tri_frames_host.h b/lasgun_amd/csrc/tri_frames_host.h
--- /dev/null
+++ b/lasgun_amd/csrc/tri_frames_host.h
@@ -0,0 +1,79 @@
+#pragma once
+#include <cstddef>
+#include <cstdint>
+
+#include "dscene.h"
+
+namespace lg {
+
+constexpr uint32_t TRI_FRAMES_MAX_INSTANCE = 1024u;
+constexpr uint32_t TRI_FRAMES_MAX_RECORDS = 4096u;
+constexpr size_t TRI_FRAME_BYTES = 176u;
+static_assert(sizeof(DTriFrame) == TRI_FRAME_BYTES, "one record");
+
+enum TriFramesRefusal : int {
+    TRI_FRAMES_OK = 0,
+    TRI_FRAMES_NOT_MESH = 1,
+    TRI_FRAMES_HAS_NORMALS = 2,
+    TRI_FRAMES_EMPTY = 3,
+    TRI_FRAMES_INSTANCE_CAP = 4,
+    TRI_FRAMES_MALFORMED = 5,
+};
+
+struct TriFramesAccel {
+    uint32_t flags, tri_base, faces;
+};
+
+inline TriFramesRefusal tri_frames_accel_gate(const TriFramesAccel &A, size_t n_tris) {
+    if (!(A.flags & AF_MESH)) return TRI_FRAMES_NOT_MESH;
+    if (A.flags & AF_HAS_N) return TRI_FRAMES_HAS_NORMALS;
+    if (A.faces == 0u) return TRI_FRAMES_EMPTY;
+    if (A.faces > TRI_FRAMES_MAX_INSTANCE) return TRI_FRAMES_INSTANCE_CAP;
+    if ((size_t)A.tri_base >= n_tris || (size_t)A.faces > n_tris - (size_t)A.tri_base) return TRI_FRAMES_MALFORMED;
+    return TRI_FRAMES_OK;
+}
+
+inline uint32_t tri_frames_plan(const TriFramesAccel *accels, size_t n_accels, size_t n_tris, uint32_t *base) {
+    size_t total = 0;
+    for (size_t a = 0; a < n_accels; ++a) {
+        base[a] = NO_HIT;
+        if (tri_frames_accel_gate(accels[a], n_tris) != TRI_FRAMES_OK) continue;
+        if (total <= TRI_FRAMES_MAX_RECORDS) base[a] = (uint32_t)total;
+        total += accels[a].faces;
+    }
+    if (total > TRI_FRAMES_MAX_RECORDS) {
+        for (size_t a = 0; a < n_accels; ++a) base[a] = NO_HIT;
+        return 0u;
+    }
+    return (uint32_t)total;
+}
+
+inline bool tri_frames_plan_ok(const TriFramesAccel *accels, size_t n_accels, size_t n_tris, const uint32_t *base, uint32_t records) {
+    if (records > TRI_FRAMES_MAX_RECORDS) return false;
+    size_t next = 0;
+    for (size_t a = 0; a < n_accels; ++a) {
+        if (base[a] == NO_HIT) continue;
+        if (tri_frames_accel_gate(accels[a], n_tris) != TRI_FRAMES_OK) return false;
+        if ((size_t)base[a] != next) return false;
+        next += accels[a].faces;
+        if (next > (size_t)records) return false;
+    }
+    return next == (size_t)records;
+}
+
+inline bool tri_frames_jobs(const TriFramesAccel *accels, size_t n_accels, size_t n_tris, const uint32_t *base, uint32_t records, DTriFrameJob *jobs) {
+    if (!tri_frames_plan_ok(accels, n_accels, n_tris, base, records)) return false;
+    for (size_t a = 0; a < n_accels; ++a) {
+        if (base[a] == NO_HIT) continue;
+        for (uint32_t k = 0; k < accels[a].faces; ++k) jobs[(size_t)base[a] + k] = DTriFrameJob{(uint32_t)a, accels[a].tri_base + k};
+    }
+    return true;
+}
+
+inline size_t tri_frames_bytes(uint32_t records) { return (size_t)records * TRI_FRAME_BYTES; }
+
+inline bool tri_frames_launch_gate(bool switched_on, bool fused_packet_closest, uint32_t records) {
+    return switched_on && fused_packet_closest && records != 0u && records <= TRI_FRAMES_MAX_RECORDS;
+}
+
+}
diff --git a/lasgun_amd/csrc/walk.h b/lasgun_amd/csrc/walk.h
--- a/lasgun_amd/csrc/walk.h
+++ b/lasgun_amd/csrc/walk.h
@@ -265,11 +265,7 @@
     else isect_set(is, t, dpdv, dpdu);
 }
 
-__device__ __forceinline__ void triangle_full(const DParams &P, uint32_t tri, uint32_t aflags, const Ray &ray, Isect &is) {
-    const uint32_t *vi = P.tri_v + 3ull * tri;
-    V3 p0 = load_f3(P.vpos, vi[0]), p1 = load_f3(P.vpos, vi[1]), p2 = load_f3(P.vpos, vi[2]);
-    TriHit h;
-    triangle_t(p0, p1, p2, ray, h);
+__device__ __forceinline__ void triangle_partials(const DParams &P, uint32_t tri, uint32_t aflags, V3 p0, V3 p1, V3 p2, V3 &dpdu, V3 &dpdv) {
     double uv[3][2];
     if (aflags & AF_HAS_UV) {
         const uint32_t *ti = P.tri_t + 3ull * tri;
@@ -282,7 +278,6 @@
     double duv12x = uv[1][0] - uv[2][0], duv12y = uv[1][1] - uv[2][1];
     V3 dp02 = p0 - p2, dp12 = p1 - p2;
     double determinant = (duv02x * duv12y) - (duv02y * duv12x);
-    V3 dpdu, dpdv;
     if (determinant == 0.0) {
         coordinate_system(cross(p2 - p1, p1 - p0), dpdu, dpdv);
     } else {
@@ -290,6 +285,16 @@
         dpdu = (duv12y * dp02 - duv02y * dp12) * inv;
         dpdv = (-duv12x * dp02 - duv02x * dp12) * inv;
     }
+}
+__device__ __forceinline__ V3 triangle_c(V3 p0, V3 p1, V3 p2) { return cross(p0 - p2, p1 - p2); }
+
+__device__ __forceinline__ void triangle_full(const DParams &P, uint32_t tri, uint32_t aflags, const Ray &ray, Isect &is) {
+    const uint32_t *vi = P.tri_v + 3ull * tri;
+    V3 p0 = load_f3(P.vpos, vi[0]), p1 = load_f3(P.vpos, vi[1]), p2 = load_f3(P.vpos, vi[2]);
+    TriHit h;
+    triangle_t(p0, p1, p2, ray, h);
+    V3 dpdu, dpdv;
+    triangle_partials(P, tri, aflags, p0, p1, p2, dpdu, dpdv);
     isect_set(is, h.t, dpdu, dpdv);
     if (aflags & AF_HAS_N) {
         const uint32_t *ni = P.tri_n + 3ull * tri;
@@ -303,7 +308,7 @@
         is.su = ss; is.sv = ts;
     } else {
         is.has_n = true;
-        is.n = face_forward(cross(dp02, dp12), -ray.d);
+        is.n = face_forward(triangle_c(p0, p1, p2), -ray.d);
     }
 }
 
@@ -1571,6 +1576,29 @@
     if (!same) cnt.a_viol++;
 }
 
+__device__ __forceinline__ int32_t chain_up(const DParams &P, uint32_t accel, Isect &is) {
+    int32_t isect_mat = P.default_material;
+    int32_t a = (int32_t)accel;
+    while (a >= 0) {
+        const DAccel *A = P.accels + a;
+        V3 gu = xf_vector(A->m, is.gu), gv = xf_vector(A->m, is.gv);
+        if (vne(is.gu, is.su) || vne(is.gv, is.sv)) {
+            is.su = xf_vector(A->m, is.su); is.sv = xf_vector(A->m, is.sv);
+        } else {
+            is.su = gu; is.sv = gv;
+        }
+        is.gu = gu; is.gv = gv;
+        if (is.has_n) is.n = xf_normal(A->minv, is.n);
+        if (A->material >= 0) isect_mat = A->material;
+        if (A->flags & AF_SWAP_BACKFACE) {
+            V3 tmp = is.gu; is.gu = is.gv; is.gv = tmp;
+            tmp = is.su; is.su = is.sv; is.sv = tmp;
+            if (is.has_n) is.n = -is.n;
+        }
+        a = A->parent;
+    }
+    return isect_mat;
+}
 __device__ __forceinline__ int32_t resolve_hit(const DParams &P, const Ray &wray, const Best &best, Isect &is) {
     Ray lr = local_ray(P, wray, best.accel);
     uint32_t kind = best.ref >> 30, idx = best.ref & PRIM_INDEX_MASK;
@@ -1592,26 +1620,7 @@
     } else {
         triangle_full(P, idx, P.accels[best.accel].flags, lr, is);
     }
-    int32_t isect_mat = P.default_material;
-    int32_t a = (int32_t)best.accel;
-    while (a >= 0) {
-        const DAccel *A = P.accels + a;
-        V3 gu = xf_vector(A->m, is.gu), gv = xf_vector(A->m, is.gv);
-        if (vne(is.gu, is.su) || vne(is.gv, is.sv)) {
-            is.su = xf_vector(A->m, is.su); is.sv = xf_vector(A->m, is.sv);
-        } else {
-            is.su = gu; is.sv = gv;
-        }
-        is.gu = gu; is.gv = gv;
-        if (is.has_n) is.n = xf_normal(A->minv, is.n);
-        if (A->material >= 0) isect_mat = A->material;
-        if (A->flags & AF_SWAP_BACKFACE) {
-            V3 tmp = is.gu; is.gu = is.gv; is.gv = tmp;
-            tmp = is.su; is.su = is.sv; is.sv = tmp;
-            if (is.has_n) is.n = -is.n;
-        }
-        a = A->parent;
-    }
+    const int32_t isect_mat = chain_up(P, best.accel, is);
     return prim_mat >= 0 ? prim_mat : isect_mat;
 }
 
```

Result: faster. 6274 Mrays/s (median of 6 runs) (+4.4%).
